# yesint/molar

Measured on AMD Instinct MI355X. Metric: frames/sec + Matom-pairs/sec, 1M-atom PBC neighbor search + RMSD fit, higher is better.
Workload: dtype f32; 1 GPU; 1M-atom synthetic triclinic box A, per frame: PBC neighbour search rc=1.2 nm (ordered pair list in HBM) + Kabsch RMSD fit/COM/gyration of a 100k-atom selection; natoms=1000000, selection_atoms=100000, frames_per_gpu=1451, parallelism=frames sharded over 1 rank(s), no data-path collective, streams_per_gpu=2, measure_overlapped_with_search=True

## Files before the change

include/molar_hip.h:

```cpp
#ifndef MOLAR_HIP_H
#define MOLAR_HIP_H

#include <stddef.h>
#include <stdint.h>

#ifdef __cplusplus
extern "C" {
#endif

enum {
    MOLAR_HIP_OK = 0,
    MOLAR_HIP_ERR_SIZES = 1,
    MOLAR_HIP_ERR_ZERO_MASS = 2,
    MOLAR_HIP_ERR_SVD = 3,
    MOLAR_HIP_ERR_NO_PBC = 4,
    MOLAR_HIP_ERR_ZERO_LENGTH_VECTOR = 5,
    MOLAR_HIP_ERR_INVERSE_FAILED = 6,
    MOLAR_HIP_ERR_LIPID_TAIL_TOO_SHORT = 7,
    MOLAR_HIP_ERR_LIPID_NORMALS_COUNT = 8,
    MOLAR_HIP_ERR_LIPID_BOND_ORDER_COUNT = 9,
    MOLAR_HIP_ERR_ANGLE_TOO_SMALL = 10,
    MOLAR_HIP_ERR_INVALID_ARGUMENT = 50,
    MOLAR_HIP_ERR_TOO_LARGE = 51,
    MOLAR_HIP_ERR_NO_SEARCH = 52,
// ... 54 lines not shown
    int32_t kind;
    float cutoff;
    const float *xyz1;
    size_t natoms1;
    const uint64_t *idx1;
    size_t n1;
    const float *xyz2;
    size_t natoms2;
    const uint64_t *idx2;
    size_t n2;
    const float *vdw1;
    const float *vdw2;
    int32_t ids_local;
    const float *box9;
    uint8_t pbc;
    const float *lower3;
    const float *upper3;
} molar_hip_search_desc;

int molar_hip_search_count(molar_hip_ctx *ctx, const molar_hip_search_desc *desc, uint64_t *out_count);
int molar_hip_search_fill(molar_hip_ctx *ctx, uint32_t *pairs, float *dist);
int molar_hip_search_fill_usize(molar_hip_ctx *ctx, uint64_t *i, uint64_t *j, float *dist);
int molar_hip_search_fill_ids(molar_hip_ctx *ctx, uint64_t *ids);
int molar_hip_within_count(molar_hip_ctx *ctx, const molar_hip_search_desc *desc, uint64_t *out_count);
int molar_hip_within_fill(molar_hip_ctx *ctx, uint64_t *ids);
int molar_hip_within_hold(molar_hip_ctx *ctx, int on);
int molar_hip_search_connectivity(molar_hip_ctx *ctx, const molar_hip_search_desc *desc, uint64_t *out_rows, uint64_t *out_entries);
int molar_hip_search_connectivity_fill(molar_hip_ctx *ctx, uint64_t *offsets, uint64_t *neigh);
int molar_hip_unwrap_connectivity(molar_hip_ctx *ctx, float *xyz, size_t natoms, const uint64_t *idx, size_t n,
                                  const float *box9, float cutoff, uint8_t pbc_dims, uint64_t *group_offsets,
                                  uint64_t *group_ids, size_t *ngroups);
int molar_hip_search_grid_dims(molar_hip_ctx *ctx, uint64_t dims[3]);
int molar_hip_search_cell_kernels(molar_hip_ctx *ctx, int32_t *lanes, uint64_t occupied_cells[2]);
int molar_hip_search_fill_device(molar_hip_ctx *ctx, const uint32_t **d_pairs, const float **d_dist);
int molar_hip_search_resident(molar_hip_ctx *ctx, const molar_hip_search_desc *desc, uint64_t *out_count,
                              const uint32_t **d_pairs, const float **d_dist);
int molar_hip_search_resident_planes(molar_hip_ctx *ctx, int want_dist);
int molar_hip_search_resident_begin(molar_hip_ctx *ctx, const molar_hip_search_desc *desc, int32_t *ticket);
int molar_hip_search_resident_end(molar_hip_ctx *ctx, int32_t ticket, uint64_t *out_count, const uint32_t **d_pairs,
                                  const float **d_dist);
int molar_hip_search_histogram(molar_hip_ctx *ctx, const molar_hip_search_desc *desc, float hmin,
                               float hmax, size_t nbins, uint64_t *bins, uint64_t *out_count);
int molar_hip_search_histogram_frames(molar_hip_ctx *ctx, const molar_hip_search_desc *desc, size_t nframes, size_t xyz1_stride,
                                      size_t xyz2_stride, const float *boxes9, float hmin, float hmax, size_t nbins,
                                      uint64_t *bins);
int molar_hip_histogram_edges(float hmin, float hmax, size_t nbins, float *edges);

typedef struct {
    const uint32_t *group1;
    size_t ngroups1;
    const uint32_t *group2;
    size_t ngroups2;
} molar_hip_contact_groups;

int molar_hip_search_contacts(molar_hip_ctx *ctx, const molar_hip_search_desc *desc, const molar_hip_contact_groups *groups ,
                              uint64_t *deg1, uint64_t *deg2, uint64_t *map, uint64_t *out_count);
int molar_hip_search_contacts_frames(molar_hip_ctx *ctx, const molar_hip_search_desc *desc, const molar_hip_contact_groups *groups,
                                     size_t nframes, size_t xyz1_stride, size_t xyz2_stride, const float *boxes9,
                                     uint64_t *deg1, uint64_t *deg2, uint64_t *map, uint32_t *occupancy);

typedef struct {
    int32_t kind;
    double cutoff;
    const double *xyz1;
    size_t natoms1;
    const uint64_t *idx1;
// ... 351 lines not shown
```

molar_amd/_lib.py:

```python
from __future__ import annotations

import ctypes as C
import os

HERE = os.path.dirname(os.path.abspath(__file__))
DEFAULT_LIB = os.path.join(HERE, "libmolar_hip.so")

_lib = None


class MolarHipError(RuntimeError):

    def __init__(self, code: int, msg: str):
        super().__init__(f"[molar_hip status {code}] {msg}")
        self.code = code


class Box(C.Structure):
    _fields_ = [("m", C.c_float * 9), ("inv", C.c_float * 9), ("nshift", C.c_int32), ("shifts", C.c_float * 78)]


class SearchDesc(C.Structure):
    _fields_ = [
        ("kind", C.c_int32), ("cutoff", C.c_float),
# ... 48 lines not shown


_P, _SZ, _F, _I, _U8 = C.c_void_p, C.c_size_t, C.c_float, C.c_int, C.c_uint8
SYMBOLS = {
    "molar_hip_create": (C.c_void_p, [_I]),
    "molar_hip_destroy": (None, [_P]),
    "molar_hip_last_error": (C.c_char_p, []),
    "molar_hip_version": (C.c_char_p, []),
    "molar_hip_device_count": (_I, []),
    "molar_hip_set_stream": (_I, [_P, _P]),
    "molar_hip_synchronize": (_I, [_P]),
    "molar_hip_profile_enable": (_I, [_P, _I]),
    "molar_hip_profile_read": (_I, [_P, _P, _P]),
    "molar_hip_box_from_matrix": (_I, [_P, _P]),
    "molar_hip_box_from_vectors_angles": (_I, [_F, _F, _F, _F, _F, _F, _P]),
    "molar_hip_box_shortest_vector": (None, [_P, _P, _U8, _P]),
    "molar_hip_copy_bandwidth": (_I, [_P, _SZ, _I, _P]),
    "molar_hip_write_bandwidth": (_I, [_P, _SZ, _I, _P]),
    "molar_hip_box_lab_extents": (None, [_P, _P]),
    "molar_hip_box_extents": (None, [_P, _P]),
    "molar_hip_box_to_box_coords": (None, [_P, _P, _P]),
    "molar_hip_box_to_lab_coords": (None, [_P, _P, _P]),
    "molar_hip_box_is_inside": (_I, [_P, _P]),
    "molar_hip_box_wrap_point": (None, [_P, _P, _P]),
    "molar_hip_search_count": (_I, [_P, _P, _P]),
    "molar_hip_search_fill": (_I, [_P, _P, _P]),
    "molar_hip_search_fill_usize": (_I, [_P, _P, _P, _P]),
    "molar_hip_search_fill_ids": (_I, [_P, _P]),
    "molar_hip_within_count": (_I, [_P, _P, _P]),
    "molar_hip_within_fill": (_I, [_P, _P]),
    "molar_hip_within_hold": (_I, [_P, _I]),
    "molar_hip_search_grid_dims": (_I, [_P, _P]),
    "molar_hip_search_cell_kernels": (_I, [_P, _P, _P]),
    "molar_hip_search_count_f64": (_I, [_P, _P, _P]),
    "molar_hip_search_fill_f64": (_I, [_P, _P, _P, _P]),
    "molar_hip_search_fill_ids_f64": (_I, [_P, _P]),
    "molar_hip_search_grid_dims_f64": (_I, [_P, _P]),
    "molar_hip_search_histogram_f64": (_I, [_P, _P, C.c_double, C.c_double, _SZ, _P, _P]),
    "molar_hip_search_histogram_frames_f64": (_I, [_P, _P, _SZ, _SZ, _SZ, _P, C.c_double, C.c_double, _SZ, _P]),
    "molar_hip_histogram_edges_f64": (_I, [C.c_double, C.c_double, _SZ, _P]),
    "molar_hip_within_count_f64": (_I, [_P, _P, _P]),
    "molar_hip_within_fill_f64": (_I, [_P, _P]),
    "molar_hip_search_connectivity_f64": (_I, [_P, _P, _P, _P]),
    "molar_hip_unwrap_connectivity_f64": (_I, [_P, _P, _SZ, _P, _SZ, _P, C.c_double, _U8, _P, _P, _P]),
    "molar_hip_search_resident": (_I, [_P, _P, _P, _P, _P]),
    "molar_hip_search_fill_device": (_I, [_P, _P, _P]),
    "molar_hip_search_resident_planes": (_I, [_P, _I]),
    "molar_hip_search_resident_begin": (_I, [_P, _P, _P]),
    "molar_hip_search_resident_end": (_I, [_P, C.c_int32, _P, _P, _P]),
    "molar_hip_search_histogram": (_I, [_P, _P, _F, _F, _SZ, _P, _P]),
    "molar_hip_search_histogram_frames": (_I, [_P, _P, _SZ, _SZ, _SZ, _P, _F, _F, _SZ, _P]),
    "molar_hip_histogram_edges": (_I, [_F, _F, _SZ, _P]),
    "molar_hip_search_contacts": (_I, [_P, _P, _P, _P, _P, _P, _P]),
    "molar_hip_search_contacts_frames": (_I, [_P, _P, _P, _SZ, _SZ, _SZ, _P, _P, _P, _P, _P]),
    "molar_hip_min_max": (_I, [_P, _P, _SZ, _P, _SZ, _P, _P]),
    "molar_hip_center_of_geometry": (_I, [_P, _P, _SZ, _P, _SZ, _P]),
    "molar_hip_center_of_mass": (_I, [_P, _P, _SZ, _P, _SZ, _P, _P]),
    "molar_hip_center_of_geometry_pbc": (_I, [_P, _P, _SZ, _P, _SZ, _P, _U8, _P]),
    "molar_hip_center_of_mass_pbc": (_I, [_P, _P, _SZ, _P, _SZ, _P, _P, _U8, _P]),
    "molar_hip_gyration": (_I, [_P, _P, _SZ, _P, _SZ, _P, _P, _P]),
    "molar_hip_inertia": (_I, [_P, _P, _SZ, _P, _SZ, _P, _P, _P, _P, _P]),
    "molar_hip_rmsd": (_I, [_P, _P, _SZ, _P, _SZ, _P, _SZ, _P, _SZ, _P]),
    "molar_hip_rmsd_mw": (_I, [_P, _P, _SZ, _P, _SZ, _P, _P, _SZ, _P, _SZ, _P]),
    "molar_hip_fit_transform": (_I, [_P, _P, _SZ, _P, _SZ, _P, _P, _SZ, _P, _SZ, _P, _I, _P, _P]),
    "molar_hip_xtc_histogram": (_I, [_P, _P, _SZ, _SZ, _P, _SZ, _F, _U8, _F, _F, _SZ, _P, _I]),
    "molar_hip_xtc_histogram_double": (_I, [_P, _P, _SZ, _SZ, _P, _SZ, _P, _SZ, _F, _U8, _F, _F, _SZ, _P, _I]),
# ... 133 lines not shown
```

molar_amd/api.py:

```python
from __future__ import annotations

import collections
import ctypes as C

import numpy as np

from . import _lib
from ._lib import (MEMBRANE_ARRAYS, Box, ContactGroups, MembraneDesc, MembraneOut, MembraneView, MolarHipError, SearchDesc, SearchDescF64,
                   check)

PBC_FULL = 7
PBC_NONE = 0

SEARCH_SINGLE, SEARCH_DOUBLE, SEARCH_WITHIN, SEARCH_DOUBLE_VDW = 0, 1, 2, 3


def _is_torch(x) -> bool:
    return type(x).__module__.startswith("torch")


def _addr(x):
    if x is None:
        return None, None
    if _is_torch(x):
# ... 214 lines not shown
            b9 = box.colmajor9() if isinstance(box, PeriodicBox) else np.ascontiguousarray(
                np.asarray(box, np.float32).reshape(3, 3).T).reshape(9)
            keep.append(b9)
            d.box9 = b9.ctypes.data
        d.pbc = pbc_mask(pbc)
        if lower is not None:
            lo = np.ascontiguousarray(lower, np.float32); up = np.ascontiguousarray(upper, np.float32)
            keep += [lo, up]
            d.lower3 = lo.ctypes.data
            d.upper3 = up.ctypes.data
        return d, keep

    def search_count(self, kind, cutoff, xyz1, idx1=None, xyz2=None, idx2=None, box=None, pbc=0, vdw1=None,
                     vdw2=None, ids_local=False, lower=None, upper=None) -> int:
        d, keep = self._search_desc(kind, cutoff, xyz1, idx1, xyz2, idx2, box, pbc, vdw1, vdw2, ids_local, lower, upper)
        cnt = C.c_uint64(0)
        check(self.lib.molar_hip_search_count(self.ctx, C.byref(d), C.byref(cnt)))
        self._keep = keep
        return int(cnt.value)

    def make_search_desc(self, kind, cutoff, xyz1, **kw):
        return self._search_desc(kind, cutoff, xyz1, **kw)

    def search_resident_desc(self, desc):
        cnt = C.c_uint64(0); p = C.c_void_p(); dd = C.c_void_p()
        check(self.lib.molar_hip_search_resident(self.ctx, C.byref(desc), C.byref(cnt), C.byref(p), C.byref(dd)))
        return int(cnt.value), p.value, dd.value

    def search_cell_kernels(self):
        lanes = C.c_int32(-1)
        occ = (C.c_uint64 * 2)()
        check(self.lib.molar_hip_search_cell_kernels(self.ctx, C.byref(lanes), occ))
        return int(lanes.value), (int(occ[0]), int(occ[1]))

    def search_resident_planes(self, want_dist=True):
        check(self.lib.molar_hip_search_resident_planes(self.ctx, 1 if want_dist else 0))

    def search_resident_begin(self, desc):
        t = C.c_int32(-1)
        check(self.lib.molar_hip_search_resident_begin(self.ctx, C.byref(desc), C.byref(t)))
        return int(t.value)

    def search_resident_end(self, ticket):
        cnt = C.c_uint64(0); p = C.c_void_p(); dd = C.c_void_p()
        check(self.lib.molar_hip_search_resident_end(self.ctx, C.c_int32(ticket), C.byref(cnt), C.byref(p), C.byref(dd)))
        return int(cnt.value), p.value, dd.value

    def search_resident(self, kind, cutoff, xyz1, idx1=None, xyz2=None, idx2=None, box=None, pbc=0, vdw1=None,
                        vdw2=None, ids_local=False, lower=None, upper=None):
        d, keep = self._search_desc(kind, cutoff, xyz1, idx1, xyz2, idx2, box, pbc, vdw1, vdw2, ids_local, lower, upper)
        cnt = C.c_uint64(0); p = C.c_void_p(); dd = C.c_void_p()
        check(self.lib.molar_hip_search_resident(self.ctx, C.byref(d), C.byref(cnt), C.byref(p), C.byref(dd)))
        self._keep = keep
        return int(cnt.value), p.value, dd.value

    def search_fill(self, count):
        pairs = np.empty((count, 2), np.uint32)
        dist = np.empty(count, np.float32)
        check(self.lib.molar_hip_search_fill(self.ctx, pairs.ctypes.data, dist.ctypes.data))
        return pairs, dist

    def search_fill_usize(self, count):
        i = np.empty(count, np.uint64); j = np.empty(count, np.uint64); d = np.empty(count, np.float32)
        check(self.lib.molar_hip_search_fill_usize(self.ctx, i.ctypes.data, j.ctypes.data, d.ctypes.data))
        return i, j, d

# ... 1729 lines not shown
```

molar_amd/build.py:

```python
from __future__ import annotations

import fcntl
import hashlib
import os
import subprocess

HERE = os.path.dirname(os.path.abspath(__file__))
CSRC = os.path.join(HERE, "csrc")
LIB = os.path.join(HERE, "libmolar_hip.so")
SOURCES = ["api.hip", "search.hip", "search_f64.hip", "measure.hip", "measure_f64.hip", "membrane.hip", "xtc.hip", "pair_k0.hip", "pair_k1.hip", "pair_k2.hip", "pair_k3.hip", "pair_k4.hip", "pair_k5.hip", "pair_k6.hip", "pair_k7.hip", "pair_k8.hip", "pair_k9.hip", "pair_small.hip", "devsort.hip", "sasa.hip", "rmsd_matrix.hip", "fluct.hip", "msd.hip"]
HEADERS = ["common.hpp", "boxmath.hpp", "linalg3.hpp", "pair_kernels.hpp", "hist_kernels.hpp", "contact_kernels.hpp", "hoststream.hpp", "stages.hpp", "csr_kernels.hpp", "unwrap_walk.hpp", "search_shape.hpp", os.path.join("..", "..", "include", "molar_hip.h")]
FLAGS = ["--offload-arch=gfx950", "-O3", "-std=c++17", "-fPIC", "-ffp-contract=off", "-fno-fast-math",
         "-Wall", "-Wno-unused-function",
         "-fno-slp-vectorize"]
FLAGS += os.environ.get("MOLAR_HIP_EXTRA_FLAGS", "").split()


HASH_FILE = LIB + ".srchash"


def _source_hash() -> str:
    h = hashlib.sha256()
    h.update(" ".join(FLAGS).encode())
    for name in sorted(SOURCES + HEADERS):
        with open(os.path.join(CSRC, name), "rb") as f:
            h.update(name.encode())
            h.update(f.read())
    return h.hexdigest()


def needs_build() -> bool:
    if not os.path.exists(LIB) or not os.path.exists(HASH_FILE):
        return True
    try:
        return open(HASH_FILE).read().strip() != _source_hash()
    except OSError:
        return True


def build_library(force: bool = False, verbose: bool = False) -> str:
    if not force and not needs_build():
        return LIB
    with open(os.path.join(HERE, ".build.lock"), "w") as lock:
# ... 127 lines not shown
```

molar_amd/csrc/api.hip:

```cpp
#include "boxmath.hpp"
#include <algorithm>

#include "common.hpp"
#include "hoststream.hpp"
namespace mh { void search64_release(molar_hip_ctx *c); }
namespace mh { void sasa_release(molar_hip_ctx *c); }
namespace mh { void rmsd_matrix_release(molar_hip_ctx *c); }
namespace mh { void fluct_release(molar_hip_ctx *c); }
namespace mh { void msd_release(molar_hip_ctx *c); }
#include <cstdlib>

using namespace mh;

typedef float v4f_copy __attribute__((ext_vector_type(4)));
__global__ __launch_bounds__(256) void k_copy_f4(const float4 *__restrict__ src, float4 *__restrict__ dst, size_t n) {
    for (size_t i = (size_t)blockIdx.x * 256u + threadIdx.x; i < n; i += (size_t)gridDim.x * 256u) dst[i] = src[i];
}
template <bool NT>
__global__ __launch_bounds__(256) void k_copy_f4x4(const v4f_copy *__restrict__ src, v4f_copy *__restrict__ dst, size_t n) {
    for (size_t i = (size_t)blockIdx.x * 1024u + threadIdx.x; i < n; i += (size_t)gridDim.x * 1024u) {
        v4f_copy v0, v1, v2, v3;
        if (NT) {
            v0 = __builtin_nontemporal_load(src + i);
            v1 = __builtin_nontemporal_load(src + i + 256);
// ... 121 lines not shown
    if ((e = hipStreamCreateWithFlags(&c->stream, hipStreamNonBlocking)) != hipSuccess) {
        fail(MOLAR_HIP_ERR_HIP, "hipStreamCreate: %s", hipGetErrorString(e));
        delete c;
        return nullptr;
    }
    c->own_stream = true;
#ifdef MOLAR_HIP_AB_KNOBS
    c->env_no_side = std::getenv("MOLAR_HIP_NO_SIDE_STREAM") != nullptr;
    c->env_no_mfma = std::getenv("MOLAR_HIP_NO_MFMA_COUNT") != nullptr;
    c->env_no_mfma_wrapped = std::getenv("MOLAR_HIP_NO_MFMA_WRAPPED") != nullptr;
    c->env_no_tile_sum = std::getenv("MOLAR_HIP_NO_TILE_SUM") != nullptr;
    c->env_host_grid_wait = std::getenv("MOLAR_HIP_HOST_GRID_WAIT") != nullptr;
    c->env_no_bin_tile = std::getenv("MOLAR_HIP_NO_BIN_TILE") != nullptr;
#endif
#ifdef MOLAR_HIP_DEBUG_KNOBS
    if (const char *dbg = std::getenv("MOLAR_HIP_DEBUG_SKIP")) c->env_debug_skip = (uint32_t)std::atoi(dbg);
    if (const char *dbg = std::getenv("MOLAR_HIP_DEBUG_LAUNCH")) c->env_debug_launch = (uint32_t)std::atoi(dbg);
#endif
    if (ensure_pinned(c, 1 << 16)) {
        (void)hipStreamDestroy(c->stream);
        delete c;
        return nullptr;
    }
    return c;
}

void molar_hip_destroy(molar_hip_ctx *c) {
    if (!c) return;
    (void)hipSetDevice(c->device);
    (void)hipStreamSynchronize(c->stream);
    if (c->side_stream) (void)hipStreamSynchronize(c->side_stream);
    for (auto &gen : c->set_store) for (auto &s : gen) {
        for (DevBuf *b : {&s.xyz_stage, &s.idx_stage, &s.vdw_stage, &s.key, &s.cell_count, &s.cnt_pad, &s.cursor, &s.tmp_key, &s.sort_buf,
                          &s.sorted, &s.sorted_vdw, &s.aabb, &s.perm, &s.chunk_aabb, &s.h16, &s.cell_org})
            b->release();
    }
    if (c->aux) molar_hip_destroy(c->aux);
    if (c->contacts) {
        c->contacts->stream = c->stream;
        molar_hip_destroy(c->contacts);
    }
    for (DevBuf *b : {&c->xh_win[0], &c->xh_win[1], &c->xh_bins, &c->fit_redo, &c->ct_g1, &c->ct_g2, &c->ct_acc, &c->ct_frame, &c->ct_occ}) b->release();
    for (auto &gen : c->hb_sets) for (auto &fr : gen) for (auto &s : fr) {
        for (DevBuf *b : {&s.xyz_stage, &s.idx_stage, &s.vdw_stage, &s.key, &s.cell_count, &s.cnt_pad, &s.cursor, &s.tmp_key, &s.sort_buf,
                          &s.sorted, &s.sorted_vdw, &s.aabb, &s.perm, &s.chunk_aabb, &s.h16, &s.cell_org})
            b->release();
    }
    for (DevBuf *b : {&c->hb_lean[0], &c->hb_lean[1], &c->hb_rest[0], &c->hb_rest[1], &c->hb_blocks[0], &c->hb_blocks[1]}) b->release();
    if (c->hb_pin) (void)hipHostFree(c->hb_pin);
    for (auto e : c->hb_pin_ev)
        if (e) (void)hipEventDestroy(e);
    for (DevBuf *b : {&c->params, &c->task_desc, &c->task_nb, &c->slot_desc, &c->slot_cnt, &c->slot_base, &c->tile_sum, &c->scan_tmp, &c->sort_tmp, &c->sort_tmp_side, &c->scan_tmp_side, &c->scan_state, &c->fplan_tiles, &c->out_pairs_set[0], &c->out_dist_set[0], &c->out_pairs_set[1], &c->out_dist_set[1], &c->out_ids,
                      &c->wide_i, &c->wide_j, &c->hist, &c->hist_queue, &c->slot_desc_rest, &c->hist_edges, &c->dbg, &c->conn_deg, &c->conn_off, &c->conn_ent, &c->conn_neigh, &c->w_flags, &c->w_list, &c->w_part_cnt, &c->w_part, &c->w_tile_cnt, &c->w_tile_off, &c->task_mu, &c->task_moff, &c->maskbuf, &c->m_xyz1, &c->m_xyz2, &c->m_idx1, &c->m_idx2,
                      &c->m_mass1, &c->m_mass2, &c->m_partials, &c->m_results, &c->m_out})
        b->release();
    for (auto &s : c->spans) {
        (void)hipEventDestroy(s.a);
        (void)hipEventDestroy(s.b);
    }
    for (auto e : c->event_pool) (void)hipEventDestroy(e);
    if (c->h_pinned) (void)hipHostFree(c->h_pinned);
    mh::ring_release(c);
    mh::search64_release(c);
    mh::sasa_release(c);
    mh::rmsd_matrix_release(c);
    mh::fluct_release(c);
    mh::msd_release(c);
    if (c->h_sizes) (void)hipHostFree(c->h_sizes);
    for (auto &t : c->tickets)
        if (t.done) (void)hipEventDestroy(t.done);
    if (c->grid_done) (void)hipEventDestroy(c->grid_done);
    for (auto e : c->gen_free)
        if (e) (void)hipEventDestroy(e);
    if (c->side_stream) (void)hipStreamDestroy(c->side_stream);
    if (c->own_stream) (void)hipStreamDestroy(c->stream);
    delete c;
}

int molar_hip_set_stream(molar_hip_ctx *c, void *hip_stream) {
    if (!c) return fail(MOLAR_HIP_ERR_INVALID_ARGUMENT, "null context");
    MH_HIP(hipSetDevice(c->device));
    MH_HIP(hipStreamSynchronize(c->stream));
    if (c->own_stream) (void)hipStreamDestroy(c->stream);
    c->stream = reinterpret_cast<hipStream_t>(hip_stream);
    c->own_stream = false;
// ... 118 lines not shown
```

molar_amd/csrc/common.hpp:

```cpp
#pragma once

#include <hip/hip_runtime.h>

#include <cstdarg>
#include <cstdint>
#include <cstdio>
#include <cstring>
#include <string>
#include <vector>

#include "../../include/molar_hip.h"

namespace mh {


inline std::string &last_error() {
    static thread_local std::string e;
    return e;
}

inline int fail(int code, const char *fmt, ...) {
    char buf[512];
    va_list ap;
    va_start(ap, fmt);
// ... 51 lines not shown
inline bool is_device_ptr(const void *p) {
    if (!p) return false;
    hipPointerAttribute_t a;
    hipError_t e = hipPointerGetAttributes(&a, p);
    if (e != hipSuccess) {
        (void)hipGetLastError();
        return false;
    }
    return a.type == hipMemoryTypeDevice || a.type == hipMemoryTypeManaged || a.type == hipMemoryTypeArray;
}


struct GridSet {
    uint32_t n = 0;
    DevBuf xyz_stage;
    DevBuf idx_stage;
    DevBuf vdw_stage;
    const float *d_xyz = nullptr;
    const uint64_t *d_idx = nullptr;
    const float *d_vdw = nullptr;
    DevBuf key;
    DevBuf cell_count;
    DevBuf cnt_pad;
    DevBuf cursor;
    DevBuf tmp_key;
    DevBuf sort_buf;
    DevBuf sorted;
    DevBuf sorted_vdw;
    DevBuf aabb;
    DevBuf perm;
    DevBuf chunk_aabb;
    DevBuf h16;
    DevBuf cell_org;
};

struct SearchShape {
    int kind = 0;
    bool use_box = false;
    uint8_t pbc = 0;
    float cutoff = 0.f;
    molar_hip_box box{};
    float lower[3]{}, upper[3]{};
    uint32_t dims[3]{1, 1, 1};
    uint64_t ntasks = 0;
    uint64_t nslots_bound = 0;
    GridSet *set = nullptr;
    uint32_t occ_use[2] = {0, 0};
};

}

struct molar_hip_search64_state;
struct molar_hip_sasa_state;
struct molar_hip_rmsd_matrix_state;
struct molar_hip_fluct_state;
struct molar_hip_msd_state;

#ifndef MH_HIST_BATCH
#define MH_HIST_BATCH 16
#endif

struct molar_hip_ctx {
    int device = 0;
    hipStream_t stream = nullptr;
    bool own_stream = false;
    int num_cus = 256;
// ... 10 lines not shown

    bool have_search = false;
    mh::SearchShape cur;
    uint64_t total = 0;
    mh::GridSet set_store[2][2];
    molar_hip_ctx() { cur.set = set_store[0]; }
    hipStream_t side_stream = nullptr;
    hipEvent_t grid_done = nullptr;
    bool env_no_side = false;
    bool env_no_mfma = false;
    bool env_no_mfma_wrapped = false;
    bool env_host_grid_wait = false;
    bool env_no_tile_sum = false;
    uint32_t env_debug_skip = 0;
    uint32_t env_debug_launch = 0, dbg_launches = 0;
    hipEvent_t gen_free[2] = {nullptr, nullptr};
    bool env_no_bin_tile = false;
    int hist_gen = 0;
    bool on_side = false;
    mh::DevBuf scan_tmp_side;
    mh::DevBuf params;
    mh::DevBuf task_desc;
    mh::DevBuf task_nb;
    mh::DevBuf slot_desc;
    mh::DevBuf slot_cnt;
    mh::DevBuf slot_base;
    mh::DevBuf tile_sum;
    bool params_fresh = false;
    unsigned long long params_fresh_cap = 0;
    mh::DevBuf scan_tmp;
    mh::DevBuf sort_tmp, sort_tmp_side;
    mh::DevBuf scan_state;
    mh::DevBuf fplan_tiles;
    mh::DevBuf out_pairs_set[2];
    mh::DevBuf out_dist_set[2];
    mh::DevBuf &out_pairs = out_pairs_set[0];
    mh::DevBuf &out_dist = out_dist_set[0];
    struct Ticket {
        bool pending = false, degenerate = false;
        unsigned long long cap0 = 0, maskcap0 = 0, serial = 0, launched = 0, ntasks = 0;
        int kind = -1;
        unsigned long long occ_key = 0;
        hipEvent_t done = nullptr;
        molar_hip_search_desc desc{};
    } tickets[2];
    int next_ticket = 0;
    bool resident_no_dist = false;
    unsigned long long search_serial = 0;
    unsigned long long trim_real = 0, trim_ntasks = 0;
    int trim_kind = -1;
    void *h_sizes = nullptr;
    unsigned long long occ_key = 0;
    uint32_t occ_cells[2] = {0, 0};
    bool occ_valid = false;
    mh::DevBuf out_ids;
    mh::DevBuf wide_i, wide_j;
    mh::DevBuf hist;
    mh::DevBuf dbg;
    mh::DevBuf hist_queue;
    mh::DevBuf slot_desc_rest;
    unsigned long long hist_frames = 0;
    mh::GridSet hb_sets[2][MH_HIST_BATCH][2];
    bool hb_zeroed[2][MH_HIST_BATCH][2] = {};
    uint32_t hb_zeroed_cells[2][MH_HIST_BATCH][2] = {};
    mh::DevBuf hb_lean[2], hb_rest[2];
    mh::DevBuf hb_blocks[2];
// ... 114 lines not shown
```

molar_amd/csrc/pair_kernels.hpp:

```cpp
#pragma once

#include "boxmath.hpp"
#include "common.hpp"

namespace mh {
namespace pairk {

enum { MODE_COUNT = 0, MODE_FILL = 1, MODE_HIST = 2 };

#ifndef MH_COUNT_WPE
#define MH_COUNT_WPE 6
#endif
#ifndef MH_FILL_WPE
#define MH_FILL_WPE 8
#endif
#ifndef MH_WPB
#define MH_WPB 1
#endif
constexpr int waves_per_block(int mode) { return mode == MODE_HIST ? 4 : MH_WPB; }
constexpr int KREG = 8;
constexpr int FIFO_CAP = 128;
#ifndef MOLAR_HIP_NO_WIDE_FLUSH
#define MOLAR_HIP_WIDE_FLUSH 1
#endif
constexpr int FIFO_WIDE = 256;
constexpr uint32_t XCD_RUN = 128;
constexpr float F32_EPS = 1.1920929e-07f;
constexpr bool MASKED_COUNT_SORTED = true;

static __constant__ uint8_t MASKS[14][6] = {
    {0, 0, 0, 0, 0, 0},
    {0, 0, 0, 1, 0, 0}, {0, 0, 0, 0, 1, 0}, {0, 0, 0, 0, 0, 1},
    {0, 0, 0, 1, 1, 0}, {0, 0, 0, 1, 0, 1}, {0, 0, 0, 0, 1, 1},
    {0, 0, 0, 1, 1, 1},
    {1, 0, 0, 0, 1, 0}, {1, 0, 0, 0, 0, 1}, {0, 1, 0, 0, 0, 1},
    {1, 1, 0, 0, 0, 1}, {1, 0, 1, 0, 1, 0}, {0, 1, 1, 1, 0, 0},
};


typedef float v4f_t __attribute__((ext_vector_type(4)));
__device__ __forceinline__ float4 gload4(const float4 *p, size_t i) {
    const v4f_t v = ((const __attribute__((address_space(1))) v4f_t *)p)[i];
    return make_float4(v.x, v.y, v.z, v.w);
}
__device__ __forceinline__ uint32_t gload_u32(const uint32_t *p, size_t i) {
    return ((const __attribute__((address_space(1))) uint32_t *)p)[i];
}
__device__ __forceinline__ void gstore_u32(uint32_t *p, size_t i, uint32_t v) {
    ((__attribute__((address_space(1))) uint32_t *)p)[i] = v;
}
__device__ __forceinline__ float uniform_f32(float v) { return __uint_as_float(__builtin_amdgcn_readfirstlane(__float_as_uint(v))); }
__device__ __forceinline__ float4 lload4(const float4 *p, uint32_t i) {
    const v4f_t v = ((const __attribute__((address_space(3))) v4f_t *)p)[i];
    return make_float4(v.x, v.y, v.z, v.w);
// ... 37 lines not shown
#ifdef MOLAR_HIP_DEBUG_KNOBS
    uint32_t debug_skip;
    unsigned long long *dbg;
#endif
    float cutoff2;
    uint64_t ntasks;
    molar_hip_box box;
    alignas(16) float shifts4[96];
    uint32_t hist_big;
};

struct TaskDesc {
    uint32_t a0, n1, b0, n2, cb, flags, pad0, pad1;
};

struct SlotDesc {
    uint32_t a0, n1, b0, n2;
    uint32_t cb, flags, i0, frame;
    unsigned long long moff, pad1;
};
static_assert(sizeof(SlotDesc) == 48, "SlotDesc is read with three 16-byte loads");

struct Task {
    uint32_t a0, n1, b0, n2;
    uint32_t rps;
    uint32_t cb;
    uint32_t ca;
    uint32_t wrap_b;
    uint32_t wrap;
    bool tri;
    bool valid;
};

template <int KIND, bool UNIFORM>
__device__ __forceinline__ Task decode_task(const SearchParams &P, uint64_t t) {
    Task T;
    T.valid = false;
    T.tri = false;
    T.a0 = T.b0 = T.n1 = T.n2 = 0;
    T.cb = 0;
    T.ca = 0;
    T.wrap_b = 0;
    T.rps = 64u;
    T.wrap = 0;
    uint32_t half = 0;
    uint64_t e = t;
    if (KIND != MOLAR_HIP_SEARCH_SINGLE) {
        half = (uint32_t)(t & 1ull);
        e = t >> 1;
    }
    const uint32_t m = (uint32_t)(e % 14ull);
    const uint64_t cidx = e / 14ull;
    const uint32_t z = (uint32_t)(cidx % P.dz);
    const uint64_t r = cidx / P.dz;
    const uint32_t y = (uint32_t)(r % P.dy);
    const uint32_t x = (uint32_t)(r / P.dy);
    const uint32_t dims[3] = {P.dx, P.dy, P.dz};
    uint32_t c[2][3] = {{x + MASKS[m][0], y + MASKS[m][1], z + MASKS[m][2]},
                        {x + MASKS[m][3], y + MASKS[m][4], z + MASKS[m][5]}};
    uint32_t wrap = 0, wrap_c2 = 0;
    for (int i = 0; i < 2; ++i)
        for (int d = 0; d < 3; ++d)
            if (c[i][d] == dims[d]) {
                if ((P.pbc >> d) & 1u) {
                    c[i][d] = 0;
                    wrap |= 1u << d;
// ... 414 lines not shown
    if (P.box.nshift != 0 && wrap == MOLAR_HIP_PBC_FULL) {
        if (WIDE4) {
            for (int k = 0; k < P.box.nshift; k += 4) {
                float sh[12];
#pragma unroll
                for (int q = 0; q < 12; ++q) sh[q] = P.shifts4[3 * k + q];
#pragma unroll
                for (int q = 0; q < 4; ++q) {
                    const float cx = sx + sh[3 * q], cy = sy + sh[3 * q + 1], cz = sz + sh[3 * q + 2];
                    const float n2 = (cx * cx + cy * cy) + cz * cz;
                    best2 = n2 < best2 ? n2 : best2;
                }
            }
        } else {
            for (int k = 0; k < P.box.nshift; ++k) {
                const float cx = sx + P.box.shifts[3 * k], cy = sy + P.box.shifts[3 * k + 1], cz = sz + P.box.shifts[3 * k + 2];
                const float n2 = (cx * cx + cy * cy) + cz * cz;
                best2 = n2 < best2 ? n2 : best2;
            }
        }
    }
    return best2;
}

__device__ __forceinline__ float aabb_d2(float ax, float ay, float az, float lx, float ly, float lz, float hx, float hy,
                                         float hz) {
    const float ex = fmaxf(fmaxf(lx - ax, ax - hx), 0.f);
    const float ey = fmaxf(fmaxf(ly - ay, ay - hy), 0.f);
    const float ez = fmaxf(fmaxf(lz - az, az - hz), 0.f);
    return (ex * ex + ey * ey) + ez * ez;
}

template <int KIND, int NCH, bool TRI>
__device__ __forceinline__ uint32_t run_count_sorted(const SearchParams &P, const Task &T, uint32_t i0, float4 *la,
                                                     uint32_t lane) {
    const float cutoff2 = P.cutoff2;
    const uint32_t rows = __builtin_amdgcn_readfirstlane(T.n1 - i0 < T.rps ? T.n1 - i0 : T.rps);
    float4 a = make_float4(0.f, 0.f, 0.f, 0.f);
    if (lane < rows) a = gload4(P.sa, T.a0 + i0 + lane);
    la[lane] = a;
    float bx[NCH], by[NCH], bz[NCH];
    uint32_t bpos[NCH];
#pragma unroll
    for (int k = 0; k < NCH; ++k) {
        const uint32_t jj = (uint32_t)k * 64u + lane;
        float4 q = make_float4(3.0e38f, 3.0e38f, 3.0e38f, 0.f);
        uint32_t pj = 0u;
        if (jj < T.n2) {
            q = gload4(P.perm_b, T.b0 + jj);
            pj = __float_as_uint(q.w);
        }
        bx[k] = q.x; by[k] = q.y; bz[k] = q.z; bpos[k] = pj;
    }
    const uint32_t ubase = (T.b0 >> 6) + T.cb;
    unsigned long long livek[NCH];
#pragma unroll
    for (int k = 0; k < NCH; ++k) {
        const float4 lo = gload4(P.chunk_aabb_b, 2u * (ubase + k)), hi = gload4(P.chunk_aabb_b, 2u * (ubase + k) + 1u);
        const bool need = lane < rows && !(aabb_d2(a.x, a.y, a.z, lo.x, lo.y, lo.z, hi.x, hi.y, hi.z) > cutoff2);
        livek[k] = __builtin_amdgcn_ballot_w64(need);
    }
    __builtin_amdgcn_wave_barrier();
    uint32_t acc = 0;
    unsigned long long live = 0ull;
#pragma unroll
    for (int k = 0; k < NCH; ++k) live |= livek[k];
    while (live) {
        const uint32_t r = (uint32_t)__builtin_ctzll(live);
        live &= ~(1ull << r);
        const float4 p = lload4(la, r);
#pragma unroll
        for (int k = 0; k < NCH; ++k) {
            if (!((livek[k] >> r) & 1ull)) continue;
            const float dx = bx[k] - p.x, dy = by[k] - p.y, dz = bz[k] - p.z;
            float d2 = (dx * dx + dy * dy) + dz * dz;
            if (TRI) d2 = (bpos[k] > i0 + r) ? d2 : INFINITY;
            asm volatile("v_cmp_ge_f32 vcc, %2, %1\n\tv_addc_co_u32 %0, vcc, 0, %0, vcc" : "+v"(acc) : "v"(d2), "s"(cutoff2) : "vcc");
        }
    }
    for (int off = 32; off > 0; off >>= 1) acc += __shfl_xor(acc, off, 64);
    return acc;
}

typedef _Float16 v8h_t __attribute__((ext_vector_type(8)));
typedef float v16f_t __attribute__((ext_vector_type(16)));

__device__ __forceinline__ uint32_t pack_h2(_Float16 a, _Float16 b) {
    return (uint32_t)__builtin_bit_cast(unsigned short, a) | ((uint32_t)__builtin_bit_cast(unsigned short, b) << 16);
}

constexpr int MFMA_TILES = 10;

__device__ __forceinline__ float mfma_error_bound(float R, float c) {
    return 2.3841858e-07f * ((16.0f * R * R + 8.0f * c) + (4.0f * R + 1.0f));
}
__device__ __forceinline__ bool mfma_bound_usable(float R, float E, float c) {
    return R < 64.0f && E < 0.02f * c && (c + R * R) < 3.0e4f;
}

template <int KIND, bool TRI>
__device__ __forceinline__ uint32_t run_count_mfma(const SearchParams &P, const Task &T, uint32_t i0, float4 *la, uint4 *lh,
                                                   uint32_t lane, bool &done) {
    typedef uint32_t u4_t __attribute__((ext_vector_type(4)));
    typedef __attribute__((address_space(3))) u4_t lds_u4;
    typedef __attribute__((address_space(3))) uint32_t lds_u32;
    typedef __attribute__((address_space(1))) u4_t glb_u4;
    const float cutoff2 = P.cutoff2;
    const uint32_t rows = __builtin_amdgcn_readfirstlane(T.n1 - i0 < T.rps ? T.n1 - i0 : T.rps);
    const uint32_t kh = lane >> 5, cl = lane & 31u;
    const uint32_t nct = (T.n2 + 31u) >> 5;
    float4 a = make_float4(0.f, 0.f, 0.f, 0.f);
    if (lane < rows) a = gload4(P.sa, T.a0 + i0 + lane);
    const float4 org = gload4(P.cell_org_b, T.cb);
    bool need = lane < rows;
    if (!TRI) {
        const float4 blo = gload4(P.aabb_b, 2 * T.cb), bhi = gload4(P.aabb_b, 2 * T.cb + 1);
        need = need && !(aabb_d2(a.x, a.y, a.z, blo.x, blo.y, blo.z, bhi.x, bhi.y, bhi.z) > cutoff2);
    }
    const unsigned long long live = __builtin_amdgcn_ballot_w64(need);
    const uint32_t nlive = TRI ? rows : (uint32_t)__popcll(live);
    if (!TRI && nlive == 0u) return 0u;
    const uint32_t rank = TRI ? lane : __builtin_amdgcn_mbcnt_hi((uint32_t)(live >> 32), __builtin_amdgcn_mbcnt_lo((uint32_t)live, 0u));
    u4_t bq[MFMA_TILES];
#pragma unroll
    for (int t = 0; t < MFMA_TILES; ++t) {
        const uint32_t col = (uint32_t)t * 32u + cl;
        if (32u * (uint32_t)(t + 1) <= T.n2) {
            bq[t] = ((const glb_u4 *)P.h16_b)[T.b0 + col];
        } else {
            bq[t] = u4_t{0u, 0u, 0u, 0x00007BFFu};
            if (col < T.n2) bq[t] = ((const glb_u4 *)P.h16_b)[T.b0 + col];
        }
    }
    if (TRI || need) la[rank] = a;
    const float r0 = a.x - org.x, r1 = a.y - org.y, r2 = a.z - org.z;
    float ra2 = need ? (r0 * r0 + r1 * r1) + r2 * r2 : 0.0f;
    const bool fin = ra2 == ra2;
    for (int off = 32; off > 0; off >>= 1) ra2 = fmaxf(ra2, __shfl_xor(ra2, off, 64));
    const float R = 1.0001f * __builtin_sqrtf(ra2) + org.w;
    const float E = uniform_f32(mfma_error_bound(R, cutoff2));
    if (__builtin_amdgcn_ballot_w64(!fin) != 0ull || !mfma_bound_usable(R, E, cutoff2)) {
        done = false;
        return 0u;
    }
    {
        u4_t k0 = {0u, 0u, 0u, 0x00007BFFu}, k1 = {0u, 0u, 0u, 0x3C003C00u};
        if (!TRI) {
            ((lds_u4 *)lh)[2u * lane] = k0;
// ... 53 lines not shown
                    m = __builtin_fminf(m, __builtin_fabsf(acc[i]));
                }
                if (__builtin_amdgcn_ballot_w64(m < E) == 0ull) {
                    cnt += (uint32_t)__popc(h);
                } else {
                    if (lane == 0) todo[ntodo] = (uint32_t)(2 * t + rt);
                    ++ntodo;
                }
            }
        }
    }
    if (ntodo) {
        __builtin_amdgcn_wave_barrier();
        for (uint32_t q = 0; q < ntodo; ++q) {
            const uint32_t id = __builtin_amdgcn_readfirstlane(todo[q]);
            const uint32_t ct = id >> 1, rt = id & 1u;
            const uint32_t col = ct * 32u + cl;
            float4 b = make_float4(3.0e38f, 3.0e38f, 3.0e38f, 0.f);
            if (col < T.n2) b = gload4(P.sb, T.b0 + col);
            for (uint32_t r = 0; r < 16u; ++r) {
                const uint32_t row = 32u * rt + 16u * kh + r;
                const float4 p = lload4(la, row);
                const float dx = b.x - p.x, dy = b.y - p.y, dz = b.z - p.z;
                const float d2 = (dx * dx + dy * dy) + dz * dz;
                cnt += (row < nlive && (!TRI || col > i0 + row) && d2 <= cutoff2) ? 1u : 0u;
            }
        }
    }
    for (int off = 32; off > 0; off >>= 1) cnt += __shfl_xor(cnt, off, 64);
    return cnt;
}

template <int KIND>
__device__ __forceinline__ bool run_count_mfma_wrapped(const SearchParams &P, const Task &T, uint32_t i0, float4 *la, uint4 *lh,
                                                       uint32_t lane, uint32_t *mwords, uint32_t &count_out) {
    typedef uint32_t u4_t __attribute__((ext_vector_type(4)));
    typedef __attribute__((address_space(3))) u4_t lds_u4;
    typedef __attribute__((address_space(3))) uint32_t lds_u32;
    typedef __attribute__((address_space(1))) u4_t glb_u4;
    const float cutoff2 = P.cutoff2;
    const uint32_t rows = __builtin_amdgcn_readfirstlane(T.n1 - i0 < 64u ? T.n1 - i0 : 64u);
    const uint32_t kh = lane >> 5, cl = lane & 31u;
    const uint32_t nct = (T.n2 + 31u) >> 5, nch = (T.n2 + 63u) >> 6;
    float Sx = 0.f, Sy = 0.f, Sz = 0.f;
    for (int d = 0; d < 3; ++d) {
        if (!((T.wrap >> d) & 1u)) continue;
        const float sgn = ((T.wrap_b >> d) & 1u) ? 1.0f : -1.0f;
        Sx += sgn * P.box.m[3 * d];
        Sy += sgn * P.box.m[3 * d + 1];
        Sz += sgn * P.box.m[3 * d + 2];
    }
    float4 a = make_float4(0.f, 0.f, 0.f, 0.f);
    if (lane < rows) a = gload4(P.sa, T.a0 + i0 + lane);
    const float4 org = gload4(P.cell_org_b, T.cb);
    const float4 blo = gload4(P.aabb_b, 2 * T.cb), bhi = gload4(P.aabb_b, 2 * T.cb + 1);
    const bool need = lane < rows && !(aabb_d2(a.x - Sx, a.y - Sy, a.z - Sz, blo.x, blo.y, blo.z, bhi.x, bhi.y, bhi.z) > P.prune_limit2);
    const unsigned long long live = __builtin_amdgcn_ballot_w64(need);
    const uint32_t nlive = (uint32_t)__popcll(live);
    if (nlive == 0u) {
        count_out = 0u;
        return true;
    }
    const uint32_t rank = __builtin_amdgcn_mbcnt_hi((uint32_t)(live >> 32), __builtin_amdgcn_mbcnt_lo((uint32_t)live, 0u));
    const float r0 = (a.x - Sx) - org.x, r1 = (a.y - Sy) - org.y, r2 = (a.z - Sz) - org.z;
    float ra2 = need ? (r0 * r0 + r1 * r1) + r2 * r2 : 0.0f;
    float big = need ? fmaxf(fmaxf(fabsf(a.x), fabsf(a.y)), fabsf(a.z)) : 0.0f;
    const bool fin = ra2 == ra2;
    for (int off = 32; off > 0; off >>= 1) {
        ra2 = fmaxf(ra2, __shfl_xor(ra2, off, 64));
        big = fmaxf(big, __shfl_xor(big, off, 64));
    }
    const float R = 1.0001f * __builtin_sqrtf(ra2) + org.w;
    const float rc = __builtin_sqrtf(P.band_hi);
    const float L = (fmaxf(fmaxf(fabsf(org.x), fabsf(org.y)), fabsf(org.z)) + R) + (fmaxf(fmaxf(fabsf(Sx), fabsf(Sy)), fabsf(Sz)) + big);
    const float Em = mfma_error_bound(R, cutoff2);
    const float E = uniform_f32((P.band_hi - cutoff2) * 1.0001f + Em + 4.0f * (5.9604645e-08f * (2.0f * L + 2.0f * rc)) * rc);
    if (__builtin_amdgcn_ballot_w64(!fin || !(E == E) || !mfma_bound_usable(R, Em, cutoff2) || !(E < 0.06f * cutoff2)) != 0ull) return false;
    u4_t bq[MFMA_TILES];
#pragma unroll
    for (int t = 0; t < MFMA_TILES; ++t) {
        const uint32_t col = (uint32_t)t * 32u + cl;
        if (32u * (uint32_t)(t + 1) <= T.n2) {
            bq[t] = ((const glb_u4 *)P.h16_b)[T.b0 + col];
        } else {
            bq[t] = u4_t{0u, 0u, 0u, 0x00007BFFu};
            if (col < T.n2) bq[t] = ((const glb_u4 *)P.h16_b)[T.b0 + col];
        }
    }
    {
// ... 69 lines not shown
                cnt += (uint32_t)__popc(word);
                gstore_u32(mwords, ((uint32_t)rt * nch + (uint32_t)k) * 64u + lane, word);
            }
        }
    }
    if (ntodo > TODO_CAP) return false;
    if (ntodo) {
        asm volatile("s_waitcnt vmcnt(0)" ::: "memory");
        __builtin_amdgcn_wave_barrier();
        for (uint32_t q0 = 0; q0 < ntodo; q0 += 64u) {
            bool hx = false;
            uint32_t rl = 0u, col = 0u;
            if (q0 + lane < ntodo) {
                const uint32_t e = todo[q0 + lane];
                rl = e >> 16;
                col = e & 0xFFFFu;
                if (rl < nlive && col < T.n2) {
                    const float4 b = gload4(P.sb, T.b0 + col);
                    const float4 p = lload4(la, rl);
                    hx = wrapped_d2_exact(P, T.wrap, b.x - p.x, b.y - p.y, b.z - p.z) <= cutoff2;
                }
            }
            if (hx) atomicOr(mwords + ((rl >> 5) * nch + (col >> 6)) * 64u + (col & 63u), 0x80000000u >> (rl & 31u));
            const unsigned long long mx = __builtin_amdgcn_ballot_w64(hx);
            if (lane == 0) cnt += (uint32_t)__popcll(mx);
        }
    }
    for (int off = 32; off > 0; off >>= 1) cnt += __shfl_xor(cnt, off, 64);
    count_out = cnt;
    return true;
}

template <int KIND, bool FILL, bool WRAPPED, int NCH, bool TRI, bool MASKED>
__device__ __forceinline__ uint32_t run_fast(const SearchParams &P, const Task &T, uint32_t i0, Fifo &F, float4 *la,
                                             uint32_t lane, uint32_t *mwords) {
    static_assert(!(WRAPPED && TRI), "a triangular (same-cell) entry never wraps on the fast path");
    if constexpr (!FILL && !WRAPPED && MASKED_COUNT_SORTED) return run_count_sorted<KIND, NCH, TRI>(P, T, i0, la, lane);
    const bool approx = WRAPPED && P.approx_wrapped != 0u && !(P.box.nshift != 0 && T.wrap == MOLAR_HIP_PBC_FULL);
    float Sx = 0.f, Sy = 0.f, Sz = 0.f;
    if (WRAPPED && approx) {
        for (int d = 0; d < 3; ++d) {
            if (!((T.wrap >> d) & 1u)) continue;
            const float sgn = ((T.wrap_b >> d) & 1u) ? 1.0f : -1.0f;
            Sx += sgn * P.box.m[3 * d];
            Sy += sgn * P.box.m[3 * d + 1];
            Sz += sgn * P.box.m[3 * d + 2];
        }
    }
    constexpr bool REPLAY = FILL && MASKED;
    float bx[NCH], by[NCH], bz[NCH];
    uint32_t bid[NCH];
    if (!REPLAY) {
#pragma unroll
        for (int k = 0; k < NCH; ++k) {
            const uint32_t jj = (uint32_t)k * 64u + lane;
            float4 q = make_float4(3.0e38f, 3.0e38f, 3.0e38f, 0.f);
            if (jj < T.n2) {
                q = gload4(P.sb, T.b0 + jj);
                if (WRAPPED) { q.x += Sx; q.y += Sy; q.z += Sz; }
            }
            bx[k] = q.x; by[k] = q.y; bz[k] = q.z; bid[k] = __float_as_uint(q.w);
        }
    }
    const float cutoff2 = P.cutoff2;
    const float band_lo = P.band_lo, band_hi = P.band_hi;
    const uint32_t rows = __builtin_amdgcn_readfirstlane(T.n1 - i0 < T.rps ? T.n1 - i0 : T.rps);
    unsigned long long live;
    {
        float4 a = make_float4(0.f, 0.f, 0.f, 0.f);
        if (lane < rows) a = gload4(P.sa, T.a0 + i0 + lane);
        la[lane] = a;
        const float4 lo = gload4(P.aabb_b, 2 * T.cb), hi = gload4(P.aabb_b, 2 * T.cb + 1);
        bool need = true;
        if (TRI) {
        } else if (!WRAPPED) {
            need = !(aabb_d2(a.x, a.y, a.z, lo.x, lo.y, lo.z, hi.x, hi.y, hi.z) > cutoff2);
        } else if (approx) {
            need = !(aabb_d2(a.x - Sx, a.y - Sy, a.z - Sz, lo.x, lo.y, lo.z, hi.x, hi.y, hi.z) > P.prune_limit2);
        }
        live = __builtin_amdgcn_ballot_w64(lane < rows && need);
    }
    __builtin_amdgcn_wave_barrier();
    uint32_t total = 0;

    if (REPLAY) {
        if (!mwords) return 0u;
        F.recompute = WRAPPED ? 1u : 2u;
        F.la = la;
        F.wrap = T.wrap;
        F.fq = F.fq_store;
        float4 q[NCH];
#pragma unroll
        for (int k = 0; k < NCH; ++k) {
            const uint32_t jj = (uint32_t)k * 64u + lane;
            q[k] = make_float4(0.f, 0.f, 0.f, 0.f);
            if (jj < T.n2) q[k] = gload4(P.sb, T.b0 + jj);
        }
        uint32_t w[NCH];
        uint32_t nrow = 0;
        while (live) {
            if ((nrow & 31u) == 0u) {
#pragma unroll
                for (int k = 0; k < NCH; ++k) w[k] = gload_u32(mwords, ((nrow >> 5) * NCH + k) * 64u + lane);
            }
            ++nrow;
            const uint32_t r = (uint32_t)__builtin_ctzll(live);
            live &= ~(1ull << r);
// ... 143 lines not shown
                            else acc += 1u;
                        }
                    }
                }
                acc_hi = acc;
            }
        }
        if (!FILL && MASKED) {
            if ((++nrow & 31u) == 0u) store_group((nrow >> 5) - 1u, 32u);
        }
    }
    if (!FILL) {
        if (MASKED && (nrow & 31u) != 0u) store_group(nrow >> 5, nrow & 31u);
        for (int off = 32; off > 0; off >>= 1) acc += __shfl_xor(acc, off, 64);
        total = acc;
    } else if (F.tail != F.head) {
        __builtin_amdgcn_wave_barrier();
        if (WIDE) {
            while (F.tail != F.head) {
                const uint32_t c = F.tail - F.head < 64u ? F.tail - F.head : 64u;
                fifo_flush<KIND, FIFO_WIDE>(P, F, c, lane);
            }
        } else {
            fifo_flush<KIND>(P, F, F.tail - F.head, lane);
        }
    }
    if (FILL) F.recompute = 0u;
    return total;
}

constexpr int KMAX_WIDE = 16;
constexpr int KMAX_HUGE = 32;
template <int KIND, bool FILL, int WK, bool MASKED, int KMAX = KREG>
__device__ __forceinline__ uint32_t run_task_nch(const SearchParams &P, const Task &T, uint32_t i0, Fifo &F, float4 *la,
                                                 uint32_t lane, uint32_t *mwords) {
    const uint32_t nchunks = (T.n2 + 63u) >> 6;
    if constexpr (KMAX > KMAX_WIDE) {
        if ((KIND == MOLAR_HIP_SEARCH_SINGLE || KIND == MOLAR_HIP_SEARCH_DOUBLE) && nchunks > (uint32_t)KREG && nchunks <= (uint32_t)KMAX) {
            constexpr bool WR = WK != WK_NONE;
            const bool tri = KIND == MOLAR_HIP_SEARCH_SINGLE && WK == WK_NONE && T.tri;
            if (!T.tri || tri) {
#define MH_HUGE_CASE(N)                                                                                              \
    if (nchunks <= (uint32_t)(N)) {                                                                                  \
        if (tri) {                                                                                                   \
            if constexpr (KIND == MOLAR_HIP_SEARCH_SINGLE && WK == WK_NONE)                                          \
                return run_fast<KIND, FILL, false, N, true, false>(P, T, i0, F, la, lane, nullptr);                  \
        }                                                                                                            \
        return run_fast<KIND, FILL, WR, N, false, false>(P, T, i0, F, la, lane, nullptr);                            \
    }
                MH_HUGE_CASE(16) MH_HUGE_CASE(20) MH_HUGE_CASE(24) MH_HUGE_CASE(28) MH_HUGE_CASE(32)
#undef MH_HUGE_CASE
            }
        }
    } else if constexpr (KMAX > KREG) {
        if ((KIND == MOLAR_HIP_SEARCH_SINGLE || KIND == MOLAR_HIP_SEARCH_DOUBLE) && nchunks > (uint32_t)KREG && nchunks <= (uint32_t)KMAX) {
            constexpr bool WR = WK != WK_NONE;
            const bool tri = KIND == MOLAR_HIP_SEARCH_SINGLE && WK == WK_NONE && T.tri;
            if (!T.tri || tri) {
#define MH_WIDE_CASE(N)                                                                                              \
    case N:                                                                                                          \
        if (tri) {                                                                                                   \
            if constexpr (KIND == MOLAR_HIP_SEARCH_SINGLE && WK == WK_NONE)                                          \
                return run_fast<KIND, FILL, false, N, true, false>(P, T, i0, F, la, lane, nullptr);                  \
        }                                                                                                            \
        return run_fast<KIND, FILL, WR, N, false, false>(P, T, i0, F, la, lane, nullptr);
                switch (nchunks) {
                    MH_WIDE_CASE(9) MH_WIDE_CASE(10) MH_WIDE_CASE(11) MH_WIDE_CASE(12)
// ... 105 lines not shown
            SlotDesc z;
            z.a0 = z.n1 = z.b0 = z.n2 = z.cb = z.flags = z.i0 = z.frame = 0u;
            z.moff = ~0ull >> 1;
            z.pad1 = 0ull;
            slot_desc[s] = z;
        }
        return;
    }
    const uint32_t s0 = task_first[t], s1 = task_first[t + 1];
    if (s1 == s0) return;
    const TaskDesc d = task_desc[t];
    const uint32_t rps = d.flags >> 16, nch = (d.n2 + 63u) >> 6;
    const unsigned long long m0 = task_moff ? task_moff[t] : (~0ull >> 1);
    for (uint32_t s = s0; s < s1; ++s) {
        SlotDesc o;
        o.a0 = d.a0; o.n1 = d.n1; o.b0 = d.b0; o.n2 = d.n2;
        o.cb = d.cb; o.flags = d.flags; o.i0 = (s - s0) * rps; o.frame = 0u;
        o.moff = task_moff ? m0 + (unsigned long long)(s - s0) * 2u * nch : m0;
        o.pad1 = 0ull;
        slot_desc[s] = o;
    }
}

template <int KIND>
__device__ __forceinline__ bool hist_lean_slot(const SearchParams &P, uint32_t flags, uint32_t n2) {
    if (KIND != MOLAR_HIP_SEARCH_SINGLE && KIND != MOLAR_HIP_SEARCH_DOUBLE) return false;
    if (((n2 + 63u) >> 6) > (uint32_t)KREG && !P.hist_big) return false;
    const uint32_t wrap = flags & 7u;
    if (!(P.use_box && wrap != 0u)) return true;
    if (flags & 0x100u) return false;
    return P.approx_wrapped != 0u && !(P.box.nshift != 0 && wrap == MOLAR_HIP_PBC_FULL);
}

template <int KIND, int MODE, int WPE = 0>
__global__ void __launch_bounds__(64 * waves_per_block(MODE))
__attribute__((amdgpu_waves_per_eu(WPE ? WPE : (MODE == MODE_HIST ? 4 : (MODE == MODE_COUNT ? MH_COUNT_WPE : MH_FILL_WPE))))) pair_kernel(const SearchParams *__restrict__ Pp,
                                                     const SlotDesc *__restrict__ slot_desc,
                                                     const uint32_t nslots_arg,
                                                     uint32_t *__restrict__ slot_cnt,
                                                     const unsigned long long *__restrict__ slot_base,
                                                     uint2 *__restrict__ out_pairs, float *__restrict__ out_dist,
                                                     uint32_t *__restrict__ out_ids) {
    constexpr int WAVES_PER_BLOCK = waves_per_block(MODE), BLOCK = 64 * WAVES_PER_BLOCK;
    constexpr int PLANE = MODE != MODE_COUNT ? FIFO_WIDE : FIFO_CAP;
    static_assert(FIFO_CAP * 16 <= 2 * FIFO_WIDE * 4, "the replay queue fits in two planes");
    __shared__ __attribute__((aligned(16))) uint32_t lds[WAVES_PER_BLOCK][3][PLANE];
    __shared__ float4 lds_a[WAVES_PER_BLOCK][64];
    __shared__ uint4 lds_h[MODE == MODE_COUNT ? WAVES_PER_BLOCK : 1][MODE == MODE_COUNT ? 128 : 1];
    constexpr bool FILL = MODE != MODE_COUNT;
    extern __shared__ uint32_t lds_hist[];
    const SearchParams &P0 = *Pp;
#ifdef MH_SLOT_LOOP
    uint32_t lane_var = threadIdx.x & 63u;
    const uint32_t &lane = lane_var;
#else
    const uint32_t lane = threadIdx.x & 63u;
#endif
    uint32_t nslots = nslots_arg;
    if (MODE == MODE_HIST && P0.hist_nslots) {
        const uint32_t real = __builtin_amdgcn_readfirstlane(P0.hist_nslots[0]);
        nslots = real < nslots_arg ? real : nslots_arg;
    }
    const uint32_t wave = WAVES_PER_BLOCK == 1 ? 0u : __builtin_amdgcn_readfirstlane(threadIdx.x >> 6);
    constexpr bool hist = MODE == MODE_HIST;
    if (hist) {
        for (uint32_t b = threadIdx.x; b < P0.hist_nbins; b += BLOCK) lds_hist[b] = 0u;
        __syncthreads();
    }
    unsigned long long wave_total = 0;
    auto process_slot = [&](uint32_t w) __attribute__((always_inline)) {
        uint32_t wr = w;
        {
            const uint32_t x = w & 7u, q = w >> 3;
            const uint32_t full = (nslots / (8u * XCD_RUN)) * (8u * XCD_RUN);
            if (w < full) wr = ((q / XCD_RUN) * 8u + x) * XCD_RUN + (q % XCD_RUN);
        }
        const uint32_t slot = nslots - 1u - wr;
        Task T;
        uint32_t i0;
        unsigned long long moff;
        uint32_t frame = 0u;
        {
            const uint4 lo = reinterpret_cast<const uint4 *>(slot_desc + slot)[0];
            const uint4 hi = reinterpret_cast<const uint4 *>(slot_desc + slot)[1];
            const uint2 mo = reinterpret_cast<const uint2 *>(slot_desc + slot)[4];
            const uint32_t fl = __builtin_amdgcn_readfirstlane(hi.y);
            if (!(fl & 0x200u)) return;
            if (MODE == MODE_HIST) frame = __builtin_amdgcn_readfirstlane(hi.w);
            T.a0 = __builtin_amdgcn_readfirstlane(lo.x);
            T.n1 = __builtin_amdgcn_readfirstlane(lo.y);
            T.b0 = __builtin_amdgcn_readfirstlane(lo.z);
            T.n2 = __builtin_amdgcn_readfirstlane(lo.w);
            T.cb = __builtin_amdgcn_readfirstlane(hi.x);
            i0 = __builtin_amdgcn_readfirstlane(hi.z);
            moff = ((unsigned long long)__builtin_amdgcn_readfirstlane(mo.y) << 32) | __builtin_amdgcn_readfirstlane(mo.x);
            T.wrap = fl & 7u;
            T.tri = (fl & 0x100u) != 0u;
            T.valid = true;
            T.wrap_b = (fl >> 12) & 7u;
            T.rps = fl >> 16;
        }
        const SearchParams &P = MODE == MODE_HIST ? Pp[frame] : P0;
        Fifo F;
        F.fi = lds[wave][0];
        F.fj = lds[wave][1];
        F.fd = lds[wave][2];
        F.head = F.tail = 0;
        F.quota = 64u;
        F.has_pairs = out_pairs != nullptr;
        F.has_dist = out_dist != nullptr;
        F.pairs = nullptr;
        F.dist = nullptr;
        F.ids = nullptr;
        F.base = 0;
        F.room = 0xFFFFFFFFu;
        F.hist = hist ? lds_hist : nullptr;
        F.recompute = 0u;
        F.la = lds_a[wave];
        F.fq = nullptr;
        F.fq_store = MODE == MODE_FILL ? reinterpret_cast<float4 *>(lds[wave][0]) : nullptr;
        F.lh = MODE == MODE_COUNT ? lds_h[wave] : nullptr;
        F.wrap = 0;
        F.hmin = P.hist_min;
        F.hmax = P.hist_max;
        F.hn = (float)P.hist_nbins;
        if (FILL && !hist) {
            F.base = slot_base[slot];
            F.quota = 64u - ((uint32_t)F.base & 63u);
            const unsigned long long end = slot_base[slot + 1];
            if (end == F.base || end > P.out_cap) return;
            F.room = end - F.base < 0xFFFFFFFFull ? (uint32_t)(end - F.base) : 0xFFFFFFFFu;
            if (out_pairs) F.pairs = out_pairs + F.base + lane;
            if (out_dist) F.dist = out_dist + F.base + lane;
// ... 25 lines not shown
        wave_total += total;
    };
    const uint32_t w0 = (blockIdx.y * gridDim.x + blockIdx.x) * WAVES_PER_BLOCK + wave;
    if (!hist) {
#ifdef MH_SLOT_LOOP
#pragma unroll 1
        for (uint32_t g = 0; g < (uint32_t)MH_SLOT_LOOP; ++g) {
            const uint32_t w = w0 + g * (gridDim.x * gridDim.y * WAVES_PER_BLOCK);
            if (w < nslots) process_slot(w);
            asm volatile("" : "+v"(lane_var));
        }
#else
        if (w0 < nslots) process_slot(w0);
#endif
    } else {
        for (uint32_t w = w0; w < nslots; w += gridDim.x * gridDim.y * WAVES_PER_BLOCK) process_slot(w);
    }
    if (hist) {
        __syncthreads();
        for (uint32_t b = threadIdx.x; b < P0.hist_nbins; b += BLOCK) {
            const uint32_t v = lds_hist[b];
            if (v) atomicAdd(&P0.hist_bins[b], (unsigned long long)v);
        }
        if (lane == 0 && wave_total && P0.hist_total) atomicAdd(P0.hist_total, wave_total);
    }
}


inline dim3 pair_grid(unsigned nblocks) {
    const unsigned gx = nblocks < (1u << 24) ? (nblocks ? nblocks : 1u) : (1u << 24);
    return dim3(gx, (nblocks + gx - 1u) / gx);
}

template <int KIND, int MODE, int WPE = 0>
inline void launch_pair_kernel(unsigned nblocks, size_t dyn_lds, hipStream_t stream, const SearchParams *dP,
                               const SlotDesc *slot_desc, uint32_t nslots, uint32_t *slot_cnt,
                               const unsigned long long *slot_base, uint2 *pairs, float *dist, uint32_t *ids) {
    if (MODE != MODE_HIST) nblocks = (nblocks + (unsigned)waves_per_block(MODE) - 1u) / (unsigned)waves_per_block(MODE);
#ifdef MH_SLOT_LOOP
    if (MODE != MODE_HIST) nblocks = (nblocks + (unsigned)MH_SLOT_LOOP - 1u) / (unsigned)MH_SLOT_LOOP;
#endif
    hipLaunchKernelGGL((pair_kernel<KIND, MODE, WPE>), pair_grid(nblocks), dim3(64 * waves_per_block(MODE)), dyn_lds, stream, dP, slot_desc, nslots,
                       slot_cnt, slot_base, pairs, dist, ids);
}

}

void launch_hist_plan(int kind, hipStream_t stream, const pairk::SearchParams &P, pairk::SearchParams *params_dst, pairk::SlotDesc *lean,
                      pairk::SlotDesc *rest, uint32_t *queue, int lslot);
void launch_hist_plan_frames(int kind, hipStream_t stream, const pairk::SearchParams *params, unsigned nframes, uint64_t ntasks_max,
                             pairk::SlotDesc *lean, pairk::SlotDesc *rest, uint32_t *queue, int lslot);
void launch_hist_lean(int kind, unsigned num_cus, size_t dyn_lds, hipStream_t stream, const pairk::SearchParams *dP,
                      const pairk::SlotDesc *slot_desc, uint32_t nslots_bound, uint32_t *queue, int lslot, bool big);
size_t hist_queue_words();
const uint32_t *hist_list_count(const uint32_t *queue, int lslot, int which);
void launch_pair_wide(int kind, int mode, unsigned nblocks, hipStream_t stream, const pairk::SearchParams *dP,
                      const pairk::SlotDesc *slot_desc, uint32_t nslots, uint32_t *slot_cnt,
                      const unsigned long long *slot_base, uint2 *pairs, float *dist);
void launch_pair_huge(int kind, int mode, unsigned nblocks, hipStream_t stream, const pairk::SearchParams *dP,
                      const pairk::SlotDesc *slot_desc, uint32_t nslots, uint32_t *slot_cnt,
                      const unsigned long long *slot_base, uint2 *pairs, float *dist);
void launch_pair_single(int mode, unsigned nblocks, size_t dyn_lds, hipStream_t stream, const pairk::SearchParams *dP,
                        const pairk::SlotDesc *slot_desc, uint32_t nslots, uint32_t *slot_cnt,
                        const unsigned long long *slot_base, uint2 *pairs, float *dist, uint32_t *ids);
void launch_pair_double(int mode, unsigned nblocks, size_t dyn_lds, hipStream_t stream, const pairk::SearchParams *dP,
                        const pairk::SlotDesc *slot_desc, uint32_t nslots, uint32_t *slot_cnt,
                        const unsigned long long *slot_base, uint2 *pairs, float *dist, uint32_t *ids);
void launch_pair_within(int mode, unsigned nblocks, size_t dyn_lds, hipStream_t stream, const pairk::SearchParams *dP,
                        const pairk::SlotDesc *slot_desc, uint32_t nslots, uint32_t *slot_cnt,
                        const unsigned long long *slot_base, uint2 *pairs, float *dist, uint32_t *ids);
void launch_pair_vdw(int mode, unsigned nblocks, size_t dyn_lds, hipStream_t stream, const pairk::SearchParams *dP,
                     const pairk::SlotDesc *slot_desc, uint32_t nslots, uint32_t *slot_cnt,
                     const unsigned long long *slot_base, uint2 *pairs, float *dist, uint32_t *ids);

}
```

molar_amd/csrc/search.hip:

```cpp
#include <cstdlib>

#include "boxmath.hpp"
#include "common.hpp"
#include "csr_kernels.hpp"
#include "hoststream.hpp"
#include <algorithm>

#include "pair_kernels.hpp"
#include "contact_kernels.hpp"
#include "search_shape.hpp"
#include "stages.hpp"
#include "unwrap_walk.hpp"

namespace mh {
void launch_pair_small(int mode, int lanes_per_slot, hipStream_t stream, const pairk::SearchParams *dP, const pairk::SlotDesc *slot_desc,
                       uint32_t nslots, uint32_t *slot_cnt, const unsigned long long *slot_base, uint2 *pairs, float *dist);
}
using namespace mh;
using namespace mh::pairk;

namespace {

constexpr uint32_t DROPPED = 0xFFFFFFFFu;

// ... 454 lines not shown
        atomicAdd(occupied + (blockIdx.x & (OCC_WORDS - 1u)), 1u);
    place_order_body(P, ncells, ids_local, cell_start, tmp_key, vdw, sorted, sorted_vdw, aabb, perm, chunk_aabb, h16, cell_org, want_order, presorted);
}
__global__ void __launch_bounds__(64) place_order_frames_kernel(const GridFrame *__restrict__ G, uint32_t ncells, int ids_local) {
    const GridFrame &g = G[blockIdx.y];
    place_order_body(g.P, ncells, ids_local, g.cell_count, g.tmp_key, nullptr, g.sorted, nullptr, g.aabb, g.perm, g.chunk_aabb, g.h16, g.cell_org,
                     1, 0);
}



constexpr int SCAN_ITEMS = 8;
constexpr int SCAN_TILE = 256 * SCAN_ITEMS;

template <class TIn, class TOut>
__global__ void __launch_bounds__(256) scan_tile_kernel(const TIn *in, TOut *out, TOut *block_sums, uint64_t n) {
    const uint64_t base = (uint64_t)blockIdx.x * SCAN_TILE + (uint64_t)threadIdx.x * SCAN_ITEMS;
    TOut item[SCAN_ITEMS];
    TOut sum = 0;
    for (int q = 0; q < SCAN_ITEMS; ++q) {
        item[q] = base + q < n ? (TOut)in[base + q] : (TOut)0;
        sum += item[q];
    }
    TOut tot;
    TOut run = block_exclusive_scan<TOut>(sum, &tot);
    for (int q = 0; q < SCAN_ITEMS; ++q) {
        if (base + q < n) out[base + q] = run;
        run += item[q];
    }
    if (threadIdx.x == 0) block_sums[blockIdx.x] = tot;
}

constexpr unsigned long long LB_MASK = (1ull << 62) - 1ull;
constexpr uint64_t FPLAN_MAX_TASKS = 1ull << 22;
constexpr uint32_t PLAN_GROUP = 128;
__device__ __forceinline__ unsigned long long lb_resolve(unsigned long long *desc, uint32_t tile, unsigned long long tot) {
    if (tile == 0) {
        __hip_atomic_store(&desc[0], (2ull << 62) | tot, __ATOMIC_RELEASE, __HIP_MEMORY_SCOPE_AGENT);
        return 0ull;
    }
    __hip_atomic_store(&desc[tile], (1ull << 62) | tot, __ATOMIC_RELEASE, __HIP_MEMORY_SCOPE_AGENT);
    unsigned long long run = 0;
    for (uint32_t t = tile - 1u;; --t) {
        unsigned long long d;
        do {
            d = __hip_atomic_load(&desc[t], __ATOMIC_ACQUIRE, __HIP_MEMORY_SCOPE_AGENT);
        } while ((d >> 62) == 0ull);
        run += d & LB_MASK;
        if ((d >> 62) == 2ull) break;
    }
    __hip_atomic_store(&desc[tile], (2ull << 62) | (run + tot), __ATOMIC_RELEASE, __HIP_MEMORY_SCOPE_AGENT);
    return run;
}

template <class TIn1, class TOut1, class TIn2, class TOut2>
__global__ void __launch_bounds__(256) scan_lookback_kernel(const TIn1 *in1, TOut1 *out1, const TIn2 *in2, TOut2 *out2, uint64_t n,
                                                            unsigned long long *state, uint32_t ntiles) {
    __shared__ uint32_t tile_s;
    __shared__ unsigned long long pre_s[2];
    if (threadIdx.x == 0) tile_s = atomicAdd(reinterpret_cast<uint32_t *>(state), 1u);
    __syncthreads();
    const uint32_t tile = tile_s;
    unsigned long long *d1 = state + 1, *d2 = state + 1 + ntiles;
    const uint64_t base = (uint64_t)tile * (blockDim.x * SCAN_ITEMS) + (uint64_t)threadIdx.x * SCAN_ITEMS;
    TOut1 a[SCAN_ITEMS];
    TOut2 b[SCAN_ITEMS];
    TOut1 sa = 0;
// ... 7 lines not shown
    TOut1 ta;
    TOut1 ra = block_exclusive_scan<TOut1>(sa, &ta);
    TOut2 tb = 0, rb = 0;
    if (in2) rb = block_exclusive_scan<TOut2>(sb, &tb);
    if (threadIdx.x == 0) pre_s[0] = lb_resolve(d1, tile, (unsigned long long)ta);
    if (threadIdx.x == (blockDim.x > 64u ? 64u : 1u) && in2) pre_s[1] = lb_resolve(d2, tile, (unsigned long long)tb);
    __syncthreads();
    ra += (TOut1)pre_s[0];
    if (in2) rb += (TOut2)pre_s[1];
    for (int q = 0; q < SCAN_ITEMS; ++q) {
        if (base + q < n) {
            out1[base + q] = ra;
            if (in2) out2[base + q] = rb;
        }
        ra += a[q];
        rb += b[q];
    }
}

inline size_t lookback_state_words(uint64_t n) { return 1 + 2 * (size_t)((n + 64 * SCAN_ITEMS - 1) / (64 * SCAN_ITEMS)); }

template <class TIn1, class TOut1, class TIn2, class TOut2>
int scan_lookback(molar_hip_ctx *c, const TIn1 *in1, TOut1 *out1, const TIn2 *in2, TOut2 *out2, uint64_t n,
                  unsigned long long *zeroed_state) {
    if (n == 0) return 0;
    const uint32_t block = c->on_side ? 64u : 256u;
    const uint32_t ntiles = (uint32_t)((n + block * SCAN_ITEMS - 1) / (block * SCAN_ITEMS));
    hipLaunchKernelGGL((scan_lookback_kernel<TIn1, TOut1, TIn2, TOut2>), dim3(ntiles), dim3(block), 0, c->stream, in1, out1, in2, out2, n,
                       zeroed_state, ntiles);
    MH_HIP(hipGetLastError());
    return 0;
}

template <int KIND>
__global__ void __launch_bounds__(256) plan_tiles_kernel(SearchParams P, uint32_t *__restrict__ local_first, TaskDesc *__restrict__ task_desc,
                                                         unsigned long long *__restrict__ local_moff, uint32_t fast_kind,
                                                         uint32_t *__restrict__ slot_cnt, uint64_t nslot_cnt,
                                                         unsigned long long *__restrict__ tile_tot, SearchParams *__restrict__ params_dst) {
    const uint64_t t = (uint64_t)blockIdx.x * 256u + threadIdx.x;
    for (uint64_t w = t; w < nslot_cnt; w += (uint64_t)gridDim.x * 256u) slot_cnt[w] = 0u;
    if (params_dst && blockIdx.x == 0) {
        const uint32_t *src = (const uint32_t *)__builtin_amdgcn_kernarg_segment_ptr();
        uint32_t *d = (uint32_t *)params_dst;
        for (uint32_t w = threadIdx.x; w < (uint32_t)(sizeof(SearchParams) / 4u); w += 256u) d[w] = src[w];
    }
    uint32_t nb = 0;
    unsigned long long mu = 0;
    if (t < P.ntasks) {
        const Task T = decode_task<KIND, false>(P, t);
        nb = T.valid ? (T.n1 + T.rps - 1u) / T.rps : 0u;
        const uint32_t nch = (T.n2 + 63u) >> 6;
        mu = (fast_kind && P.use_box && T.wrap != 0u && nch <= (uint32_t)KREG) ? (unsigned long long)nb * 2u * nch : 0ull;
        TaskDesc d;
        d.a0 = T.a0; d.n1 = T.n1; d.b0 = T.b0; d.n2 = T.n2; d.cb = T.cb;
        d.flags = T.wrap | (T.tri ? 0x100u : 0u) | (T.valid ? 0x200u : 0u) | (T.wrap_b << 12) | (T.rps << 16);
        d.pad0 = nb;
        d.pad1 = 0u;
        task_desc[t] = d;
    }
    uint32_t tot_nb;
    const uint32_t first = block_exclusive_scan<uint32_t>(nb, &tot_nb);
    unsigned long long tot_mu = 0ull, m0 = 0ull;
    if (fast_kind) m0 = block_exclusive_scan<unsigned long long>(mu, &tot_mu);
    if (t <= P.ntasks) {
        local_first[t] = first;
        if (fast_kind) local_moff[t] = m0;
    }
    if (threadIdx.x == 0) {
        tile_tot[2 * blockIdx.x] = tot_nb;
        tile_tot[2 * blockIdx.x + 1] = tot_mu;
    }
}

static __global__ void __launch_bounds__(64) plan_groups_kernel(uint32_t ntiles, const unsigned long long *__restrict__ tile_tot,
                                                                unsigned long long *__restrict__ group_tot) {
    unsigned long long n = 0, m = 0;
    for (uint32_t k = threadIdx.x; k < PLAN_GROUP; k += 64u) {
        const uint32_t b = blockIdx.x * PLAN_GROUP + k;
        if (b < ntiles) { n += tile_tot[2 * b]; m += tile_tot[2 * b + 1]; }
    }
    for (int off = 32; off > 0; off >>= 1) {
        n += __shfl_xor(n, off, 64);
        m += __shfl_xor(m, off, 64);
    }
    if (threadIdx.x == 0) { group_tot[2 * blockIdx.x] = n; group_tot[2 * blockIdx.x + 1] = m; }
}

constexpr uint32_t PLAN_SUB = 64;
static __global__ void __launch_bounds__(256) plan_slots_kernel(uint64_t ntasks, uint32_t ntiles, const uint32_t *__restrict__ local_first,
                                                                const unsigned long long *__restrict__ local_moff,
                                                                uint32_t *__restrict__ task_first, const TaskDesc *__restrict__ task_desc,
                                                                unsigned long long *__restrict__ task_moff,
                                                                const unsigned long long *__restrict__ tile_tot,
                                                                SlotDesc *__restrict__ slot_desc, uint64_t nslots_bound,
                                                                unsigned long long *__restrict__ sizes_host,
                                                                const unsigned long long *__restrict__ group_tot) {
    __shared__ unsigned long long part[3][4];
    const uint32_t tile = blockIdx.x / (256u / PLAN_SUB), sub = blockIdx.x % (256u / PLAN_SUB);
    unsigned long long pn = 0, pm = 0, all_n = 0;
    if (!group_tot) {
        for (uint32_t b = threadIdx.x; b < ntiles; b += 256u) {
            const unsigned long long n = tile_tot[2 * b];
            all_n += n;
            if (b < tile) {
                pn += n;
                pm += tile_tot[2 * b + 1];
            }
        }
    } else {
        const uint32_t ngroups = (ntiles + PLAN_GROUP - 1u) / PLAN_GROUP, g = tile / PLAN_GROUP;
        for (uint32_t b = threadIdx.x; b < ngroups; b += 256u) {
            const unsigned long long n = group_tot[2 * b];
            all_n += n;
            if (b < g) {
                pn += n;
                pm += group_tot[2 * b + 1];
            }
        }
        for (uint32_t b = g * PLAN_GROUP + threadIdx.x; b < tile; b += 256u) {
            pn += tile_tot[2 * b];
            pm += tile_tot[2 * b + 1];
        }
    }
    for (int off = 32; off > 0; off >>= 1) {
        pn += __shfl_xor(pn, off, 64);
        pm += __shfl_xor(pm, off, 64);
        all_n += __shfl_xor(all_n, off, 64);
    }
    if ((threadIdx.x & 63u) == 0u) { part[0][threadIdx.x >> 6] = pn; part[1][threadIdx.x >> 6] = pm; part[2][threadIdx.x >> 6] = all_n; }
    __syncthreads();
    const uint32_t base_n = (uint32_t)((part[0][0] + part[0][1]) + (part[0][2] + part[0][3]));
    const unsigned long long base_m = (part[1][0] + part[1][1]) + (part[1][2] + part[1][3]);
    const unsigned long long total = (part[2][0] + part[2][1]) + (part[2][2] + part[2][3]);
    __shared__ uint32_t lfirst[PLAN_SUB + 1];
    __shared__ TaskDesc ldesc[PLAN_SUB];
    __shared__ unsigned long long lm0[PLAN_SUB];
    const uint32_t tile_n = (uint32_t)tile_tot[2 * tile];
    if (threadIdx.x <= PLAN_SUB) {
        const uint64_t t = (uint64_t)tile * 256u + sub * PLAN_SUB + threadIdx.x;
        const bool inside = threadIdx.x < PLAN_SUB || sub + 1u < 256u / PLAN_SUB;
        uint32_t local = tile_n;
        unsigned long long m0 = ~0ull >> 1;
        TaskDesc d;
        d.a0 = d.n1 = d.b0 = d.n2 = d.cb = d.flags = d.pad0 = d.pad1 = 0u;
        if (inside && t <= ntasks) {
            local = local_first[t];
            if (threadIdx.x < PLAN_SUB) {
                if (task_moff) m0 = base_m + local_moff[t];
                if (t < ntasks) d = task_desc[t];
            }
        }
        lfirst[threadIdx.x] = local;
        if (threadIdx.x < PLAN_SUB) {
            ldesc[threadIdx.x] = d;
            lm0[threadIdx.x] = m0;
        }
    }
    __syncthreads();
    if (threadIdx.x < PLAN_SUB) {
        const uint64_t t = (uint64_t)tile * 256u + sub * PLAN_SUB + threadIdx.x;
        if (t <= ntasks) {
            task_first[t] = base_n + lfirst[threadIdx.x];
            if (task_moff) task_moff[t] = lm0[threadIdx.x];
            if (t == ntasks && sizes_host) {
                sizes_host[1] = task_moff ? lm0[threadIdx.x] : 0ull;
                sizes_host[2] = base_n + lfirst[threadIdx.x];
            }
        }
    }
    const uint32_t s0 = lfirst[0], s1 = lfirst[PLAN_SUB];
    uint4 *out = reinterpret_cast<uint4 *>(slot_desc) + 3 * ((size_t)base_n + s0);
    for (uint32_t i = threadIdx.x; i < 3u * (s1 - s0); i += 256u) {
        const uint32_t sl = s0 + i / 3u, part3 = i % 3u;
        uint32_t lo = 0u, hi = PLAN_SUB;
        while (hi - lo > 1u) {
            const uint32_t mid = (lo + hi) >> 1;
            if (lfirst[mid] <= sl) lo = mid;
            else hi = mid;
        }
        const TaskDesc d = ldesc[lo];
        const uint32_t q = sl - lfirst[lo], rps = d.flags >> 16, nch = (d.n2 + 63u) >> 6;
        uint4 w;
        if (part3 == 0u) w = make_uint4(d.a0, d.n1, d.b0, d.n2);
        else if (part3 == 1u) w = make_uint4(d.cb, d.flags, q * rps, 0u);
        else {
            const unsigned long long mo = task_moff ? lm0[lo] + (unsigned long long)q * 2u * nch : lm0[lo];
            w = make_uint4((uint32_t)mo, (uint32_t)(mo >> 32), 0u, 0u);
        }
        out[i] = w;
    }
    if (total <= nslots_bound) {
        uint4 *blank = reinterpret_cast<uint4 *>(slot_desc) + 3 * (size_t)total;
        const uint64_t nw = 3ull * (nslots_bound + 1ull - total);
        for (uint64_t i = (uint64_t)blockIdx.x * 256u + threadIdx.x; i < nw; i += (uint64_t)gridDim.x * 256u)
            blank[i] = (i % 3ull == 2ull) ? make_uint4(0xFFFFFFFFu, 0x7FFFFFFFu, 0u, 0u) : make_uint4(0u, 0u, 0u, 0u);
    }
}

template <class T>
__global__ void __launch_bounds__(256) scan_sums_kernel(T *sums, uint64_t nb) {
    __shared__ T carry_s;
    if (threadIdx.x == 0) carry_s = 0;
    __syncthreads();
    for (uint64_t start = 0; start < nb; start += 256) {
        const uint64_t i = start + threadIdx.x;
        const T v = i < nb ? sums[i] : (T)0;
        T tot;
        const T ex = block_exclusive_scan<T>(v, &tot);
        const T carry = carry_s;
        if (i < nb) sums[i] = carry + ex;
        __syncthreads();
        if (threadIdx.x == 0) carry_s = carry + tot;
        __syncthreads();
    }
}

template <class T>
__global__ void __launch_bounds__(256) scan_add_kernel(T *out, const T *sums, uint64_t n) {
    const uint64_t base = (uint64_t)blockIdx.x * SCAN_TILE + (uint64_t)threadIdx.x * SCAN_ITEMS;
    const T add = sums[blockIdx.x];
// ... 250 lines not shown
}

__global__ void upload_params_kernel(SearchParams P, SearchParams *dst) {
    const uint32_t *src = (const uint32_t *)__builtin_amdgcn_kernarg_segment_ptr();
    uint32_t *d = (uint32_t *)dst;
    for (uint32_t t = threadIdx.x; t < (uint32_t)(sizeof(SearchParams) / 4u); t += blockDim.x) d[t] = src[t];
}


static void occ_latch(molar_hip_ctx *c) {
    const bool known = c->occ_valid && c->occ_key == occ_key_of(c->cur);
    c->cur.occ_use[0] = known ? c->occ_cells[0] : 0u;
    c->cur.occ_use[1] = known ? c->occ_cells[1] : 0u;
}
static void occ_note(molar_hip_ctx *c, unsigned long long key, unsigned long long packed) {
    if (!key || !(uint32_t)packed) return;
    c->occ_key = key;
    c->occ_cells[0] = (uint32_t)packed;
    c->occ_cells[1] = (uint32_t)(packed >> 32);
    c->occ_valid = true;
}

struct SearchCall {
    bool plan = true;
    bool within_set = false;
    bool hist_plan = false;
    bool size_masks = true;
    bool side = false;
    hipEvent_t side_wait = nullptr;
    unsigned long long out_cap = ~0ull;
    unsigned long long *sizes_dev = nullptr;
    bool drop_nonfinite = false;
    uint32_t slot_launch = 0;
};

struct OnSideStream {
    template <class T>
    struct Restore {
        T &ref;
        const T old;
        explicit Restore(T &r) : ref(r), old(r) {}
        ~Restore() { ref = old; }
        Restore(const Restore &) = delete;
    };
    Restore<hipStream_t> stream;
    Restore<bool> on_side;
    explicit OnSideStream(molar_hip_ctx *c) : stream(c->stream), on_side(c->on_side) {
        c->stream = c->side_stream;
        c->on_side = true;
    }
};

static int ensure_side_stream(molar_hip_ctx *c) {
    if (c->side_stream) return 0;
    int lo = 0, hi = 0;
    MH_HIP(hipDeviceGetStreamPriorityRange(&lo, &hi));
    MH_HIP(hipStreamCreateWithPriority(&c->side_stream, hipStreamNonBlocking, hi));
    MH_HIP(hipEventCreateWithFlags(&c->grid_done, hipEventDisableTiming));
    return 0;
}

static BinParams grid_bin_params(const SearchShape &shape, const GridSet &S, bool drop_nonfinite) {
    BinParams P{};
    P.xyz = S.d_xyz;
    P.idx = S.d_idx;
    P.n = S.n;
// ... 212 lines not shown
#endif
    }
    MH_TRY(c->params.reserve(sizeof(SearchParams)));
    const bool plan_wrote = c->params_fresh && !FILL && !hist.nbins && call.out_cap == c->params_fresh_cap;
    c->params_fresh = false;
    if (!params_resident && !plan_wrote && !P.hist_lean)
        hipLaunchKernelGGL(upload_params_kernel, dim3(1), dim3(256), 0, c->stream, P, c->params.as<SearchParams>());
    const SearchParams *dP = c->params.as<SearchParams>();
    const SlotDesc *tf = c->slot_desc.as<SlotDesc>();
    uint32_t st = (uint32_t)cur.nslots_bound;
    if (call.slot_launch && !hist.nbins && call.slot_launch < st) P.nblocks = st = call.slot_launch;
    uint32_t *sc = c->slot_cnt.as<uint32_t>();
    auto *sb = c->slot_base.as<unsigned long long>();
    const int mode = !FILL ? MODE_COUNT : (hist.nbins ? MODE_HIST : MODE_FILL);
    if (P.hist_lean) {
        if (!c->hist_queue.p) {
            MH_TRY(c->hist_queue.reserve(hist_queue_words() * 4));
            MH_HIP(hipMemsetAsync(c->hist_queue.p, 0, hist_queue_words() * 4, c->stream));
        }
        uint32_t *queue = c->hist_queue.as<uint32_t>();
        const int lslot = (int)(c->hist_frames++ & 3u);
        P.hist_nslots = hist_list_count(queue, lslot, 1);
        launch_hist_plan(cur.kind, c->stream, P, c->params.as<SearchParams>(), c->slot_desc.as<SlotDesc>(), c->slot_desc_rest.as<SlotDesc>(), queue, lslot);
        launch_hist_lean(cur.kind, (unsigned)c->num_cus, dyn_lds, c->stream, dP, tf, st, queue, lslot, P.hist_big != 0u);
        tf = c->slot_desc_rest.as<SlotDesc>();
    }
    if (const int family = (!hist.nbins && !out.ids) ? pair_family(cur) : 0) {
        if (family == -2) launch_pair_huge(cur.kind, mode, P.nblocks, c->stream, dP, tf, st, sc, sb, out.pairs, out.dist);
        else if (family == -1) launch_pair_wide(cur.kind, mode, P.nblocks, c->stream, dP, tf, st, sc, sb, out.pairs, out.dist);
        else launch_pair_small(mode, family, c->stream, dP, tf, st, sc, sb, out.pairs, out.dist);
        MH_HIP(hipGetLastError());
        return 0;
    }
    switch (cur.kind) {
        case MOLAR_HIP_SEARCH_SINGLE: launch_pair_single(mode, P.nblocks, dyn_lds, c->stream, dP, tf, st, sc, sb, out.pairs, out.dist, out.ids); break;
        case MOLAR_HIP_SEARCH_DOUBLE: launch_pair_double(mode, P.nblocks, dyn_lds, c->stream, dP, tf, st, sc, sb, out.pairs, out.dist, out.ids); break;
        case MOLAR_HIP_SEARCH_WITHIN: launch_pair_within(mode, P.nblocks, dyn_lds, c->stream, dP, tf, st, sc, sb, out.pairs, out.dist, out.ids); break;
        default: launch_pair_vdw(mode, P.nblocks, dyn_lds, c->stream, dP, tf, st, sc, sb, out.pairs, out.dist, out.ids); break;
    }
    MH_HIP(hipGetLastError());
    return 0;
}

bool histogram_edges(float hmin, float hmax, size_t nbins, float *edges) {
    if (!(hmax > hmin) || !std::isfinite(hmin) || !std::isfinite(hmax) || nbins == 0) return false;
    const float hn = (float)nbins, range = hmax - hmin;
    auto bin_of = [&](uint32_t bits) -> float {
        float x;
        std::memcpy(&x, &bits, 4);
        volatile float d = std::sqrt(x);
        volatile float t = d - hmin;
        volatile float u = hn * t;
        volatile float v = u / range;
        return std::floor(v);
    };
    for (size_t b = 0; b <= nbins; ++b) {
        uint32_t lo = 0u, hi = 0x7F800000u;
        if (bin_of(lo) >= (float)b) {
            hi = lo;
        } else {
            while (hi - lo > 1u) {
                const uint32_t mid = lo + (hi - lo) / 2u;
                if (bin_of(mid) >= (float)b) hi = mid;
                else lo = mid;
            }
        }
// ... 72 lines not shown
        c->task_moff.as<unsigned long long>(), cur.ntasks + 1, c->scan_state.as<unsigned long long>())));
    const unsigned nbs = (unsigned)((cur.ntasks + cur.nslots_bound + 1 + pbs - 1) / pbs);
    hipLaunchKernelGGL(slotmap_kernel, dim3(nbs), dim3(pbs), 0, c->stream, cur.ntasks, c->task_nb.as<uint32_t>(),
                       c->task_desc.as<TaskDesc>(), fast_kind ? c->task_moff.as<unsigned long long>() : nullptr,
                       c->slot_desc.as<SlotDesc>(), cur.nslots_bound, sizes_dev);
    MH_HIP(hipGetLastError());
    return 0;
}

int size_plan(molar_hip_ctx *c) {
    SearchShape &cur = c->cur;
    const bool fast_kind = records_hit_history(cur);
    if (!fast_kind && cur.nslots_bound <= 65536ull) return 0;
    MH_TRY(ensure_pinned(c, 64));
    unsigned long long *h = reinterpret_cast<unsigned long long *>(c->h_pinned);
    h[0] = h[1] = 0ull;
    if (fast_kind) MH_HIP(hipMemcpyAsync(&h[0], c->task_moff.as<unsigned long long>() + cur.ntasks, 8, hipMemcpyDeviceToHost, c->stream));
    MH_HIP(hipMemcpyAsync(&h[1], c->task_nb.as<uint32_t>() + cur.ntasks, 4, hipMemcpyDeviceToHost, c->stream));
    MH_HIP(hipStreamSynchronize(c->stream));
    if (fast_kind) {
        c->mask_units = h[0];
        MH_TRY(c->maskbuf.reserve((size_t)h[0] * 256u + 256u));
    }
    const uint64_t real = (uint32_t)h[1];
    if (real < cur.nslots_bound) cur.nslots_bound = real;
    return 0;
}

int prepare_search(molar_hip_ctx *c, const molar_hip_search_desc *q, const SearchCall &call) {
    if (!c || !q) return fail(MOLAR_HIP_ERR_INVALID_ARGUMENT, "search: null argument");
    if (q->kind < 0 || q->kind > 3) return fail(MOLAR_HIP_ERR_INVALID_ARGUMENT, "search: unknown kind %d", q->kind);
    MH_HIP(hipSetDevice(c->device));
    c->have_search = false;
    SearchShape &cur = c->cur;
    cur.kind = q->kind;
    const bool two = q->kind != MOLAR_HIP_SEARCH_SINGLE;
    const bool vdw = q->kind == MOLAR_HIP_SEARCH_DOUBLE_VDW;
    cur.use_box = q->box9 != nullptr;
    cur.pbc = q->pbc & 7u;
    if (cur.use_box) MH_TRY(molar_hip_box_from_matrix(q->box9, &cur.box));
    const bool may_hold = c->within_hold && q->kind == MOLAR_HIP_SEARCH_WITHIN && call.within_set;
    uint64_t fp = 0;
    if (may_hold && q->xyz1 && q->natoms1 && !is_device_ptr(q->xyz1)) {
        fp = 0xcbf29ce484222325ull;
        auto mix = [&](size_t atom) {
            uint32_t w[3];
            std::memcpy(w, q->xyz1 + 3 * atom, 12);
            for (int k = 0; k < 3; ++k) fp = (fp ^ w[k]) * 0x100000001b3ull;
        };
        const size_t n = q->natoms1, step = n > 512 ? n / 512 : 1;
        for (size_t a = 0; a < n && a < 64; ++a) mix(a);
        for (size_t a = 0; a < n; a += step) mix(a);
        for (size_t a = n > 64 ? n - 64 : 0; a < n; ++a) mix(a);
        fp |= 1ull;
    }
    bool reuse0 = may_hold && c->hold_valid && c->hold_fp == fp && c->hold_set == cur.set && c->hold_xyz == q->xyz1 && c->hold_natoms == q->natoms1 &&
                  c->hold_idx == q->idx1 && c->hold_n == q->n1 && c->hold_ids_local == q->ids_local && c->hold_use_box == cur.use_box &&
                  c->hold_pbc == cur.pbc && (!cur.use_box || std::memcmp(&c->hold_box, &cur.box, sizeof cur.box) == 0);
    if (!reuse0) {
        c->hold_valid = false;
        MH_TRY(stage_set(c, cur.set[0], q->xyz1, q->natoms1, q->idx1, q->n1, q->vdw1, vdw));
    }
    if (two) MH_TRY(stage_set(c, cur.set[1], q->xyz2, q->natoms2, q->idx2, q->n2, q->vdw2, vdw));
    else cur.set[1].n = 0;

    float cutoff = q->cutoff;
// ... 37 lines not shown
                cur.lower[d] = ord2f(mm[d]) + (-cutoff - F32_EPS);
                cur.upper[d] = ord2f(mm[3 + d]) + (cutoff + F32_EPS);
            }
        }
        for (int d = 0; d < 3; ++d) ext[d] = cur.upper[d] - cur.lower[d];
    }
    MH_TRY(dims_from_extents(cur, ext));
    if (reuse0) {
        bool same = c->hold_dims[0] == cur.dims[0] && c->hold_dims[1] == cur.dims[1] && c->hold_dims[2] == cur.dims[2];
        for (int d = 0; d < 3 && !cur.use_box; ++d) same = same && c->hold_lower[d] == cur.lower[d] && c->hold_upper[d] == cur.upper[d];
        if (!same) {
            reuse0 = false;
            c->hold_valid = false;
            MH_TRY(stage_set(c, cur.set[0], q->xyz1, q->natoms1, q->idx1, q->n1, q->vdw1, vdw));
        }
    }
    occ_latch(c);
    cur.ntasks = plan_entries(cur);
    cur.nslots_bound = slots_bound(cur, call.hist_plan);
    if (cur.ntasks >= 0xFFFFFFF0ull || cur.nslots_bound >= 0xFFFFFFF0ull || cur.ntasks + cur.nslots_bound >= 0xFFFFFF00ull)
        return fail(MOLAR_HIP_ERR_TOO_LARGE, "search plan too large (%llu entries)", (unsigned long long)cur.ntasks);
    MH_TRY(c->task_nb.reserve((cur.ntasks + 1) * 4));
    MH_TRY(c->task_desc.reserve((cur.ntasks + 1) * sizeof(TaskDesc)));
    MH_TRY(c->slot_desc.reserve((cur.nslots_bound + 1) * sizeof(SlotDesc)));
    if (call.hist_plan) MH_TRY(c->slot_desc_rest.reserve((cur.nslots_bound + 1) * sizeof(SlotDesc)));
    MH_TRY(c->slot_cnt.reserve((cur.nslots_bound + 1) * 4));
    MH_TRY(c->slot_base.reserve((cur.nslots_bound + 1) * 8));
    MH_TRY(c->params.reserve(sizeof(SearchParams)));
    const size_t st_tasks = lookback_state_words(cur.ntasks + 1), st_slots = lookback_state_words(cur.nslots_bound + 1);
    MH_TRY(c->scan_state.reserve((st_tasks + st_slots) * 8));
    MH_TRY(c->task_mu.reserve((cur.ntasks + 1) * 4));
    MH_TRY(c->task_moff.reserve((cur.ntasks + 1) * 8));
    const uint32_t fast_kind = records_hit_history(cur) ? 1u : 0u;
    auto enqueue_plan = [&]() -> int {
        Prof prof(c, 0);
        SearchParams P = make_params(c, cur);
        SearchParams *params_dst = nullptr;
        c->params_fresh = false;
        if (!call.size_masks) {
            P.out_cap = call.out_cap;
            params_dst = c->params.as<SearchParams>();
            c->params_fresh = true;
            c->params_fresh_cap = P.out_cap;
        }
        if (!c->on_side && cur.ntasks + 1 <= FPLAN_MAX_TASKS) {
            const uint32_t ntiles = (uint32_t)((cur.ntasks + 1 + 255) / 256);
            const uint32_t ngroups = ntiles > 1024u ? (ntiles + PLAN_GROUP - 1u) / PLAN_GROUP : 0u;
            MH_TRY(c->fplan_tiles.reserve((size_t)ntiles * 16 + (cur.ntasks + 1) * 8 + (size_t)ngroups * 16));
            unsigned long long *moff = fast_kind ? c->task_moff.as<unsigned long long>() : nullptr;
            unsigned long long *tt = c->fplan_tiles.as<unsigned long long>();
            unsigned long long *lmoff = tt + 2 * (size_t)ntiles;
            uint32_t *lfirst = c->task_mu.as<uint32_t>();
            if (cur.kind == MOLAR_HIP_SEARCH_SINGLE)
                hipLaunchKernelGGL((plan_tiles_kernel<MOLAR_HIP_SEARCH_SINGLE>), dim3(ntiles), dim3(256), 0, c->stream, P, lfirst,
                                   c->task_desc.as<TaskDesc>(), lmoff, fast_kind, c->slot_cnt.as<uint32_t>(), cur.nslots_bound + 1, tt, params_dst);
            else
                hipLaunchKernelGGL((plan_tiles_kernel<MOLAR_HIP_SEARCH_DOUBLE>), dim3(ntiles), dim3(256), 0, c->stream, P, lfirst,
                                   c->task_desc.as<TaskDesc>(), lmoff, fast_kind, c->slot_cnt.as<uint32_t>(), cur.nslots_bound + 1, tt, params_dst);
            unsigned long long *gt = ngroups ? lmoff + (cur.ntasks + 1) : nullptr;
            if (ngroups) hipLaunchKernelGGL(plan_groups_kernel, dim3(ngroups), dim3(64), 0, c->stream, ntiles, tt, gt);
            hipLaunchKernelGGL(plan_slots_kernel, dim3(ntiles * (256u / PLAN_SUB)), dim3(256), 0, c->stream, cur.ntasks, ntiles, lfirst, lmoff, c->task_nb.as<uint32_t>(),
                               c->task_desc.as<TaskDesc>(), moff, tt, c->slot_desc.as<SlotDesc>(), cur.nslots_bound, call.sizes_dev, gt);
            MH_HIP(hipGetLastError());
            return 0;
        }
        const uint64_t nplan = std::max<uint64_t>(std::max<uint64_t>(cur.ntasks + 1, cur.nslots_bound + 1), st_tasks + st_slots);
        const unsigned pbs = c->on_side ? 64u : 256u;
        const unsigned nb = (unsigned)((nplan + pbs - 1) / pbs);
        switch (cur.kind) {
            case MOLAR_HIP_SEARCH_SINGLE:
                hipLaunchKernelGGL((plan_kernel<MOLAR_HIP_SEARCH_SINGLE>), dim3(nb), dim3(pbs), 0, c->stream, P, c->task_nb.as<uint32_t>(), c->task_desc.as<TaskDesc>(),
                                   c->task_mu.as<uint32_t>(), fast_kind, c->slot_cnt.as<uint32_t>(), cur.nslots_bound + 1,
                                   c->scan_state.as<unsigned long long>(), (uint64_t)(st_tasks + st_slots), params_dst);
                break;
            default:
                hipLaunchKernelGGL((plan_kernel<MOLAR_HIP_SEARCH_DOUBLE>), dim3(nb), dim3(pbs), 0, c->stream, P, c->task_nb.as<uint32_t>(), c->task_desc.as<TaskDesc>(),
                                   c->task_mu.as<uint32_t>(), fast_kind, c->slot_cnt.as<uint32_t>(), cur.nslots_bound + 1,
                                   c->scan_state.as<unsigned long long>(), (uint64_t)(st_tasks + st_slots), params_dst);
                break;
        }
        MH_HIP(hipGetLastError());
        return enqueue_plan_slots(c, call.sizes_dev);
    };
    const bool side = call.side && c->own_stream && cur.use_box && !vdw && cur.set[0].d_xyz == q->xyz1 &&
                      cur.set[0].d_idx == q->idx1 && (!two || (cur.set[1].d_xyz == q->xyz2 && cur.set[1].d_idx == q->idx2));
    if (side) {
        MH_TRY(ensure_side_stream(c));
        if (call.side_wait) MH_HIP(hipStreamWaitEvent(c->side_stream, call.side_wait, 0));
        {
            OnSideStream on_side(c);
            if (!reuse0) MH_TRY(build_grid(c, call, cur.set[0], q->ids_local || vdw));
            if (two) MH_TRY(build_grid(c, call, cur.set[1], q->ids_local || vdw));
            MH_HIP(hipEventRecord(c->grid_done, c->side_stream));
        }
        if (c->env_host_grid_wait) MH_HIP(hipEventSynchronize(c->grid_done));
        else MH_HIP(hipStreamWaitEvent(c->stream, c->grid_done, 0));
    } else {
        if (!reuse0) MH_TRY(build_grid(c, call, cur.set[0], q->ids_local || vdw));
        if (two) MH_TRY(build_grid(c, call, cur.set[1], q->ids_local || vdw));
    }
    if (may_hold && !reuse0) {
        c->hold_valid = true;
        c->hold_fp = fp;
        c->hold_set = cur.set;
        c->hold_xyz = q->xyz1; c->hold_natoms = q->natoms1; c->hold_idx = q->idx1; c->hold_n = q->n1;
        c->hold_ids_local = q->ids_local; c->hold_use_box = cur.use_box; c->hold_pbc = cur.pbc; c->hold_box = cur.box;
        for (int d = 0; d < 3; ++d) { c->hold_dims[d] = cur.dims[d]; c->hold_lower[d] = cur.lower[d]; c->hold_upper[d] = cur.upper[d]; }
    }

    if (call.plan) MH_TRY(enqueue_plan());
    c->mask_units = 0;
    if (call.size_masks && call.plan) MH_TRY(size_plan(c));
    return 0;
}

int finish_count(molar_hip_ctx *c) {
    Prof *prof = new Prof(c, 2);
    void *sizes_dev = nullptr;
    if (ensure_pinned(c, 64) == 0 && hipHostGetDevicePointer(&sizes_dev, c->h_pinned, 0) == hipSuccess && sizes_dev) {
        std::memset(c->h_pinned, 0, 32);
    } else {
        (void)hipGetLastError();
        sizes_dev = nullptr;
    }
    int rc = scan_slot_counts(c, (unsigned long long *)sizes_dev);
    delete prof;
    MH_TRY(rc);
    unsigned long long tot = 0;
    if (sizes_dev) {
        MH_HIP(hipStreamSynchronize(c->stream));
        unsigned long long occ = 0;
        std::memcpy(&tot, c->h_pinned, 8);
// ... 174 lines not shown
}

extern "C" {

int molar_hip_search_count(molar_hip_ctx *c, const molar_hip_search_desc *q, uint64_t *out_count) {
    SearchCall call;
    MH_TRY(prepare_search(c, q, call));
    if (c->have_search) {
        if (out_count) *out_count = 0;
        return MOLAR_HIP_OK;
    }
    MH_TRY(launch_pairs<false>(c, call, PairOut{}));
    MH_TRY(finish_count(c));
    if (out_count) *out_count = c->total;
    return MOLAR_HIP_OK;
}

int molar_hip_search_grid_dims(molar_hip_ctx *c, uint64_t dims[3]) {
    if (!c || !c->have_search) return fail(MOLAR_HIP_ERR_NO_SEARCH, "no cached search: call molar_hip_search_count first");
    for (int d = 0; d < 3; ++d) dims[d] = c->cur.dims[d];
    return MOLAR_HIP_OK;
}

int molar_hip_search_cell_kernels(molar_hip_ctx *c, int32_t *lanes, uint64_t occupied_cells[2]) {
    if (!c || !lanes) return fail(MOLAR_HIP_ERR_INVALID_ARGUMENT, "search_cell_kernels: null argument");
    *lanes = pair_family(c->cur);
    if (occupied_cells) {
        occupied_cells[0] = c->cur.occ_use[0];
        occupied_cells[1] = c->cur.occ_use[1];
    }
    return MOLAR_HIP_OK;
}

static int fill_common(molar_hip_ctx *c, uint2 *d_pairs, float *d_dist, uint32_t *d_ids) {
    if (!c || !c->have_search) return fail(MOLAR_HIP_ERR_NO_SEARCH, "no cached search: call molar_hip_search_count first");
    MH_HIP(hipSetDevice(c->device));
    if (c->total == 0 || c->cur.ntasks == 0) return 0;
    uint2 *p = d_pairs;
    float *d = d_dist;
    const bool via_p = p && ((uintptr_t)p & 15u) != 0, via_d = d && ((uintptr_t)d & 7u) != 0;
    if (via_p) {
        MH_TRY(c->out_pairs.reserve((size_t)c->total * 8));
        p = c->out_pairs.as<uint2>();
    }
    if (via_d) {
        MH_TRY(c->out_dist.reserve((size_t)c->total * 4));
        d = c->out_dist.as<float>();
    }
    MH_TRY(launch_pairs<true>(c, SearchCall{}, PairOut{p, d, d_ids}));
    if (via_p) MH_HIP(hipMemcpyAsync(d_pairs, p, (size_t)c->total * 8, hipMemcpyDeviceToDevice, c->stream));
    if (via_d) MH_HIP(hipMemcpyAsync(d_dist, d, (size_t)c->total * 4, hipMemcpyDeviceToDevice, c->stream));
    return 0;
}

int molar_hip_search_fill(molar_hip_ctx *c, uint32_t *pairs, float *dist) {
    if (!c || !c->have_search) return fail(MOLAR_HIP_ERR_NO_SEARCH, "no cached search: call molar_hip_search_count first");
    if (c->cur.kind == MOLAR_HIP_SEARCH_WITHIN)
        return fail(MOLAR_HIP_ERR_INVALID_ARGUMENT, "within search yields ids: use molar_hip_search_fill_ids");
    const bool pd = is_device_ptr(pairs), dd = is_device_ptr(dist);
    uint2 *dp = nullptr;
    float *ddist = nullptr;
    if (pairs) {
        if (pd) dp = reinterpret_cast<uint2 *>(pairs);
        else {
            MH_TRY(c->out_pairs.reserve((size_t)(c->total ? c->total : 1) * 8));
            dp = c->out_pairs.as<uint2>();
// ... 739 lines not shown
    MH_TRY(s->ct_acc.reserve(words * 8));
    MH_HIP(hipMemsetAsync(s->ct_acc.p, 0, words * 8, s->stream));
    unsigned long long *w = s->ct_acc.as<unsigned long long>();
    K.t_count = w;
    w += 1;
    K.t_deg1 = reinterpret_cast<unsigned long long *>(deg1);
    K.t_deg2 = reinterpret_cast<unsigned long long *>(deg2);
    K.t_map = reinterpret_cast<unsigned long long *>(map);
    if (d1) { K.h_deg1 = deg1; K.t_deg1 = w; w += K.n1; }
    if (d2) { K.h_deg2 = deg2; K.t_deg2 = w; w += K.n2; }
    if (dm) { K.h_map = map; K.t_map = w; w += K.nmap; }
    if (occ && K.nmap) {
        MH_TRY(s->ct_frame.reserve(K.nmap * 4));
        MH_HIP(hipMemsetAsync(s->ct_frame.p, 0, K.nmap * 4, s->stream));
        K.t_frame = s->ct_frame.as<uint32_t>();
        K.t_occ = occ;
        if (!is_device_ptr(occ)) {
            MH_TRY(s->ct_occ.reserve(K.nmap * 4));
            MH_HIP(hipMemsetAsync(s->ct_occ.p, 0, K.nmap * 4, s->stream));
            K.h_occ = occ;
            K.t_occ = s->ct_occ.as<uint32_t>();
        }
    }
    return 0;
}

int contacts_frame(ContactCall &K, const molar_hip_search_desc *q) {
    if (K.n1 == 0 || (K.two && K.n2 == 0)) return 0;
    molar_hip_ctx *s = K.s;
    molar_hip_search_desc qq = *q;
    qq.ids_local = 1;
    SearchCall call;
    call.size_masks = false;
    MH_TRY(prepare_search(s, &qq, call));
    s->params_fresh = false;
    const SearchShape &cur = s->cur;
    if (cur.nslots_bound == 0) return 0;
    ContactArgs A{};
    A.g1 = K.g1;
    A.g2 = K.g2;
    A.ng2 = (uint32_t)K.ng2;
    A.deg1 = K.t_deg1;
    A.deg2 = K.two ? K.t_deg2 : K.t_deg1;
    A.map = K.t_frame ? nullptr : K.t_map;
    A.map32 = K.t_frame;
    if (!A.map && !A.map32) A.g1 = A.g2 = nullptr;
    A.count = K.t_count;
    {
        Prof prof(s, 3);
        launch_contacts(cur.kind, (unsigned)s->num_cus, s->stream, s->params.as<SearchParams>(), s->slot_desc.as<SlotDesc>(), (uint32_t)cur.nslots_bound, A);
        MH_HIP(hipGetLastError());
    }
    if (K.t_frame) {
        const unsigned nb = (unsigned)std::min<size_t>((K.nmap + 255) / 256, (size_t)s->num_cus * 16);
        hipLaunchKernelGGL(contact_fold_kernel, dim3(nb), dim3(256), 0, s->stream, K.t_frame, K.nmap, K.t_map, K.t_occ);
        MH_HIP(hipGetLastError());
    }
    return 0;
}

int contacts_end(ContactCall &K, uint64_t *out_count) {
    molar_hip_ctx *s = K.s;
    auto add_back = [&](uint64_t *dst, const unsigned long long *src, size_t n) -> int {
        if (!dst || n == 0) return 0;
        std::vector<unsigned long long> h(n);
        MH_TRY(read_back(s, h.data(), src, n * 8));
// ... 267 lines not shown
```

molar_amd/csrc/search_shape.hpp:

```cpp
#pragma once

#include <algorithm>
#include <cmath>

#include "common.hpp"

namespace mh {

inline bool fixed_cutoff_kind(int kind) { return kind == MOLAR_HIP_SEARCH_SINGLE || kind == MOLAR_HIP_SEARCH_DOUBLE; }

inline uint64_t grid_cells(const SearchShape &s) { return (uint64_t)s.dims[0] * s.dims[1] * s.dims[2]; }

inline int dims_from_extents(SearchShape &s, const float ext[3]) {
    double cells = 1.0;
    for (int d = 0; d < 3; ++d) {
        const float q = std::floor(ext[d] / s.cutoff);
        uint64_t n = (q > 0.0f) ? (q >= 4.0e9f ? 4000000000ull : (uint64_t)q) : 0ull;
        if (n < 1) n = 1;
        s.dims[d] = (uint32_t)n;
        cells *= (double)n;
    }
    if (cells > 1.0e8)
        return fail(MOLAR_HIP_ERR_TOO_LARGE, "search grid %u x %u x %u has too many cells (cutoff %g)", s.dims[0],
                    s.dims[1], s.dims[2], (double)s.cutoff);
// ... 19 lines not shown
    }
    return lanes;
}

inline int pair_family(const SearchShape &s) {
    if (const int lanes = small_cell_lanes(s)) return lanes;
    if (!fixed_cutoff_kind(s.kind)) return 0;
    const int b = s.kind == MOLAR_HIP_SEARCH_SINGLE ? 0 : 1;
    const uint64_t cells = judged_cells(s, b), n = s.set[b].n;
    return n > 1000ull * cells ? -2 : (n > 448ull * cells ? -1 : 0);
}

inline bool records_hit_history(const SearchShape &s) { return fixed_cutoff_kind(s.kind) && small_cell_lanes(s) == 0; }

inline bool sorted_by_device_sort(uint64_t n, uint64_t ncells) { return n > 384ull * ncells; }

inline unsigned long long occ_key_of(const SearchShape &s) {
    unsigned long long h = 1469598103934665603ull;
    auto mix = [&](unsigned long long v) { h = (h ^ v) * 1099511628211ull; };
    mix((unsigned long long)s.kind + 1u); mix(s.set[0].n); mix(s.kind == MOLAR_HIP_SEARCH_SINGLE ? 0u : s.set[1].n);
    mix(s.dims[0]); mix(s.dims[1]); mix(s.dims[2]); mix(s.use_box ? 1u : 2u);
    return h ? h : 1ull;
}

inline uint64_t plan_entries(const SearchShape &s) { return grid_cells(s) * 14ull * (s.kind != MOLAR_HIP_SEARCH_SINGLE ? 2ull : 1ull); }

inline uint64_t slots_bound(const SearchShape &s, bool hist_plan) {
    const uint64_t n0 = s.set[0].n;
    uint64_t bound = (s.kind != MOLAR_HIP_SEARCH_SINGLE ? 28ull : 14ull) * ((n0 + 63ull) / 64ull) + plan_entries(s) + 28ull * 512ull;
    if (hist_plan) bound += (n0 + 31ull) / 32ull + grid_cells(s);
    return bound;
}

struct WrapPolicy {
    uint32_t wrap_kind;
    uint32_t prune_wrapped;
    uint32_t approx_wrapped;
    float band_lo, band_hi;
    float prune_limit2;
};

inline WrapPolicy wrapped_pair_policy(const SearchShape &s) {
    WrapPolicy W{};
    const float cutoff2 = s.cutoff * s.cutoff;
    W.wrap_kind = 3u;
    if (s.use_box) {
        const float *m = s.box.m, *iv = s.box.inv;
        auto z = [&](int k) { return m[k] == 0.0f && iv[k] == 0.0f; };
        const bool lower_zero = z(1) && z(2) && z(5);
        const bool upper_zero = z(3) && z(6) && z(7);
        if (lower_zero && upper_zero) W.wrap_kind = 1u;
        else if (lower_zero) W.wrap_kind = 2u;
    }
    W.prune_wrapped = 0u;
    if (s.use_box) {
        bool ok = true;
        for (int d = 0; d < 3; ++d)
            if (((s.pbc >> d) & 1u) && s.dims[d] < 3u) ok = false;
        W.prune_wrapped = ok ? 1u : 0u;
    }
    W.approx_wrapped = 0u;
    W.band_lo = W.band_hi = cutoff2;
    float margin = 1.0e-3f;
    if (s.use_box) {
        bool ok = (uint64_t)s.set[0].n + (uint64_t)s.set[1].n < (1ull << 26);
        float ext[3], lmax = 0.f;
// ... 44 lines not shown
```

rust/molar_hip/src/ffi.rs:

```rust
#![allow(non_camel_case_types, clippy::too_many_arguments, clippy::missing_safety_doc)]

use std::os::raw::{c_char, c_int, c_void};

use crate::types::{
    MolarHipBox, MolarHipContactGroups, MolarHipCtx, MolarHipFitStream, MolarHipMembraneDesc, MolarHipMembraneOut, MolarHipMembranePatches, MolarHipMembranePlan, MolarHipMembraneState,
    MolarHipMembraneStateF64,
    MolarHipMembraneView, MolarHipSearchDesc, MolarHipSearchDescF64, MolarHipXtc,
};

pub struct MolarHipFns {
    pub create: unsafe extern "C" fn(c_int) -> *mut MolarHipCtx,
    pub destroy: unsafe extern "C" fn(*mut MolarHipCtx),
    pub last_error: unsafe extern "C" fn() -> *const c_char,
    pub version: unsafe extern "C" fn() -> *const c_char,
    pub device_count: unsafe extern "C" fn() -> c_int,
    pub set_stream: unsafe extern "C" fn(*mut MolarHipCtx, *mut c_void) -> c_int,
    pub synchronize: unsafe extern "C" fn(*mut MolarHipCtx) -> c_int,
    pub profile_enable: unsafe extern "C" fn(*mut MolarHipCtx, c_int) -> c_int,
    pub profile_read: unsafe extern "C" fn(*mut MolarHipCtx, *mut f32, *mut u64) -> c_int,
    pub copy_bandwidth: unsafe extern "C" fn(*mut MolarHipCtx, usize, c_int, *mut f32) -> c_int,
    pub write_bandwidth: unsafe extern "C" fn(*mut MolarHipCtx, usize, c_int, *mut f32) -> c_int,
    pub box_from_matrix: unsafe extern "C" fn(*const f32, *mut MolarHipBox) -> c_int,
    pub box_from_vectors_angles: unsafe extern "C" fn(f32, f32, f32, f32, f32, f32, *mut MolarHipBox) -> c_int,
    pub box_shortest_vector: unsafe extern "C" fn(*const MolarHipBox, *const f32, u8, *mut f32),
    pub box_lab_extents: unsafe extern "C" fn(*const MolarHipBox, *mut f32),
    pub box_extents: unsafe extern "C" fn(*const MolarHipBox, *mut f32),
    pub box_to_box_coords: unsafe extern "C" fn(*const MolarHipBox, *const f32, *mut f32),
    pub box_to_lab_coords: unsafe extern "C" fn(*const MolarHipBox, *const f32, *mut f32),
    pub box_is_inside: unsafe extern "C" fn(*const MolarHipBox, *const f32) -> c_int,
    pub box_wrap_point: unsafe extern "C" fn(*const MolarHipBox, *const f32, *mut f32),
    pub search_count: unsafe extern "C" fn(*mut MolarHipCtx, *const MolarHipSearchDesc, *mut u64) -> c_int,
    pub search_fill: unsafe extern "C" fn(*mut MolarHipCtx, *mut u32, *mut f32) -> c_int,
    pub search_fill_usize: unsafe extern "C" fn(*mut MolarHipCtx, *mut u64, *mut u64, *mut f32) -> c_int,
    pub search_fill_ids: unsafe extern "C" fn(*mut MolarHipCtx, *mut u64) -> c_int,
    pub within_count: unsafe extern "C" fn(*mut MolarHipCtx, *const MolarHipSearchDesc, *mut u64) -> c_int,
    pub within_fill: unsafe extern "C" fn(*mut MolarHipCtx, *mut u64) -> c_int,
    pub within_hold: unsafe extern "C" fn(*mut MolarHipCtx, c_int) -> c_int,
    pub search_connectivity: unsafe extern "C" fn(*mut MolarHipCtx, *const MolarHipSearchDesc, *mut u64, *mut u64) -> c_int,
    pub search_connectivity_fill: unsafe extern "C" fn(*mut MolarHipCtx, *mut u64, *mut u64) -> c_int,
    pub unwrap_connectivity: unsafe extern "C" fn(*mut MolarHipCtx, *mut f32, usize, *const u64, usize, *const f32, f32, u8, *mut u64, *mut u64, *mut usize) -> c_int,
    pub search_grid_dims: unsafe extern "C" fn(*mut MolarHipCtx, *mut u64) -> c_int,
    pub search_cell_kernels: unsafe extern "C" fn(*mut MolarHipCtx, *mut i32, *mut u64) -> c_int,
    pub search_fill_device: unsafe extern "C" fn(*mut MolarHipCtx, *mut *const u32, *mut *const f32) -> c_int,
    pub search_resident: unsafe extern "C" fn(*mut MolarHipCtx, *const MolarHipSearchDesc, *mut u64, *mut *const u32, *mut *const f32) -> c_int,
    pub search_resident_planes: unsafe extern "C" fn(*mut MolarHipCtx, c_int) -> c_int,
    pub search_resident_begin: unsafe extern "C" fn(*mut MolarHipCtx, *const MolarHipSearchDesc, *mut i32) -> c_int,
    pub search_resident_end: unsafe extern "C" fn(*mut MolarHipCtx, i32, *mut u64, *mut *const u32, *mut *const f32) -> c_int,
    pub search_histogram: unsafe extern "C" fn(*mut MolarHipCtx, *const MolarHipSearchDesc, f32, f32, usize, *mut u64, *mut u64) -> c_int,
    pub search_histogram_frames: unsafe extern "C" fn(*mut MolarHipCtx, *const MolarHipSearchDesc, usize, usize, usize, *const f32, f32, f32, usize, *mut u64) -> c_int,
    pub histogram_edges: unsafe extern "C" fn(f32, f32, usize, *mut f32) -> c_int,
    pub search_contacts: unsafe extern "C" fn(*mut MolarHipCtx, *const MolarHipSearchDesc, *const MolarHipContactGroups, *mut u64, *mut u64, *mut u64, *mut u64) -> c_int,
    pub search_contacts_frames: unsafe extern "C" fn(*mut MolarHipCtx, *const MolarHipSearchDesc, *const MolarHipContactGroups, usize, usize, usize, *const f32, *mut u64, *mut u64, *mut u64, *mut u32) -> c_int,
    pub search_count_f64: unsafe extern "C" fn(*mut MolarHipCtx, *const MolarHipSearchDescF64, *mut u64) -> c_int,
    pub search_fill_f64: unsafe extern "C" fn(*mut MolarHipCtx, *mut u64, *mut u64, *mut f64) -> c_int,
    pub search_fill_ids_f64: unsafe extern "C" fn(*mut MolarHipCtx, *mut u64) -> c_int,
    pub search_grid_dims_f64: unsafe extern "C" fn(*mut MolarHipCtx, *mut u64) -> c_int,
    pub search_histogram_f64: unsafe extern "C" fn(*mut MolarHipCtx, *const MolarHipSearchDescF64, f64, f64, usize, *mut u64, *mut u64) -> c_int,
    pub search_histogram_frames_f64: unsafe extern "C" fn(*mut MolarHipCtx, *const MolarHipSearchDescF64, usize, usize, usize, *const f64, f64, f64, usize, *mut u64) -> c_int,
    pub histogram_edges_f64: unsafe extern "C" fn(f64, f64, usize, *mut f64) -> c_int,
    pub within_count_f64: unsafe extern "C" fn(*mut MolarHipCtx, *const MolarHipSearchDescF64, *mut u64) -> c_int,
    pub within_fill_f64: unsafe extern "C" fn(*mut MolarHipCtx, *mut u64) -> c_int,
    pub search_connectivity_f64: unsafe extern "C" fn(*mut MolarHipCtx, *const MolarHipSearchDescF64, *mut u64, *mut u64) -> c_int,
    pub unwrap_connectivity_f64: unsafe extern "C" fn(*mut MolarHipCtx, *mut f64, usize, *const u64, usize, *const f64, f64, u8, *mut u64, *mut u64, *mut usize) -> c_int,
    pub min_max: unsafe extern "C" fn(*mut MolarHipCtx, *const f32, usize, *const u64, usize, *mut f32, *mut f32) -> c_int,
    pub center_of_geometry: unsafe extern "C" fn(*mut MolarHipCtx, *const f32, usize, *const u64, usize, *mut f32) -> c_int,
    pub center_of_mass: unsafe extern "C" fn(*mut MolarHipCtx, *const f32, usize, *const u64, usize, *const f32, *mut f32) -> c_int,
    pub center_of_geometry_pbc: unsafe extern "C" fn(*mut MolarHipCtx, *const f32, usize, *const u64, usize, *const f32, u8, *mut f32) -> c_int,
    pub center_of_mass_pbc: unsafe extern "C" fn(*mut MolarHipCtx, *const f32, usize, *const u64, usize, *const f32, *const f32, u8, *mut f32) -> c_int,
    pub gyration: unsafe extern "C" fn(*mut MolarHipCtx, *const f32, usize, *const u64, usize, *const f32, *const f32, *mut f32) -> c_int,
    pub inertia: unsafe extern "C" fn(*mut MolarHipCtx, *const f32, usize, *const u64, usize, *const f32, *const f32, *mut f32, *mut f32, *mut f32) -> c_int,
    pub rmsd: unsafe extern "C" fn(*mut MolarHipCtx, *const f32, usize, *const u64, usize, *const f32, usize, *const u64, usize, *mut f32) -> c_int,
    pub rmsd_mw: unsafe extern "C" fn(*mut MolarHipCtx, *const f32, usize, *const u64, usize, *const f32, *const f32, usize, *const u64, usize, *mut f32) -> c_int,
    pub fit_transform: unsafe extern "C" fn(*mut MolarHipCtx, *const f32, usize, *const u64, usize, *const f32, *const f32, usize, *const u64, usize, *const f32, c_int, *mut f32, *mut f32) -> c_int,
    pub center_of_geometry_f64: unsafe extern "C" fn(*mut MolarHipCtx, *const f64, usize, *const u64, usize, *mut f64) -> c_int,
    pub center_of_mass_f64: unsafe extern "C" fn(*mut MolarHipCtx, *const f64, usize, *const u64, usize, *const f64, *mut f64) -> c_int,
// ... 85 lines not shown
            Ok(MolarHipFns {
                create: *lib.get::<unsafe extern "C" fn(c_int) -> *mut MolarHipCtx>(b"molar_hip_create\0")?,
                destroy: *lib.get::<unsafe extern "C" fn(*mut MolarHipCtx)>(b"molar_hip_destroy\0")?,
                last_error: *lib.get::<unsafe extern "C" fn() -> *const c_char>(b"molar_hip_last_error\0")?,
                version: *lib.get::<unsafe extern "C" fn() -> *const c_char>(b"molar_hip_version\0")?,
                device_count: *lib.get::<unsafe extern "C" fn() -> c_int>(b"molar_hip_device_count\0")?,
                set_stream: *lib.get::<unsafe extern "C" fn(*mut MolarHipCtx, *mut c_void) -> c_int>(b"molar_hip_set_stream\0")?,
                synchronize: *lib.get::<unsafe extern "C" fn(*mut MolarHipCtx) -> c_int>(b"molar_hip_synchronize\0")?,
                profile_enable: *lib.get::<unsafe extern "C" fn(*mut MolarHipCtx, c_int) -> c_int>(b"molar_hip_profile_enable\0")?,
                profile_read: *lib.get::<unsafe extern "C" fn(*mut MolarHipCtx, *mut f32, *mut u64) -> c_int>(b"molar_hip_profile_read\0")?,
                copy_bandwidth: *lib.get::<unsafe extern "C" fn(*mut MolarHipCtx, usize, c_int, *mut f32) -> c_int>(b"molar_hip_copy_bandwidth\0")?,
                write_bandwidth: *lib.get::<unsafe extern "C" fn(*mut MolarHipCtx, usize, c_int, *mut f32) -> c_int>(b"molar_hip_write_bandwidth\0")?,
                box_from_matrix: *lib.get::<unsafe extern "C" fn(*const f32, *mut MolarHipBox) -> c_int>(b"molar_hip_box_from_matrix\0")?,
                box_from_vectors_angles: *lib.get::<unsafe extern "C" fn(f32, f32, f32, f32, f32, f32, *mut MolarHipBox) -> c_int>(b"molar_hip_box_from_vectors_angles\0")?,
                box_shortest_vector: *lib.get::<unsafe extern "C" fn(*const MolarHipBox, *const f32, u8, *mut f32)>(b"molar_hip_box_shortest_vector\0")?,
                box_lab_extents: *lib.get::<unsafe extern "C" fn(*const MolarHipBox, *mut f32)>(b"molar_hip_box_lab_extents\0")?,
                box_extents: *lib.get::<unsafe extern "C" fn(*const MolarHipBox, *mut f32)>(b"molar_hip_box_extents\0")?,
                box_to_box_coords: *lib.get::<unsafe extern "C" fn(*const MolarHipBox, *const f32, *mut f32)>(b"molar_hip_box_to_box_coords\0")?,
                box_to_lab_coords: *lib.get::<unsafe extern "C" fn(*const MolarHipBox, *const f32, *mut f32)>(b"molar_hip_box_to_lab_coords\0")?,
                box_is_inside: *lib.get::<unsafe extern "C" fn(*const MolarHipBox, *const f32) -> c_int>(b"molar_hip_box_is_inside\0")?,
                box_wrap_point: *lib.get::<unsafe extern "C" fn(*const MolarHipBox, *const f32, *mut f32)>(b"molar_hip_box_wrap_point\0")?,
                search_count: *lib.get::<unsafe extern "C" fn(*mut MolarHipCtx, *const MolarHipSearchDesc, *mut u64) -> c_int>(b"molar_hip_search_count\0")?,
                search_fill: *lib.get::<unsafe extern "C" fn(*mut MolarHipCtx, *mut u32, *mut f32) -> c_int>(b"molar_hip_search_fill\0")?,
                search_fill_usize: *lib.get::<unsafe extern "C" fn(*mut MolarHipCtx, *mut u64, *mut u64, *mut f32) -> c_int>(b"molar_hip_search_fill_usize\0")?,
                search_fill_ids: *lib.get::<unsafe extern "C" fn(*mut MolarHipCtx, *mut u64) -> c_int>(b"molar_hip_search_fill_ids\0")?,
                within_count: *lib.get::<unsafe extern "C" fn(*mut MolarHipCtx, *const MolarHipSearchDesc, *mut u64) -> c_int>(b"molar_hip_within_count\0")?,
                within_fill: *lib.get::<unsafe extern "C" fn(*mut MolarHipCtx, *mut u64) -> c_int>(b"molar_hip_within_fill\0")?,
                within_hold: *lib.get::<unsafe extern "C" fn(*mut MolarHipCtx, c_int) -> c_int>(b"molar_hip_within_hold\0")?,
                search_connectivity: *lib.get::<unsafe extern "C" fn(*mut MolarHipCtx, *const MolarHipSearchDesc, *mut u64, *mut u64) -> c_int>(b"molar_hip_search_connectivity\0")?,
                search_connectivity_fill: *lib.get::<unsafe extern "C" fn(*mut MolarHipCtx, *mut u64, *mut u64) -> c_int>(b"molar_hip_search_connectivity_fill\0")?,
                unwrap_connectivity: *lib.get::<unsafe extern "C" fn(*mut MolarHipCtx, *mut f32, usize, *const u64, usize, *const f32, f32, u8, *mut u64, *mut u64, *mut usize) -> c_int>(b"molar_hip_unwrap_connectivity\0")?,
                search_grid_dims: *lib.get::<unsafe extern "C" fn(*mut MolarHipCtx, *mut u64) -> c_int>(b"molar_hip_search_grid_dims\0")?,
                search_cell_kernels: *lib.get::<unsafe extern "C" fn(*mut MolarHipCtx, *mut i32, *mut u64) -> c_int>(b"molar_hip_search_cell_kernels\0")?,
                search_fill_device: *lib.get::<unsafe extern "C" fn(*mut MolarHipCtx, *mut *const u32, *mut *const f32) -> c_int>(b"molar_hip_search_fill_device\0")?,
                search_resident: *lib.get::<unsafe extern "C" fn(*mut MolarHipCtx, *const MolarHipSearchDesc, *mut u64, *mut *const u32, *mut *const f32) -> c_int>(b"molar_hip_search_resident\0")?,
                search_resident_planes: *lib.get::<unsafe extern "C" fn(*mut MolarHipCtx, c_int) -> c_int>(b"molar_hip_search_resident_planes\0")?,
                search_resident_begin: *lib.get::<unsafe extern "C" fn(*mut MolarHipCtx, *const MolarHipSearchDesc, *mut i32) -> c_int>(b"molar_hip_search_resident_begin\0")?,
                search_resident_end: *lib.get::<unsafe extern "C" fn(*mut MolarHipCtx, i32, *mut u64, *mut *const u32, *mut *const f32) -> c_int>(b"molar_hip_search_resident_end\0")?,
                search_histogram: *lib.get::<unsafe extern "C" fn(*mut MolarHipCtx, *const MolarHipSearchDesc, f32, f32, usize, *mut u64, *mut u64) -> c_int>(b"molar_hip_search_histogram\0")?,
                search_histogram_frames: *lib.get::<unsafe extern "C" fn(*mut MolarHipCtx, *const MolarHipSearchDesc, usize, usize, usize, *const f32, f32, f32, usize, *mut u64) -> c_int>(b"molar_hip_search_histogram_frames\0")?,
                histogram_edges: *lib.get::<unsafe extern "C" fn(f32, f32, usize, *mut f32) -> c_int>(b"molar_hip_histogram_edges\0")?,
                search_contacts: *lib.get::<unsafe extern "C" fn(*mut MolarHipCtx, *const MolarHipSearchDesc, *const MolarHipContactGroups, *mut u64, *mut u64, *mut u64, *mut u64) -> c_int>(b"molar_hip_search_contacts\0")?,
                search_contacts_frames: *lib.get::<unsafe extern "C" fn(*mut MolarHipCtx, *const MolarHipSearchDesc, *const MolarHipContactGroups, usize, usize, usize, *const f32, *mut u64, *mut u64, *mut u64, *mut u32) -> c_int>(b"molar_hip_search_contacts_frames\0")?,
                search_count_f64: *lib.get::<unsafe extern "C" fn(*mut MolarHipCtx, *const MolarHipSearchDescF64, *mut u64) -> c_int>(b"molar_hip_search_count_f64\0")?,
                search_fill_f64: *lib.get::<unsafe extern "C" fn(*mut MolarHipCtx, *mut u64, *mut u64, *mut f64) -> c_int>(b"molar_hip_search_fill_f64\0")?,
                search_fill_ids_f64: *lib.get::<unsafe extern "C" fn(*mut MolarHipCtx, *mut u64) -> c_int>(b"molar_hip_search_fill_ids_f64\0")?,
                search_grid_dims_f64: *lib.get::<unsafe extern "C" fn(*mut MolarHipCtx, *mut u64) -> c_int>(b"molar_hip_search_grid_dims_f64\0")?,
                search_histogram_f64: *lib.get::<unsafe extern "C" fn(*mut MolarHipCtx, *const MolarHipSearchDescF64, f64, f64, usize, *mut u64, *mut u64) -> c_int>(b"molar_hip_search_histogram_f64\0")?,
                search_histogram_frames_f64: *lib.get::<unsafe extern "C" fn(*mut MolarHipCtx, *const MolarHipSearchDescF64, usize, usize, usize, *const f64, f64, f64, usize, *mut u64) -> c_int>(b"molar_hip_search_histogram_frames_f64\0")?,
                histogram_edges_f64: *lib.get::<unsafe extern "C" fn(f64, f64, usize, *mut f64) -> c_int>(b"molar_hip_histogram_edges_f64\0")?,
                within_count_f64: *lib.get::<unsafe extern "C" fn(*mut MolarHipCtx, *const MolarHipSearchDescF64, *mut u64) -> c_int>(b"molar_hip_within_count_f64\0")?,
                within_fill_f64: *lib.get::<unsafe extern "C" fn(*mut MolarHipCtx, *mut u64) -> c_int>(b"molar_hip_within_fill_f64\0")?,
                search_connectivity_f64: *lib.get::<unsafe extern "C" fn(*mut MolarHipCtx, *const MolarHipSearchDescF64, *mut u64, *mut u64) -> c_int>(b"molar_hip_search_connectivity_f64\0")?,
                unwrap_connectivity_f64: *lib.get::<unsafe extern "C" fn(*mut MolarHipCtx, *mut f64, usize, *const u64, usize, *const f64, f64, u8, *mut u64, *mut u64, *mut usize) -> c_int>(b"molar_hip_unwrap_connectivity_f64\0")?,
                min_max: *lib.get::<unsafe extern "C" fn(*mut MolarHipCtx, *const f32, usize, *const u64, usize, *mut f32, *mut f32) -> c_int>(b"molar_hip_min_max\0")?,
                center_of_geometry: *lib.get::<unsafe extern "C" fn(*mut MolarHipCtx, *const f32, usize, *const u64, usize, *mut f32) -> c_int>(b"molar_hip_center_of_geometry\0")?,
                center_of_mass: *lib.get::<unsafe extern "C" fn(*mut MolarHipCtx, *const f32, usize, *const u64, usize, *const f32, *mut f32) -> c_int>(b"molar_hip_center_of_mass\0")?,
                center_of_geometry_pbc: *lib.get::<unsafe extern "C" fn(*mut MolarHipCtx, *const f32, usize, *const u64, usize, *const f32, u8, *mut f32) -> c_int>(b"molar_hip_center_of_geometry_pbc\0")?,
                center_of_mass_pbc: *lib.get::<unsafe extern "C" fn(*mut MolarHipCtx, *const f32, usize, *const u64, usize, *const f32, *const f32, u8, *mut f32) -> c_int>(b"molar_hip_center_of_mass_pbc\0")?,
                gyration: *lib.get::<unsafe extern "C" fn(*mut MolarHipCtx, *const f32, usize, *const u64, usize, *const f32, *const f32, *mut f32) -> c_int>(b"molar_hip_gyration\0")?,
                inertia: *lib.get::<unsafe extern "C" fn(*mut MolarHipCtx, *const f32, usize, *const u64, usize, *const f32, *const f32, *mut f32, *mut f32, *mut f32) -> c_int>(b"molar_hip_inertia\0")?,
                rmsd: *lib.get::<unsafe extern "C" fn(*mut MolarHipCtx, *const f32, usize, *const u64, usize, *const f32, usize, *const u64, usize, *mut f32) -> c_int>(b"molar_hip_rmsd\0")?,
                rmsd_mw: *lib.get::<unsafe extern "C" fn(*mut MolarHipCtx, *const f32, usize, *const u64, usize, *const f32, *const f32, usize, *const u64, usize, *mut f32) -> c_int>(b"molar_hip_rmsd_mw\0")?,
                fit_transform: *lib.get::<unsafe extern "C" fn(*mut MolarHipCtx, *const f32, usize, *const u64, usize, *const f32, *const f32, usize, *const u64, usize, *const f32, c_int, *mut f32, *mut f32) -> c_int>(b"molar_hip_fit_transform\0")?,
                center_of_geometry_f64: *lib.get::<unsafe extern "C" fn(*mut MolarHipCtx, *const f64, usize, *const u64, usize, *mut f64) -> c_int>(b"molar_hip_center_of_geometry_f64\0")?,
                center_of_mass_f64: *lib.get::<unsafe extern "C" fn(*mut MolarHipCtx, *const f64, usize, *const u64, usize, *const f64, *mut f64) -> c_int>(b"molar_hip_center_of_mass_f64\0")?,
// ... 52 lines not shown
                membrane_frame_fetch: *lib.get::<unsafe extern "C" fn(*mut MolarHipMembranePlan, i32, *const MolarHipMembraneOut) -> c_int>(b"molar_hip_membrane_frame_fetch\0")?,
                membrane_frame_end_fetch: *lib.get::<unsafe extern "C" fn(*mut MolarHipMembranePlan, i32, *mut MolarHipMembraneView, *const MolarHipMembraneOut) -> c_int>(b"molar_hip_membrane_frame_end_fetch\0")?,
                lipid_tail_order: *lib.get::<unsafe extern "C" fn(*mut MolarHipCtx, *const f32, usize, *const u64, *const u64, usize, c_int, *const f32, *const u64, *const u8, *mut f32) -> c_int>(b"molar_hip_lipid_tail_order\0")?,
                xtc_open: *lib.get::<unsafe extern "C" fn(*const c_char) -> *mut MolarHipXtc>(b"molar_hip_xtc_open\0")?,
                xtc_open_memory: *lib.get::<unsafe extern "C" fn(*const c_void, usize) -> *mut MolarHipXtc>(b"molar_hip_xtc_open_memory\0")?,
                xtc_close: *lib.get::<unsafe extern "C" fn(*mut MolarHipXtc)>(b"molar_hip_xtc_close\0")?,
                xtc_nframes: *lib.get::<unsafe extern "C" fn(*const MolarHipXtc) -> usize>(b"molar_hip_xtc_nframes\0")?,
                xtc_natoms: *lib.get::<unsafe extern "C" fn(*const MolarHipXtc) -> usize>(b"molar_hip_xtc_natoms\0")?,
                xtc_frame_info: *lib.get::<unsafe extern "C" fn(*const MolarHipXtc, usize, *mut i32, *mut i32, *mut f32, *mut f32, *mut f32) -> c_int>(b"molar_hip_xtc_frame_info\0")?,
                xtc_seek_time: *lib.get::<unsafe extern "C" fn(*const MolarHipXtc, f32, *mut usize) -> c_int>(b"molar_hip_xtc_seek_time\0")?,
                xtc_read: *lib.get::<unsafe extern "C" fn(*mut MolarHipCtx, *const MolarHipXtc, usize, usize, *mut f32, c_int) -> c_int>(b"molar_hip_xtc_read\0")?,
                xtc_read_device: *lib.get::<unsafe extern "C" fn(*mut MolarHipCtx, *const MolarHipXtc, usize, usize, *mut f32) -> c_int>(b"molar_hip_xtc_read_device\0")?,
                xtc_histogram: *lib.get::<unsafe extern "C" fn(*mut MolarHipCtx, *const MolarHipXtc, usize, usize, *const u64, usize, f32, u8, f32, f32, usize, *mut u64, c_int) -> c_int>(b"molar_hip_xtc_histogram\0")?,
                xtc_histogram_double: *lib.get::<unsafe extern "C" fn(*mut MolarHipCtx, *const MolarHipXtc, usize, usize, *const u64, usize, *const u64, usize, f32, u8, f32, f32, usize, *mut u64, c_int) -> c_int>(b"molar_hip_xtc_histogram_double\0")?,
                xtc_encode_frame: *lib.get::<unsafe extern "C" fn(*const f32, usize, *const f32, i32, f32, f32, *mut u8, usize, *mut usize) -> c_int>(b"molar_hip_xtc_encode_frame\0")?,
                apply_transform: *lib.get::<unsafe extern "C" fn(*mut MolarHipCtx, *mut f32, usize, *const u64, usize, *const f32, *const f32) -> c_int>(b"molar_hip_apply_transform\0")?,
                unwrap_simple: *lib.get::<unsafe extern "C" fn(*mut MolarHipCtx, *mut f32, usize, *const u64, usize, *const f32, u8) -> c_int>(b"molar_hip_unwrap_simple\0")?,
                fit_rmsd_batch: *lib.get::<unsafe extern "C" fn(*mut MolarHipCtx, *mut f32, usize, usize, *const u64, usize, *const f32, *const f32, usize, *const u64, c_int, *mut f32, *mut f32, *mut f32, *mut f32, *mut f32) -> c_int>(b"molar_hip_fit_rmsd_batch\0")?,
                fit_stream_create: *lib.get::<unsafe extern "C" fn(*mut MolarHipCtx, usize, *const u64, usize, *const f32, *const f32, usize, *const u64, c_int, *mut *mut MolarHipFitStream) -> c_int>(b"molar_hip_fit_stream_create\0")?,
                fit_stream_begin: *lib.get::<unsafe extern "C" fn(*mut MolarHipFitStream, *mut f32, c_int, *mut i32) -> c_int>(b"molar_hip_fit_stream_begin\0")?,
                fit_stream_end: *lib.get::<unsafe extern "C" fn(*mut MolarHipFitStream, i32, *mut f32, *mut f32, *mut f32, *mut f32, *mut f32) -> c_int>(b"molar_hip_fit_stream_end\0")?,
                fit_stream_destroy: *lib.get::<unsafe extern "C" fn(*mut MolarHipFitStream)>(b"molar_hip_fit_stream_destroy\0")?,
                gyration_batch: *lib.get::<unsafe extern "C" fn(*mut MolarHipCtx, *const f32, usize, *const u64, *const u64, usize, *const f32, *const f32, *mut f32) -> c_int>(b"molar_hip_gyration_batch\0")?,
                rmsd_batch: *lib.get::<unsafe extern "C" fn(*mut MolarHipCtx, *const f32, usize, *const u64, *const f32, usize, *const u64, *const u64, usize, *const f32, *mut f32) -> c_int>(b"molar_hip_rmsd_batch\0")?,
                fit_batch: *lib.get::<unsafe extern "C" fn(*mut MolarHipCtx, *mut f32, usize, *const u64, *const f32, *const f32, usize, *const u64, *const f32, *const u64, usize, c_int, *mut f32, *mut f32, *mut f32, *mut f32, *mut f32) -> c_int>(b"molar_hip_fit_batch\0")?,
                translate: *lib.get::<unsafe extern "C" fn(*mut MolarHipCtx, *mut f32, usize, *const u64, usize, *const f32) -> c_int>(b"molar_hip_translate\0")?,
                rotate: *lib.get::<unsafe extern "C" fn(*mut MolarHipCtx, *mut f32, usize, *const u64, usize, *const f32, f32) -> c_int>(b"molar_hip_rotate\0")?,
                principal_transform: *lib.get::<unsafe extern "C" fn(*mut MolarHipCtx, *const f32, usize, *const u64, usize, *const f32, *const f32, *mut f32, *mut f32) -> c_int>(b"molar_hip_principal_transform\0")?,
            })
        }
    }
}

pub const ENTRY_POINTS: usize = 145;
```

Before: 736.5 frames/s.

## Plan pair slots over live rows only, skipping AABB-pruned rows

Adds a live_rows pre-pass that, per task, builds bitmasks of rows that can reach the neighbour cell's bounding box. The slot planner then packs only those live rows into slots, and new LIVE instances of the single/double pair kernels use the mask to gather rows instead of walking contiguous rows and re-running the AABB test. The goal is fewer idle lanes and fewer wasted slots in the count and fill passes for dense boxes. In exchange it adds an extra kernel, mask storage, a gather load per lane and more kernel instantiations, plus a slot-statistics query entry point.

```diff
diff --git a/include/molar_hip.h b/include/molar_hip.h
--- a/include/molar_hip.h
+++ b/include/molar_hip.h
@@ -110,6 +110,7 @@
                                   uint64_t *group_ids, size_t *ngroups);
 int molar_hip_search_grid_dims(molar_hip_ctx *ctx, uint64_t dims[3]);
 int molar_hip_search_cell_kernels(molar_hip_ctx *ctx, int32_t *lanes, uint64_t occupied_cells[2]);
+int molar_hip_search_slot_counts(molar_hip_ctx *ctx, uint64_t *slots, uint64_t *consecutive_slots);
 int molar_hip_search_fill_device(molar_hip_ctx *ctx, const uint32_t **d_pairs, const float **d_dist);
 int molar_hip_search_resident(molar_hip_ctx *ctx, const molar_hip_search_desc *desc, uint64_t *out_count,
                               const uint32_t **d_pairs, const float **d_dist);
diff --git a/molar_amd/_lib.py b/molar_amd/_lib.py
--- a/molar_amd/_lib.py
+++ b/molar_amd/_lib.py
@@ -104,6 +104,7 @@
     "molar_hip_within_hold": (_I, [_P, _I]),
     "molar_hip_search_grid_dims": (_I, [_P, _P]),
     "molar_hip_search_cell_kernels": (_I, [_P, _P, _P]),
+    "molar_hip_search_slot_counts": (_I, [_P, _P, _P]),
     "molar_hip_search_count_f64": (_I, [_P, _P, _P]),
     "molar_hip_search_fill_f64": (_I, [_P, _P, _P, _P]),
     "molar_hip_search_fill_ids_f64": (_I, [_P, _P]),
diff --git a/molar_amd/api.py b/molar_amd/api.py
--- a/molar_amd/api.py
+++ b/molar_amd/api.py
@@ -270,6 +270,11 @@
         occ = (C.c_uint64 * 2)()
         check(self.lib.molar_hip_search_cell_kernels(self.ctx, C.byref(lanes), occ))
         return int(lanes.value), (int(occ[0]), int(occ[1]))
+
+    def search_slot_counts(self):
+        slots, rows = C.c_uint64(0), C.c_uint64(0)
+        check(self.lib.molar_hip_search_slot_counts(self.ctx, C.byref(slots), C.byref(rows)))
+        return int(slots.value), int(rows.value)
 
     def search_resident_planes(self, want_dist=True):
         check(self.lib.molar_hip_search_resident_planes(self.ctx, 1 if want_dist else 0))
diff --git a/molar_amd/build.py b/molar_amd/build.py
--- a/molar_amd/build.py
+++ b/molar_amd/build.py
@@ -8,7 +8,7 @@
 HERE = os.path.dirname(os.path.abspath(__file__))
 CSRC = os.path.join(HERE, "csrc")
 LIB = os.path.join(HERE, "libmolar_hip.so")
-SOURCES = ["api.hip", "search.hip", "search_f64.hip", "measure.hip", "measure_f64.hip", "membrane.hip", "xtc.hip", "pair_k0.hip", "pair_k1.hip", "pair_k2.hip", "pair_k3.hip", "pair_k4.hip", "pair_k5.hip", "pair_k6.hip", "pair_k7.hip", "pair_k8.hip", "pair_k9.hip", "pair_small.hip", "devsort.hip", "sasa.hip", "rmsd_matrix.hip", "fluct.hip", "msd.hip"]
+SOURCES = ["api.hip", "search.hip", "search_f64.hip", "measure.hip", "measure_f64.hip", "membrane.hip", "xtc.hip", "pair_k0.hip", "pair_k1.hip", "pair_k2.hip", "pair_k3.hip", "pair_k4.hip", "pair_k5.hip", "pair_k6.hip", "pair_k7.hip", "pair_k8.hip", "pair_k9.hip", "pair_k10.hip", "pair_k11.hip", "pair_small.hip", "devsort.hip", "sasa.hip", "rmsd_matrix.hip", "fluct.hip", "msd.hip"]
 HEADERS = ["common.hpp", "boxmath.hpp", "linalg3.hpp", "pair_kernels.hpp", "hist_kernels.hpp", "contact_kernels.hpp", "hoststream.hpp", "stages.hpp", "csr_kernels.hpp", "unwrap_walk.hpp", "search_shape.hpp", os.path.join("..", "..", "include", "molar_hip.h")]
 FLAGS = ["--offload-arch=gfx950", "-O3", "-std=c++17", "-fPIC", "-ffp-contract=off", "-fno-fast-math",
          "-Wall", "-Wno-unused-function",
diff --git a/molar_amd/csrc/api.hip b/molar_amd/csrc/api.hip
--- a/molar_amd/csrc/api.hip
+++ b/molar_amd/csrc/api.hip
@@ -177,7 +177,7 @@
     if (c->side_stream) (void)hipStreamSynchronize(c->side_stream);
     for (auto &gen : c->set_store) for (auto &s : gen) {
         for (DevBuf *b : {&s.xyz_stage, &s.idx_stage, &s.vdw_stage, &s.key, &s.cell_count, &s.cnt_pad, &s.cursor, &s.tmp_key, &s.sort_buf,
-                          &s.sorted, &s.sorted_vdw, &s.aabb, &s.perm, &s.chunk_aabb, &s.h16, &s.cell_org})
+                          &s.sorted, &s.sorted_vdw, &s.aabb, &s.perm, &s.chunk_aabb, &s.h16, &s.cell_org, &s.live})
             b->release();
     }
     if (c->aux) molar_hip_destroy(c->aux);
@@ -188,14 +188,14 @@
     for (DevBuf *b : {&c->xh_win[0], &c->xh_win[1], &c->xh_bins, &c->fit_redo, &c->ct_g1, &c->ct_g2, &c->ct_acc, &c->ct_frame, &c->ct_occ}) b->release();
     for (auto &gen : c->hb_sets) for (auto &fr : gen) for (auto &s : fr) {
         for (DevBuf *b : {&s.xyz_stage, &s.idx_stage, &s.vdw_stage, &s.key, &s.cell_count, &s.cnt_pad, &s.cursor, &s.tmp_key, &s.sort_buf,
-                          &s.sorted, &s.sorted_vdw, &s.aabb, &s.perm, &s.chunk_aabb, &s.h16, &s.cell_org})
+                          &s.sorted, &s.sorted_vdw, &s.aabb, &s.perm, &s.chunk_aabb, &s.h16, &s.cell_org, &s.live})
             b->release();
     }
     for (DevBuf *b : {&c->hb_lean[0], &c->hb_lean[1], &c->hb_rest[0], &c->hb_rest[1], &c->hb_blocks[0], &c->hb_blocks[1]}) b->release();
     if (c->hb_pin) (void)hipHostFree(c->hb_pin);
     for (auto e : c->hb_pin_ev)
         if (e) (void)hipEventDestroy(e);
-    for (DevBuf *b : {&c->params, &c->task_desc, &c->task_nb, &c->slot_desc, &c->slot_cnt, &c->slot_base, &c->tile_sum, &c->scan_tmp, &c->sort_tmp, &c->sort_tmp_side, &c->scan_tmp_side, &c->scan_state, &c->fplan_tiles, &c->out_pairs_set[0], &c->out_dist_set[0], &c->out_pairs_set[1], &c->out_dist_set[1], &c->out_ids,
+    for (DevBuf *b : {&c->params, &c->task_desc, &c->task_nb, &c->slot_desc, &c->slot_cnt, &c->slot_base, &c->tile_sum, &c->scan_tmp, &c->sort_tmp, &c->sort_tmp_side, &c->scan_tmp_side, &c->scan_state, &c->fplan_tiles, &c->slot_stat, &c->out_pairs_set[0], &c->out_dist_set[0], &c->out_pairs_set[1], &c->out_dist_set[1], &c->out_ids,
                       &c->wide_i, &c->wide_j, &c->hist, &c->hist_queue, &c->slot_desc_rest, &c->hist_edges, &c->dbg, &c->conn_deg, &c->conn_off, &c->conn_ent, &c->conn_neigh, &c->w_flags, &c->w_list, &c->w_part_cnt, &c->w_part, &c->w_tile_cnt, &c->w_tile_off, &c->task_mu, &c->task_moff, &c->maskbuf, &c->m_xyz1, &c->m_xyz2, &c->m_idx1, &c->m_idx2,
                       &c->m_mass1, &c->m_mass2, &c->m_partials, &c->m_results, &c->m_out})
         b->release();
diff --git a/molar_amd/csrc/common.hpp b/molar_amd/csrc/common.hpp
--- a/molar_amd/csrc/common.hpp
+++ b/molar_amd/csrc/common.hpp
@@ -107,6 +107,7 @@
     DevBuf chunk_aabb;
     DevBuf h16;
     DevBuf cell_org;
+    DevBuf live;
 };
 
 struct SearchShape {
@@ -183,6 +184,9 @@
     mh::DevBuf sort_tmp, sort_tmp_side;
     mh::DevBuf scan_state;
     mh::DevBuf fplan_tiles;
+    mh::DevBuf slot_stat;
+    bool slot_stat_valid = false;
+    bool plan_live = false;
     mh::DevBuf out_pairs_set[2];
     mh::DevBuf out_dist_set[2];
     mh::DevBuf &out_pairs = out_pairs_set[0];
diff --git a/molar_amd/csrc/pair_k10.hip b/molar_amd/csrc/pair_k10.hip
--- /dev/null
+++ b/molar_amd/csrc/pair_k10.hip
@@ -0,0 +1,16 @@
+#include "pair_kernels.hpp"
+
+namespace mh {
+
+void launch_pair_single_live(int mode, unsigned nblocks, hipStream_t stream, const pairk::SearchParams *dP,
+                             const pairk::SlotDesc *slot_desc, uint32_t nslots, uint32_t *slot_cnt,
+                             const unsigned long long *slot_base, uint2 *pairs, float *dist) {
+    using namespace pairk;
+    constexpr int KIND = MOLAR_HIP_SEARCH_SINGLE;
+    if (mode == MODE_COUNT)
+        launch_pair_kernel<KIND, MODE_COUNT, 0, true>(nblocks, 0, stream, dP, slot_desc, nslots, slot_cnt, slot_base, pairs, dist, nullptr);
+    else
+        launch_pair_kernel<KIND, MODE_FILL, 0, true>(nblocks, 0, stream, dP, slot_desc, nslots, slot_cnt, slot_base, pairs, dist, nullptr);
+}
+
+}
diff --git a/molar_amd/csrc/pair_k11.hip b/molar_amd/csrc/pair_k11.hip
--- /dev/null
+++ b/molar_amd/csrc/pair_k11.hip
@@ -0,0 +1,16 @@
+#include "pair_kernels.hpp"
+
+namespace mh {
+
+void launch_pair_double_live(int mode, unsigned nblocks, hipStream_t stream, const pairk::SearchParams *dP,
+                             const pairk::SlotDesc *slot_desc, uint32_t nslots, uint32_t *slot_cnt,
+                             const unsigned long long *slot_base, uint2 *pairs, float *dist) {
+    using namespace pairk;
+    constexpr int KIND = MOLAR_HIP_SEARCH_DOUBLE;
+    if (mode == MODE_COUNT)
+        launch_pair_kernel<KIND, MODE_COUNT, 0, true>(nblocks, 0, stream, dP, slot_desc, nslots, slot_cnt, slot_base, pairs, dist, nullptr);
+    else
+        launch_pair_kernel<KIND, MODE_FILL, 0, true>(nblocks, 0, stream, dP, slot_desc, nslots, slot_cnt, slot_base, pairs, dist, nullptr);
+}
+
+}
diff --git a/molar_amd/csrc/pair_kernels.hpp b/molar_amd/csrc/pair_kernels.hpp
--- a/molar_amd/csrc/pair_kernels.hpp
+++ b/molar_amd/csrc/pair_kernels.hpp
@@ -20,6 +20,8 @@
 constexpr int waves_per_block(int mode) { return mode == MODE_HIST ? 4 : MH_WPB; }
 constexpr int KREG = 8;
 constexpr int FIFO_CAP = 128;
+constexpr int LIVE_GROUPS = KREG;
+constexpr uint32_t SLOT_LIVE = 0x400u;
 #ifndef MOLAR_HIP_NO_WIDE_FLUSH
 #define MOLAR_HIP_WIDE_FLUSH 1
 #endif
@@ -123,6 +125,13 @@
     bool valid;
 };
 
+struct SlotTask : Task {
+    bool live = false;
+    uint32_t lrow = 0;
+};
+
+__device__ __forceinline__ uint32_t slot_row(const SlotTask &T, uint32_t i0, uint32_t lane) { return T.live ? T.lrow : i0 + lane; }
+
 template <int KIND, bool UNIFORM>
 __device__ __forceinline__ Task decode_task(const SearchParams &P, uint64_t t) {
     Task T;
@@ -603,12 +612,12 @@
 }
 
 template <int KIND, int NCH, bool TRI>
-__device__ __forceinline__ uint32_t run_count_sorted(const SearchParams &P, const Task &T, uint32_t i0, float4 *la,
+__device__ __forceinline__ uint32_t run_count_sorted(const SearchParams &P, const SlotTask &T, uint32_t i0, float4 *la,
                                                      uint32_t lane) {
     const float cutoff2 = P.cutoff2;
     const uint32_t rows = __builtin_amdgcn_readfirstlane(T.n1 - i0 < T.rps ? T.n1 - i0 : T.rps);
     float4 a = make_float4(0.f, 0.f, 0.f, 0.f);
-    if (lane < rows) a = gload4(P.sa, T.a0 + i0 + lane);
+    if (lane < rows) a = gload4(P.sa, T.a0 + slot_row(T, i0, lane));
     la[lane] = a;
     float bx[NCH], by[NCH], bz[NCH];
     uint32_t bpos[NCH];
@@ -670,7 +679,7 @@
 }
 
 template <int KIND, bool TRI>
-__device__ __forceinline__ uint32_t run_count_mfma(const SearchParams &P, const Task &T, uint32_t i0, float4 *la, uint4 *lh,
+__device__ __forceinline__ uint32_t run_count_mfma(const SearchParams &P, const SlotTask &T, uint32_t i0, float4 *la, uint4 *lh,
                                                    uint32_t lane, bool &done) {
     typedef uint32_t u4_t __attribute__((ext_vector_type(4)));
     typedef __attribute__((address_space(3))) u4_t lds_u4;
@@ -681,10 +690,10 @@
     const uint32_t kh = lane >> 5, cl = lane & 31u;
     const uint32_t nct = (T.n2 + 31u) >> 5;
     float4 a = make_float4(0.f, 0.f, 0.f, 0.f);
-    if (lane < rows) a = gload4(P.sa, T.a0 + i0 + lane);
+    if (lane < rows) a = gload4(P.sa, T.a0 + slot_row(T, i0, lane));
     const float4 org = gload4(P.cell_org_b, T.cb);
     bool need = lane < rows;
-    if (!TRI) {
+    if (!TRI && !T.live) {
         const float4 blo = gload4(P.aabb_b, 2 * T.cb), bhi = gload4(P.aabb_b, 2 * T.cb + 1);
         need = need && !(aabb_d2(a.x, a.y, a.z, blo.x, blo.y, blo.z, bhi.x, bhi.y, bhi.z) > cutoff2);
     }
@@ -804,7 +813,7 @@
 }
 
 template <int KIND>
-__device__ __forceinline__ bool run_count_mfma_wrapped(const SearchParams &P, const Task &T, uint32_t i0, float4 *la, uint4 *lh,
+__device__ __forceinline__ bool run_count_mfma_wrapped(const SearchParams &P, const SlotTask &T, uint32_t i0, float4 *la, uint4 *lh,
                                                        uint32_t lane, uint32_t *mwords, uint32_t &count_out) {
     typedef uint32_t u4_t __attribute__((ext_vector_type(4)));
     typedef __attribute__((address_space(3))) u4_t lds_u4;
@@ -823,10 +832,13 @@
         Sz += sgn * P.box.m[3 * d + 2];
     }
     float4 a = make_float4(0.f, 0.f, 0.f, 0.f);
-    if (lane < rows) a = gload4(P.sa, T.a0 + i0 + lane);
+    if (lane < rows) a = gload4(P.sa, T.a0 + slot_row(T, i0, lane));
     const float4 org = gload4(P.cell_org_b, T.cb);
-    const float4 blo = gload4(P.aabb_b, 2 * T.cb), bhi = gload4(P.aabb_b, 2 * T.cb + 1);
-    const bool need = lane < rows && !(aabb_d2(a.x - Sx, a.y - Sy, a.z - Sz, blo.x, blo.y, blo.z, bhi.x, bhi.y, bhi.z) > P.prune_limit2);
+    bool need = lane < rows;
+    if (!T.live) {
+        const float4 blo = gload4(P.aabb_b, 2 * T.cb), bhi = gload4(P.aabb_b, 2 * T.cb + 1);
+        need = need && !(aabb_d2(a.x - Sx, a.y - Sy, a.z - Sz, blo.x, blo.y, blo.z, bhi.x, bhi.y, bhi.z) > P.prune_limit2);
+    }
     const unsigned long long live = __builtin_amdgcn_ballot_w64(need);
     const uint32_t nlive = (uint32_t)__popcll(live);
     if (nlive == 0u) {
@@ -962,7 +974,7 @@
 }
 
 template <int KIND, bool FILL, bool WRAPPED, int NCH, bool TRI, bool MASKED>
-__device__ __forceinline__ uint32_t run_fast(const SearchParams &P, const Task &T, uint32_t i0, Fifo &F, float4 *la,
+__device__ __forceinline__ uint32_t run_fast(const SearchParams &P, const SlotTask &T, uint32_t i0, Fifo &F, float4 *la,
                                              uint32_t lane, uint32_t *mwords) {
     static_assert(!(WRAPPED && TRI), "a triangular (same-cell) entry never wraps on the fast path");
     if constexpr (!FILL && !WRAPPED && MASKED_COUNT_SORTED) return run_count_sorted<KIND, NCH, TRI>(P, T, i0, la, lane);
@@ -998,11 +1010,15 @@
     unsigned long long live;
     {
         float4 a = make_float4(0.f, 0.f, 0.f, 0.f);
-        if (lane < rows) a = gload4(P.sa, T.a0 + i0 + lane);
+        if (lane < rows) a = gload4(P.sa, T.a0 + slot_row(T, i0, lane));
         la[lane] = a;
-        const float4 lo = gload4(P.aabb_b, 2 * T.cb), hi = gload4(P.aabb_b, 2 * T.cb + 1);
+        float4 lo = make_float4(0.f, 0.f, 0.f, 0.f), hi = lo;
+        if (!T.live) {
+            lo = gload4(P.aabb_b, 2 * T.cb);
+            hi = gload4(P.aabb_b, 2 * T.cb + 1);
+        }
         bool need = true;
-        if (TRI) {
+        if (TRI || T.live) {
         } else if (!WRAPPED) {
             need = !(aabb_d2(a.x, a.y, a.z, lo.x, lo.y, lo.z, hi.x, hi.y, hi.z) > cutoff2);
         } else if (approx) {
@@ -1212,7 +1228,7 @@
 constexpr int KMAX_WIDE = 16;
 constexpr int KMAX_HUGE = 32;
 template <int KIND, bool FILL, int WK, bool MASKED, int KMAX = KREG>
-__device__ __forceinline__ uint32_t run_task_nch(const SearchParams &P, const Task &T, uint32_t i0, Fifo &F, float4 *la,
+__device__ __forceinline__ uint32_t run_task_nch(const SearchParams &P, const SlotTask &T, uint32_t i0, Fifo &F, float4 *la,
                                                  uint32_t lane, uint32_t *mwords) {
     const uint32_t nchunks = (T.n2 + 63u) >> 6;
     if constexpr (KMAX > KMAX_WIDE) {
@@ -1384,7 +1400,7 @@
     return P.approx_wrapped != 0u && !(P.box.nshift != 0 && wrap == MOLAR_HIP_PBC_FULL);
 }
 
-template <int KIND, int MODE, int WPE = 0>
+template <int KIND, int MODE, int WPE = 0, bool LIVE = false>
 __global__ void __launch_bounds__(64 * waves_per_block(MODE))
 __attribute__((amdgpu_waves_per_eu(WPE ? WPE : (MODE == MODE_HIST ? 4 : (MODE == MODE_COUNT ? MH_COUNT_WPE : MH_FILL_WPE))))) pair_kernel(const SearchParams *__restrict__ Pp,
                                                      const SlotDesc *__restrict__ slot_desc,
@@ -1400,6 +1416,9 @@
     __shared__ float4 lds_a[WAVES_PER_BLOCK][64];
     __shared__ uint4 lds_h[MODE == MODE_COUNT ? WAVES_PER_BLOCK : 1][MODE == MODE_COUNT ? 128 : 1];
     constexpr bool FILL = MODE != MODE_COUNT;
+    static_assert(!LIVE || (WPE == 0 && MODE != MODE_HIST && (KIND == MOLAR_HIP_SEARCH_SINGLE || KIND == MOLAR_HIP_SEARCH_DOUBLE)),
+                  "live-ranked slots: regular count / fill instances of the fixed-cutoff kinds");
+    constexpr bool LIVE_SLOTS = LIVE;
     extern __shared__ uint32_t lds_hist[];
     const SearchParams &P0 = *Pp;
 #ifdef MH_SLOT_LOOP
@@ -1428,7 +1447,7 @@
             if (w < full) wr = ((q / XCD_RUN) * 8u + x) * XCD_RUN + (q % XCD_RUN);
         }
         const uint32_t slot = nslots - 1u - wr;
-        Task T;
+        SlotTask T;
         uint32_t i0;
         unsigned long long moff;
         uint32_t frame = 0u;
@@ -1451,6 +1470,34 @@
             T.valid = true;
             T.wrap_b = (fl >> 12) & 7u;
             T.rps = fl >> 16;
+            if constexpr (LIVE_SLOTS) {
+                if (fl & SLOT_LIVE) {
+                    typedef __attribute__((address_space(1))) unsigned long long glb_u64;
+                    const uint2 mp = reinterpret_cast<const uint2 *>(slot_desc + slot)[5];
+                    const glb_u64 *mk = (const glb_u64 *)(((unsigned long long)(uint32_t)__builtin_amdgcn_readfirstlane(mp.y) << 32) |
+                                                          (unsigned long long)(uint32_t)__builtin_amdgcn_readfirstlane(mp.x));
+                    unsigned long long mw = 0ull;
+                    if (lane < (uint32_t)LIVE_GROUPS) mw = mk[lane];
+                    uint32_t *scr = lds[wave][0];
+                    uint32_t before = 0u;
+#pragma unroll
+                    for (int g = 0; g < LIVE_GROUPS; ++g) {
+                        const uint32_t wlo = __builtin_amdgcn_readlane((uint32_t)mw, g), whi = __builtin_amdgcn_readlane((uint32_t)(mw >> 32), g);
+                        const uint32_t n = (uint32_t)__popc(wlo) + (uint32_t)__popc(whi);
+                        if (n != 0u && before + n > i0 && before < i0 + 64u) {
+                            const uint32_t rank = before + __builtin_amdgcn_mbcnt_hi(whi, __builtin_amdgcn_mbcnt_lo(wlo, 0u)) - i0;
+                            const bool bit = (((lane < 32u ? wlo : whi) >> (lane & 31u)) & 1u) != 0u;
+                            if (bit && rank < 64u) scr[rank] = 64u * (uint32_t)g + lane;
+                        }
+                        before += n;
+                    }
+                    __builtin_amdgcn_wave_barrier();
+                    T.lrow = scr[lane];
+                    __builtin_amdgcn_wave_barrier();
+                    T.live = true;
+                    T.n1 = before;
+                }
+            }
         }
         const SearchParams &P = MODE == MODE_HIST ? Pp[frame] : P0;
         Fifo F;
@@ -1542,7 +1589,7 @@
     return dim3(gx, (nblocks + gx - 1u) / gx);
 }
 
-template <int KIND, int MODE, int WPE = 0>
+template <int KIND, int MODE, int WPE = 0, bool LIVE = false>
 inline void launch_pair_kernel(unsigned nblocks, size_t dyn_lds, hipStream_t stream, const SearchParams *dP,
                                const SlotDesc *slot_desc, uint32_t nslots, uint32_t *slot_cnt,
                                const unsigned long long *slot_base, uint2 *pairs, float *dist, uint32_t *ids) {
@@ -1550,7 +1597,7 @@
 #ifdef MH_SLOT_LOOP
     if (MODE != MODE_HIST) nblocks = (nblocks + (unsigned)MH_SLOT_LOOP - 1u) / (unsigned)MH_SLOT_LOOP;
 #endif
-    hipLaunchKernelGGL((pair_kernel<KIND, MODE, WPE>), pair_grid(nblocks), dim3(64 * waves_per_block(MODE)), dyn_lds, stream, dP, slot_desc, nslots,
+    hipLaunchKernelGGL((pair_kernel<KIND, MODE, WPE, LIVE>), pair_grid(nblocks), dim3(64 * waves_per_block(MODE)), dyn_lds, stream, dP, slot_desc, nslots,
                        slot_cnt, slot_base, pairs, dist, ids);
 }
 
@@ -1576,6 +1623,12 @@
 void launch_pair_double(int mode, unsigned nblocks, size_t dyn_lds, hipStream_t stream, const pairk::SearchParams *dP,
                         const pairk::SlotDesc *slot_desc, uint32_t nslots, uint32_t *slot_cnt,
                         const unsigned long long *slot_base, uint2 *pairs, float *dist, uint32_t *ids);
+void launch_pair_single_live(int mode, unsigned nblocks, hipStream_t stream, const pairk::SearchParams *dP,
+                             const pairk::SlotDesc *slot_desc, uint32_t nslots, uint32_t *slot_cnt,
+                             const unsigned long long *slot_base, uint2 *pairs, float *dist);
+void launch_pair_double_live(int mode, unsigned nblocks, hipStream_t stream, const pairk::SearchParams *dP,
+                             const pairk::SlotDesc *slot_desc, uint32_t nslots, uint32_t *slot_cnt,
+                             const unsigned long long *slot_base, uint2 *pairs, float *dist);
 void launch_pair_within(int mode, unsigned nblocks, size_t dyn_lds, hipStream_t stream, const pairk::SearchParams *dP,
                         const pairk::SlotDesc *slot_desc, uint32_t nslots, uint32_t *slot_cnt,
                         const unsigned long long *slot_base, uint2 *pairs, float *dist, uint32_t *ids);
diff --git a/molar_amd/csrc/search.hip b/molar_amd/csrc/search.hip
--- a/molar_amd/csrc/search.hip
+++ b/molar_amd/csrc/search.hip
@@ -510,7 +510,6 @@
 }
 
 constexpr unsigned long long LB_MASK = (1ull << 62) - 1ull;
-constexpr uint64_t FPLAN_MAX_TASKS = 1ull << 22;
 constexpr uint32_t PLAN_GROUP = 128;
 __device__ __forceinline__ unsigned long long lb_resolve(unsigned long long *desc, uint32_t tile, unsigned long long tot) {
     if (tile == 0) {
@@ -584,11 +583,59 @@
     return 0;
 }
 
+constexpr uint32_t LIVE_NONE = 0xFFFFFFFFu;
+static_assert(LIVE_ROW_GROUPS == (uint32_t)LIVE_GROUPS, "the host sizes the masks the kernels index");
+template <int KIND>
+__global__ void __launch_bounds__(64) live_rows_kernel(SearchParams P, unsigned long long *__restrict__ masks, uint32_t *__restrict__ live_cnt) {
+    const uint64_t t = (uint64_t)blockIdx.y * gridDim.x + blockIdx.x;
+    if (t >= P.ntasks) return;
+    const uint32_t lane = threadIdx.x;
+    const Task T = decode_task<KIND, true>(P, t);
+    const bool wrapped = P.use_box && T.wrap != 0u;
+    const bool approx = wrapped && P.approx_wrapped != 0u && !(P.box.nshift != 0 && T.wrap == MOLAR_HIP_PBC_FULL);
+    if (!T.valid || T.tri || T.rps != 64u || T.n1 > 64u * (uint32_t)LIVE_GROUPS || T.n2 > 64u * (uint32_t)KREG || (wrapped && !approx)) {
+        if (lane == 0) live_cnt[t] = LIVE_NONE;
+        return;
+    }
+    float Sx = 0.f, Sy = 0.f, Sz = 0.f;
+    float limit2 = P.cutoff2;
+    if (approx) {
+#pragma unroll
+        for (int d = 0; d < 3; ++d) {
+            if (!((T.wrap >> d) & 1u)) continue;
+            const float sgn = ((T.wrap_b >> d) & 1u) ? 1.0f : -1.0f;
+            Sx += sgn * P.box.m[3 * d];
+            Sy += sgn * P.box.m[3 * d + 1];
+            Sz += sgn * P.box.m[3 * d + 2];
+        }
+        limit2 = P.prune_limit2;
+    }
+    const float4 lo = gload4(P.aabb_b, 2 * T.cb), hi = gload4(P.aabb_b, 2 * T.cb + 1);
+    unsigned long long mine = 0ull;
+    uint32_t nlive = 0u;
+#pragma unroll
+    for (int g = 0; g < LIVE_GROUPS; ++g) {
+        const uint32_t row = 64u * (uint32_t)g + lane;
+        if (64u * (uint32_t)g >= T.n1) break;
+        bool need = false;
+        if (row < T.n1) {
+            const float4 a = gload4(P.sa, T.a0 + row);
+            need = !(aabb_d2(a.x - Sx, a.y - Sy, a.z - Sz, lo.x, lo.y, lo.z, hi.x, hi.y, hi.z) > limit2);
+        }
+        const unsigned long long m = __builtin_amdgcn_ballot_w64(need);
+        if (lane == (uint32_t)g) mine = m;
+        nlive += (uint32_t)__popcll(m);
+    }
+    if (lane < (uint32_t)LIVE_GROUPS) masks[t * (uint64_t)LIVE_GROUPS + lane] = mine;
+    if (lane == 0) live_cnt[t] = nlive;
+}
+
 template <int KIND>
 __global__ void __launch_bounds__(256) plan_tiles_kernel(SearchParams P, uint32_t *__restrict__ local_first, TaskDesc *__restrict__ task_desc,
                                                          unsigned long long *__restrict__ local_moff, uint32_t fast_kind,
                                                          uint32_t *__restrict__ slot_cnt, uint64_t nslot_cnt,
-                                                         unsigned long long *__restrict__ tile_tot, SearchParams *__restrict__ params_dst) {
+                                                         unsigned long long *__restrict__ tile_tot, SearchParams *__restrict__ params_dst,
+                                                         const uint32_t *__restrict__ live_cnt) {
     const uint64_t t = (uint64_t)blockIdx.x * 256u + threadIdx.x;
     for (uint64_t w = t; w < nslot_cnt; w += (uint64_t)gridDim.x * 256u) slot_cnt[w] = 0u;
     if (params_dst && blockIdx.x == 0) {
@@ -596,22 +643,25 @@
         uint32_t *d = (uint32_t *)params_dst;
         for (uint32_t w = threadIdx.x; w < (uint32_t)(sizeof(SearchParams) / 4u); w += 256u) d[w] = src[w];
     }
-    uint32_t nb = 0;
+    uint32_t nb = 0, nb_rows = 0;
     unsigned long long mu = 0;
     if (t < P.ntasks) {
         const Task T = decode_task<KIND, false>(P, t);
-        nb = T.valid ? (T.n1 + T.rps - 1u) / T.rps : 0u;
+        nb = nb_rows = T.valid ? (T.n1 + T.rps - 1u) / T.rps : 0u;
+        const uint32_t lc = (live_cnt && T.valid) ? live_cnt[t] : LIVE_NONE;
+        if (lc != LIVE_NONE) nb = (lc + 63u) >> 6;
         const uint32_t nch = (T.n2 + 63u) >> 6;
         mu = (fast_kind && P.use_box && T.wrap != 0u && nch <= (uint32_t)KREG) ? (unsigned long long)nb * 2u * nch : 0ull;
         TaskDesc d;
         d.a0 = T.a0; d.n1 = T.n1; d.b0 = T.b0; d.n2 = T.n2; d.cb = T.cb;
-        d.flags = T.wrap | (T.tri ? 0x100u : 0u) | (T.valid ? 0x200u : 0u) | (T.wrap_b << 12) | (T.rps << 16);
+        d.flags = T.wrap | (T.tri ? 0x100u : 0u) | (T.valid ? 0x200u : 0u) | (lc != LIVE_NONE ? SLOT_LIVE : 0u) | (T.wrap_b << 12) | (T.rps << 16);
         d.pad0 = nb;
         d.pad1 = 0u;
         task_desc[t] = d;
     }
-    uint32_t tot_nb;
+    uint32_t tot_nb, tot_rows;
     const uint32_t first = block_exclusive_scan<uint32_t>(nb, &tot_nb);
+    (void)block_exclusive_scan<uint32_t>(nb_rows, &tot_rows);
     unsigned long long tot_mu = 0ull, m0 = 0ull;
     if (fast_kind) m0 = block_exclusive_scan<unsigned long long>(mu, &tot_mu);
     if (t <= P.ntasks) {
@@ -619,7 +669,7 @@
         if (fast_kind) local_moff[t] = m0;
     }
     if (threadIdx.x == 0) {
-        tile_tot[2 * blockIdx.x] = tot_nb;
+        tile_tot[2 * blockIdx.x] = (unsigned long long)tot_nb | ((unsigned long long)tot_rows << 32);
         tile_tot[2 * blockIdx.x + 1] = tot_mu;
     }
 }
@@ -646,7 +696,9 @@
                                                                 const unsigned long long *__restrict__ tile_tot,
                                                                 SlotDesc *__restrict__ slot_desc, uint64_t nslots_bound,
                                                                 unsigned long long *__restrict__ sizes_host,
-                                                                const unsigned long long *__restrict__ group_tot) {
+                                                                const unsigned long long *__restrict__ group_tot,
+                                                                const unsigned long long *__restrict__ live_masks,
+                                                                unsigned long long *__restrict__ slot_stat) {
     __shared__ unsigned long long part[3][4];
     const uint32_t tile = blockIdx.x / (256u / PLAN_SUB), sub = blockIdx.x % (256u / PLAN_SUB);
     unsigned long long pn = 0, pm = 0, all_n = 0;
@@ -683,7 +735,8 @@
     __syncthreads();
     const uint32_t base_n = (uint32_t)((part[0][0] + part[0][1]) + (part[0][2] + part[0][3]));
     const unsigned long long base_m = (part[1][0] + part[1][1]) + (part[1][2] + part[1][3]);
-    const unsigned long long total = (part[2][0] + part[2][1]) + (part[2][2] + part[2][3]);
+    const unsigned long long total2 = (part[2][0] + part[2][1]) + (part[2][2] + part[2][3]);
+    const unsigned long long total = total2 & 0xFFFFFFFFull;
     __shared__ uint32_t lfirst[PLAN_SUB + 1];
     __shared__ TaskDesc ldesc[PLAN_SUB];
     __shared__ unsigned long long lm0[PLAN_SUB];
@@ -718,6 +771,10 @@
                 sizes_host[1] = task_moff ? lm0[threadIdx.x] : 0ull;
                 sizes_host[2] = base_n + lfirst[threadIdx.x];
             }
+            if (t == ntasks && slot_stat) {
+                slot_stat[0] = total;
+                slot_stat[1] = total2 >> 32;
+            }
         }
     }
     const uint32_t s0 = lfirst[0], s1 = lfirst[PLAN_SUB];
@@ -737,7 +794,8 @@
         else if (part3 == 1u) w = make_uint4(d.cb, d.flags, q * rps, 0u);
         else {
             const unsigned long long mo = task_moff ? lm0[lo] + (unsigned long long)q * 2u * nch : lm0[lo];
-            w = make_uint4((uint32_t)mo, (uint32_t)(mo >> 32), 0u, 0u);
+            const unsigned long long mp = (d.flags & SLOT_LIVE) ? (unsigned long long)(live_masks + (((uint64_t)tile * 256u + sub * PLAN_SUB + lo) * (uint64_t)LIVE_GROUPS)) : 0ull;
+            w = make_uint4((uint32_t)mo, (uint32_t)(mo >> 32), (uint32_t)mp, (uint32_t)(mp >> 32));
         }
         out[i] = w;
     }
@@ -1054,6 +1112,7 @@
     unsigned long long *sizes_dev = nullptr;
     bool drop_nonfinite = false;
     uint32_t slot_launch = 0;
+    bool live_rows = true;
 };
 
 struct OnSideStream {
@@ -1332,6 +1391,12 @@
         MH_HIP(hipGetLastError());
         return 0;
     }
+    if (c->plan_live && mode != MODE_HIST && !out.ids && fixed_cutoff_kind(cur.kind)) {
+        if (cur.kind == MOLAR_HIP_SEARCH_SINGLE) launch_pair_single_live(mode, P.nblocks, c->stream, dP, tf, st, sc, sb, out.pairs, out.dist);
+        else launch_pair_double_live(mode, P.nblocks, c->stream, dP, tf, st, sc, sb, out.pairs, out.dist);
+        MH_HIP(hipGetLastError());
+        return 0;
+    }
     switch (cur.kind) {
         case MOLAR_HIP_SEARCH_SINGLE: launch_pair_single(mode, P.nblocks, dyn_lds, c->stream, dP, tf, st, sc, sb, out.pairs, out.dist, out.ids); break;
         case MOLAR_HIP_SEARCH_DOUBLE: launch_pair_double(mode, P.nblocks, dyn_lds, c->stream, dP, tf, st, sc, sb, out.pairs, out.dist, out.ids); break;
@@ -1470,6 +1535,8 @@
     if (q->kind < 0 || q->kind > 3) return fail(MOLAR_HIP_ERR_INVALID_ARGUMENT, "search: unknown kind %d", q->kind);
     MH_HIP(hipSetDevice(c->device));
     c->have_search = false;
+    c->slot_stat_valid = false;
+    c->plan_live = false;
     SearchShape &cur = c->cur;
     cur.kind = q->kind;
     const bool two = q->kind != MOLAR_HIP_SEARCH_SINGLE;
@@ -1573,6 +1640,20 @@
     MH_TRY(c->task_mu.reserve((cur.ntasks + 1) * 4));
     MH_TRY(c->task_moff.reserve((cur.ntasks + 1) * 8));
     const uint32_t fast_kind = records_hit_history(cur) ? 1u : 0u;
+    MH_TRY(c->slot_stat.reserve(16));
+    const bool use_live = call.plan && call.live_rows && !call.hist_plan && live_row_slots(cur);
+    auto enqueue_live_rows = [&]() -> int {
+        if (!use_live) return 0;
+        MH_TRY(cur.set[0].live.reserve(live_rows_bytes(cur)));
+        unsigned long long *masks = cur.set[0].live.as<unsigned long long>();
+        uint32_t *cnt = reinterpret_cast<uint32_t *>(masks + live_rows_mask_words(cur));
+        const SearchParams P = make_params(c, cur);
+        const dim3 grid = pair_grid((unsigned)cur.ntasks);
+        if (cur.kind == MOLAR_HIP_SEARCH_SINGLE) hipLaunchKernelGGL((live_rows_kernel<MOLAR_HIP_SEARCH_SINGLE>), grid, dim3(64), 0, c->stream, P, masks, cnt);
+        else hipLaunchKernelGGL((live_rows_kernel<MOLAR_HIP_SEARCH_DOUBLE>), grid, dim3(64), 0, c->stream, P, masks, cnt);
+        MH_HIP(hipGetLastError());
+        return 0;
+    };
     auto enqueue_plan = [&]() -> int {
         Prof prof(c, 0);
         SearchParams P = make_params(c, cur);
@@ -1592,17 +1673,22 @@
             unsigned long long *tt = c->fplan_tiles.as<unsigned long long>();
             unsigned long long *lmoff = tt + 2 * (size_t)ntiles;
             uint32_t *lfirst = c->task_mu.as<uint32_t>();
+            const unsigned long long *live_masks = use_live ? cur.set[0].live.as<unsigned long long>() : nullptr;
+            const uint32_t *live_cnt = use_live ? reinterpret_cast<const uint32_t *>(live_masks + live_rows_mask_words(cur)) : nullptr;
             if (cur.kind == MOLAR_HIP_SEARCH_SINGLE)
                 hipLaunchKernelGGL((plan_tiles_kernel<MOLAR_HIP_SEARCH_SINGLE>), dim3(ntiles), dim3(256), 0, c->stream, P, lfirst,
-                                   c->task_desc.as<TaskDesc>(), lmoff, fast_kind, c->slot_cnt.as<uint32_t>(), cur.nslots_bound + 1, tt, params_dst);
+                                   c->task_desc.as<TaskDesc>(), lmoff, fast_kind, c->slot_cnt.as<uint32_t>(), cur.nslots_bound + 1, tt, params_dst, live_cnt);
             else
                 hipLaunchKernelGGL((plan_tiles_kernel<MOLAR_HIP_SEARCH_DOUBLE>), dim3(ntiles), dim3(256), 0, c->stream, P, lfirst,
-                                   c->task_desc.as<TaskDesc>(), lmoff, fast_kind, c->slot_cnt.as<uint32_t>(), cur.nslots_bound + 1, tt, params_dst);
+                                   c->task_desc.as<TaskDesc>(), lmoff, fast_kind, c->slot_cnt.as<uint32_t>(), cur.nslots_bound + 1, tt, params_dst, live_cnt);
             unsigned long long *gt = ngroups ? lmoff + (cur.ntasks + 1) : nullptr;
             if (ngroups) hipLaunchKernelGGL(plan_groups_kernel, dim3(ngroups), dim3(64), 0, c->stream, ntiles, tt, gt);
             hipLaunchKernelGGL(plan_slots_kernel, dim3(ntiles * (256u / PLAN_SUB)), dim3(256), 0, c->stream, cur.ntasks, ntiles, lfirst, lmoff, c->task_nb.as<uint32_t>(),
-                               c->task_desc.as<TaskDesc>(), moff, tt, c->slot_desc.as<SlotDesc>(), cur.nslots_bound, call.sizes_dev, gt);
+                               c->task_desc.as<TaskDesc>(), moff, tt, c->slot_desc.as<SlotDesc>(), cur.nslots_bound, call.sizes_dev, gt,
+                               live_masks, c->slot_stat.as<unsigned long long>());
             MH_HIP(hipGetLastError());
+            c->slot_stat_valid = true;
+            c->plan_live = use_live;
             return 0;
         }
         const uint64_t nplan = std::max<uint64_t>(std::max<uint64_t>(cur.ntasks + 1, cur.nslots_bound + 1), st_tasks + st_slots);
@@ -1632,6 +1718,7 @@
             OnSideStream on_side(c);
             if (!reuse0) MH_TRY(build_grid(c, call, cur.set[0], q->ids_local || vdw));
             if (two) MH_TRY(build_grid(c, call, cur.set[1], q->ids_local || vdw));
+            MH_TRY(enqueue_live_rows());
             MH_HIP(hipEventRecord(c->grid_done, c->side_stream));
         }
         if (c->env_host_grid_wait) MH_HIP(hipEventSynchronize(c->grid_done));
@@ -1639,6 +1726,7 @@
     } else {
         if (!reuse0) MH_TRY(build_grid(c, call, cur.set[0], q->ids_local || vdw));
         if (two) MH_TRY(build_grid(c, call, cur.set[1], q->ids_local || vdw));
+        MH_TRY(enqueue_live_rows());
     }
     if (may_hold && !reuse0) {
         c->hold_valid = true;
@@ -1879,6 +1967,17 @@
     return MOLAR_HIP_OK;
 }
 
+int molar_hip_search_slot_counts(molar_hip_ctx *c, uint64_t *slots, uint64_t *consecutive_slots) {
+    if (!c || !slots || !consecutive_slots) return fail(MOLAR_HIP_ERR_INVALID_ARGUMENT, "search_slot_counts: null argument");
+    if (!c->slot_stat_valid) return fail(MOLAR_HIP_ERR_NO_SEARCH, "search_slot_counts: the context's last search was not planned by plan_slots_kernel");
+    MH_HIP(hipSetDevice(c->device));
+    unsigned long long st[2] = {0ull, 0ull};
+    MH_TRY(read_back(c, st, c->slot_stat.p, sizeof st));
+    *slots = st[0];
+    *consecutive_slots = st[1];
+    return MOLAR_HIP_OK;
+}
+
 static int fill_common(molar_hip_ctx *c, uint2 *d_pairs, float *d_dist, uint32_t *d_ids) {
     if (!c || !c->have_search) return fail(MOLAR_HIP_ERR_NO_SEARCH, "no cached search: call molar_hip_search_count first");
     MH_HIP(hipSetDevice(c->device));
@@ -2684,6 +2783,7 @@
     qq.ids_local = 1;
     SearchCall call;
     call.size_masks = false;
+    call.live_rows = false;
     MH_TRY(prepare_search(s, &qq, call));
     s->params_fresh = false;
     const SearchShape &cur = s->cur;
diff --git a/molar_amd/csrc/search_shape.hpp b/molar_amd/csrc/search_shape.hpp
--- a/molar_amd/csrc/search_shape.hpp
+++ b/molar_amd/csrc/search_shape.hpp
@@ -75,6 +75,16 @@
     return bound;
 }
 
+constexpr uint64_t FPLAN_MAX_TASKS = 1ull << 22;
+
+constexpr uint32_t LIVE_ROW_GROUPS = 8;
+inline bool live_row_slots(const SearchShape &s) {
+    return fixed_cutoff_kind(s.kind) && pair_family(s) == 0 && plan_entries(s) + 1 <= FPLAN_MAX_TASKS &&
+           (plan_entries(s) <= 8192ull || (uint64_t)s.set[0].n >= 96ull * grid_cells(s));
+}
+inline size_t live_rows_mask_words(const SearchShape &s) { return (size_t)plan_entries(s) * LIVE_ROW_GROUPS; }
+inline size_t live_rows_bytes(const SearchShape &s) { return live_rows_mask_words(s) * 8u + (size_t)plan_entries(s) * 4u; }
+
 struct WrapPolicy {
     uint32_t wrap_kind;
     uint32_t prune_wrapped;
diff --git a/rust/molar_hip/src/ffi.rs b/rust/molar_hip/src/ffi.rs
--- a/rust/molar_hip/src/ffi.rs
+++ b/rust/molar_hip/src/ffi.rs
@@ -41,6 +41,7 @@
     pub unwrap_connectivity: unsafe extern "C" fn(*mut MolarHipCtx, *mut f32, usize, *const u64, usize, *const f32, f32, u8, *mut u64, *mut u64, *mut usize) -> c_int,
     pub search_grid_dims: unsafe extern "C" fn(*mut MolarHipCtx, *mut u64) -> c_int,
     pub search_cell_kernels: unsafe extern "C" fn(*mut MolarHipCtx, *mut i32, *mut u64) -> c_int,
+    pub search_slot_counts: unsafe extern "C" fn(*mut MolarHipCtx, *mut u64, *mut u64) -> c_int,
     pub search_fill_device: unsafe extern "C" fn(*mut MolarHipCtx, *mut *const u32, *mut *const f32) -> c_int,
     pub search_resident: unsafe extern "C" fn(*mut MolarHipCtx, *const MolarHipSearchDesc, *mut u64, *mut *const u32, *mut *const f32) -> c_int,
     pub search_resident_planes: unsafe extern "C" fn(*mut MolarHipCtx, c_int) -> c_int,
@@ -192,6 +193,7 @@
                 unwrap_connectivity: *lib.get::<unsafe extern "C" fn(*mut MolarHipCtx, *mut f32, usize, *const u64, usize, *const f32, f32, u8, *mut u64, *mut u64, *mut usize) -> c_int>(b"molar_hip_unwrap_connectivity\0")?,
                 search_grid_dims: *lib.get::<unsafe extern "C" fn(*mut MolarHipCtx, *mut u64) -> c_int>(b"molar_hip_search_grid_dims\0")?,
                 search_cell_kernels: *lib.get::<unsafe extern "C" fn(*mut MolarHipCtx, *mut i32, *mut u64) -> c_int>(b"molar_hip_search_cell_kernels\0")?,
+                search_slot_counts: *lib.get::<unsafe extern "C" fn(*mut MolarHipCtx, *mut u64, *mut u64) -> c_int>(b"molar_hip_search_slot_counts\0")?,
                 search_fill_device: *lib.get::<unsafe extern "C" fn(*mut MolarHipCtx, *mut *const u32, *mut *const f32) -> c_int>(b"molar_hip_search_fill_device\0")?,
                 search_resident: *lib.get::<unsafe extern "C" fn(*mut MolarHipCtx, *const MolarHipSearchDesc, *mut u64, *mut *const u32, *mut *const f32) -> c_int>(b"molar_hip_search_resident\0")?,
                 search_resident_planes: *lib.get::<unsafe extern "C" fn(*mut MolarHipCtx, c_int) -> c_int>(b"molar_hip_search_resident_planes\0")?,
@@ -310,4 +312,4 @@
     }
 }
 
-pub const ENTRY_POINTS: usize = 145;
+pub const ENTRY_POINTS: usize = 146;
```

Measured after the change: 775.6 frames/s (median of 6 runs). 1.05x the previous value.
